# Ali-Xiyao/emr2a-evidence-grounded-multimodal-retrieval

Measured on NVIDIA B200. Metric: queries/sec (cosine Top-K + vote), higher is better.
Workload: dtype bf16+f32

## Files before the change

### emr2a_b200/csrc/api.cu

```cuda
#include "common.cuh"

#include <math.h>
#include <stdlib.h>
#include <string.h>

namespace emr2a {

static thread_local char g_err[512] = "";

int fail(int code, const char* fmt, ...) {
  va_list ap;
  va_start(ap, fmt);
  vsnprintf(g_err, sizeof(g_err), fmt, ap);
  va_end(ap);
  return code;
}
int cuda_fail(cudaError_t e, const char* where) {
  snprintf(g_err, sizeof(g_err), "CUDA error %d (%s) at %s", static_cast<int>(e), cudaGetErrorString(e), where);
  cudaGetLastError();
  return EMR2A_ERR_CUDA;
}
int sm_count() {
  int dev = 0, n = 0;
  if (cudaGetDevice(&dev) != cudaSuccess) return 148;
  if (cudaDeviceGetAttribute(&n, cudaDevAttrMultiProcessorCount, dev) != cudaSuccess || n <= 0) return 148;
  return n;
}

size_t simt_topk_workspace_bytes(int64_t Q, int64_t N, int K);
int simt_topk_search(const float* q, const float* db, int64_t Q, int64_t N, int D, int64_t ldq, int64_t lddb,
                     const uint8_t* q_fold, const uint8_t* db_fold, int64_t idx_base, int K, uint64_t* out_keys,
                     void* workspace, size_t ws_bytes, cudaStream_t st);
size_t tc_topk_workspace_bytes(int64_t Q, int64_t N, int K, int D);
int tc_debug_unit_clocks(unsigned long long* host_out, int64_t cap_units, int64_t* plan_out);
struct TcPartials {
  const uint64_t* parts;
  int splits;
  const uint32_t* tau;
};
int tc_topk_search(const uint16_t* q_hi, const uint16_t* q_lo, const uint16_t* db_hi, const uint16_t* db_lo,
                   int64_t Q, int64_t N, int D, int64_t ldq, int64_t lddb, const uint8_t* q_fold,
                   const uint8_t* db_fold, int64_t idx_base, int K, int passes, uint64_t* out_keys,
                   void* workspace, size_t ws_bytes, float* debug_scores, cudaStream_t st, TcPartials* partials,
                   int fold_sorted, int min_splits);
int tc_planned_splits(int64_t Q, int64_t N, int min_splits);
int tc_timing_enable(int on);
int tc_timing_read(float* ms_out, int cap, int* n_out);
void tc_timing_record(int which, cudaStream_t st);
int tc_range_filter(const uint16_t* q_hi, const uint16_t* db_hi, int64_t Q, int64_t N, int D, int64_t ldq, int64_t lddb,
                    const uint8_t* q_fold, const uint8_t* db_fold, int fold_sorted, int64_t idx_base, float min_score,
                    const float* q_stats, const float* db_stats, uint64_t* cand, int64_t cand_cap,
                    unsigned long long* count, void* workspace, size_t ws_bytes, cudaStream_t st);

size_t rescore_workspace_bytes(int64_t Q, int K);
int rescore_pipeline(const uint64_t* approx, int KP, const uint32_t* tau, const float* q, int64_t ldq, const float* db,
                     int64_t lddb, const emr2a_lazy_rows* db_lazy, const uint16_t* db_hi, int64_t lddb_hi, int64_t Q, int64_t N,
                     int D, int64_t idx_base, int K,
                     const float* q_stats, const float* db_stats, const uint8_t* q_fold, const uint8_t* db_fold,
                     uint64_t* out_keys, int* status, uint8_t* qflags, void* workspace, size_t ws_bytes, cudaStream_t st);

int rescore_kth_scores(const uint64_t* approx, int KP, int K, int64_t Q, float* kth, cudaStream_t st);
int rescore_select_only(const uint64_t* approx, int KP, const uint32_t* tau, const float* kth_floor, const float* q,
                        int64_t ldq, const float* db, int64_t lddb, const emr2a_lazy_rows* db_lazy, int64_t Q, int64_t N, int D,
                        int64_t idx_base, int K, const float* q_stats, const float* db_stats, uint64_t* out_keys,
                        float* bound_out, cudaStream_t st);
int rescore_verify_merged(const uint64_t* keys, int K, int64_t Q, const float* bounds, int parts, int64_t bounds_stride,
                          uint8_t* flags, int* count, cudaStream_t st);
size_t exact_rescan_workspace_bytes(int n_flagged, int K);
int rescore_exact_rescan(const float* q, int64_t ldq, const float* db, int64_t lddb, const emr2a_lazy_rows* db_lazy, int64_t N,
                         int D, int64_t idx_base, int K, const uint8_t* q_fold, const uint8_t* db_fold, const int* flag_list,
                         int n_flagged, uint64_t* out_compact, void* workspace, size_t ws_bytes, const uint16_t* db_hi,
                         int64_t lddb_hi, const float* q_stats, const float* db_stats, const uint64_t* seed_keys,
                         cudaStream_t st);

int range_refine_check(const float* q, int64_t ldq, const float* db, int64_t lddb, const emr2a_lazy_rows* db_lazy, int D);
int range_refine(const uint64_t* cand, int64_t cand_cap, unsigned long long* counts, uint64_t* out, int64_t out_cap,
                 const float* q, int64_t ldq, const float* db, int64_t lddb, const emr2a_lazy_rows* db_lazy, int D,
                 int64_t idx_base, float min_score, cudaStream_t st);

constexpr int RESCORE_KP = 32;
constexpr int RESCORE_KPM = 64;
static inline size_t align256(size_t x) { return (x + 255) & ~static_cast<size_t>(255); }

__global__ void zero_keys_kernel(uint64_t* k, int64_t n) {
  const int64_t i = static_cast<int64_t>(blockIdx.x) * blockDim.x + threadIdx.x;
  if (i < n) k[i] = 0ull;
}

}

using namespace emr2a;

extern "C" int emr2a_abi_version(void) { return EMR2A_ABI_VERSION; }
extern "C" const char* emr2a_last_error(void) { return g_err; }

extern "C" int emr2a_device_check(int* sms, int* cc_major, int* cc_minor) {
  int dev = 0;
  EMR2A_CUDA_TRY(cudaGetDevice(&dev));
  int major = 0, minor = 0, n = 0;
  EMR2A_CUDA_TRY(cudaDeviceGetAttribute(&major, cudaDevAttrComputeCapabilityMajor, dev));
  EMR2A_CUDA_TRY(cudaDeviceGetAttribute(&minor, cudaDevAttrComputeCapabilityMinor, dev));
  EMR2A_CUDA_TRY(cudaDeviceGetAttribute(&n, cudaDevAttrMultiProcessorCount, dev));
  if (sms) *sms = n;
  if (cc_major) *cc_major = major;
  if (cc_minor) *cc_minor = minor;
  if (major != 10) return fail(EMR2A_ERR_UNSUPPORTED, "libemr2a is built for sm_100a only; device is sm_%d%d", major, minor);
  return EMR2A_OK;
}

extern "C" size_t emr2a_topk_search_workspace_bytes(int64_t Q, int64_t N, int D, int K, int precision) {
  if (Q <= 0 || N <= 0 || K <= 0) return 256;
  if (precision == EMR2A_PREC_FP32) return simt_topk_workspace_bytes(Q, N, K) + 256;
  if (precision == EMR2A_PREC_BF16_RESCORE) {
    return align256(sizeof(uint64_t) * static_cast<size_t>(Q) * RESCORE_KPM) +
           align256(tc_topk_workspace_bytes(Q, N, RESCORE_KP, D)) + align256(rescore_workspace_bytes(Q, K));
  }
  return tc_topk_workspace_bytes(Q, N, K, D);
}

static int rescore_filter_stage(const uint16_t* q_hi, int64_t ldq_bf16, const uint16_t* db_hi, int64_t lddb_bf16, int64_t Q,
                                int64_t N, int D, const uint8_t* q_fold, const uint8_t* db_fold, int fold_sorted,
                                int64_t idx_base, int K, uint64_t* approx, void* tc_ws, size_t tc_ws_bytes,
                                float* debug_scores, cudaStream_t st, const uint64_t** cand, int* kpm,
                                const uint32_t** tau) {
  TcPartials parts{};
  const int planned = tc_planned_splits(Q, N, 2);
  int kp = planned > 128 ? 8 : ((planned >= 8 || K <= 5) ? 16 : RESCORE_KP);
  {
    const char* e = getenv("EMR2A_RESCORE_KP");
    const int v = (e && *e) ? atoi(e) : 0;
    if (v == 8 || v == 16 || v == 32) kp = v;
  }
  int rc = tc_topk_search(q_hi, nullptr, db_hi, nullptr, Q, N, D, ldq_bf16, lddb_bf16, q_fold, db_fold, idx_base,
                          kp, 1, nullptr, tc_ws, tc_ws_bytes, debug_scores, st, &parts, fold_sorted, 2);
  if (rc != EMR2A_OK) return rc;
  *kpm = kp;
  *cand = parts.parts;
  *tau = parts.tau;
  if (parts.splits > 1) {
    *kpm = RESCORE_KPM;
    rc = emr2a_topk_merge(parts.parts, parts.splits, Q, kp, Q * kp, kp, RESCORE_KPM, approx, st);
    if (rc != EMR2A_OK) return rc;
    *cand = approx;
  }
  return EMR2A_OK;
}

static int topk_search_impl(const float* q_f32, int64_t ldq_f32, const uint16_t* q_hi, const uint16_t* q_lo,
                            int64_t ldq_bf16, const float* db_f32, int64_t lddb_f32, const uint16_t* db_hi,
                            const uint16_t* db_lo, int64_t lddb_bf16, int64_t Q, int64_t N, int D,
                            const uint8_t* q_fold, const uint8_t* db_fold, int fold_sorted, int64_t idx_base, int K,
                            int precision, const float* q_stats, const float* db_stats, uint64_t* out_keys,
                            int32_t* status, uint8_t* qflags, void* workspace, size_t ws_bytes, float* debug_scores,
                            const emr2a_lazy_rows* db_lazy, void* stream) {
  if (Q < 0 || N < 0 || D <= 0 || K <= 0 || !out_keys) return fail(EMR2A_ERR_INVALID, "topk_search: bad arguments (Q=%lld N=%lld D=%d K=%d)", (long long)Q, (long long)N, D, K);
  if ((q_fold == nullptr) != (db_fold == nullptr)) return fail(EMR2A_ERR_INVALID, "topk_search: q_fold and db_fold must be given together");
  if (idx_base < 0) return fail(EMR2A_ERR_INVALID, "topk_search: negative idx_base");
  cudaStream_t st = static_cast<cudaStream_t>(stream);
  if (Q == 0) return EMR2A_OK;
  if (N == 0) {
    const int64_t n = Q * K;
    zero_keys_kernel<<<static_cast<unsigned>((n + 255) / 256), 256, 0, st>>>(out_keys, n);
    EMR2A_LAUNCH_CHECK("zero_keys_kernel");
    return EMR2A_OK;
  }
  switch (precision) {
    case EMR2A_PREC_FP32:
      if (!q_f32 || !db_f32) return fail(EMR2A_ERR_INVALID, "topk_search(fp32): q_f32/db_f32 required");
      if (ldq_f32 < D || lddb_f32 < D) return fail(EMR2A_ERR_INVALID, "topk_search(fp32): leading dimension smaller than D");
      return simt_topk_search(q_f32, db_f32, Q, N, D, ldq_f32, lddb_f32, q_fold, db_fold, idx_base, K, out_keys, workspace, ws_bytes, st);
    case EMR2A_PREC_BF16X3:
      return tc_topk_search(q_hi, q_lo, db_hi, db_lo, Q, N, D, ldq_bf16, lddb_bf16, q_fold, db_fold, idx_base, K, 3, out_keys, workspace, ws_bytes, debug_scores, st, nullptr, fold_sorted, 1);
    case EMR2A_PREC_BF16X1:
      return tc_topk_search(q_hi, nullptr, db_hi, nullptr, Q, N, D, ldq_bf16, lddb_bf16, q_fold, db_fold, idx_base, K, 1, out_keys, workspace, ws_bytes, debug_scores, st, nullptr, fold_sorted, 1);
    case EMR2A_PREC_BF16_RESCORE: {
      if (K > 10) return fail(EMR2A_ERR_UNSUPPORTED, "topk_search(rescore): K=%d > 10 (use EMR2A_PREC_BF16X3)", K);
      if (!q_f32 || (!db_f32 && !db_lazy)) return fail(EMR2A_ERR_INVALID, "topk_search(rescore): q_f32 and db_f32 (or db_lazy) required");
      if (ldq_f32 < D || (!db_lazy && lddb_f32 < D)) return fail(EMR2A_ERR_INVALID, "topk_search(rescore): leading dimension smaller than D");
      if (!workspace || (reinterpret_cast<uintptr_t>(workspace) & 255)) return fail(EMR2A_ERR_INVALID, "topk_search(rescore): workspace must be 256-byte aligned");
      const size_t a_bytes = align256(sizeof(uint64_t) * static_cast<size_t>(Q) * RESCORE_KPM);
      const size_t t_bytes = align256(tc_topk_workspace_bytes(Q, N, RESCORE_KP, D));
      const size_t r_bytes = align256(rescore_workspace_bytes(Q, K));
      if (ws_bytes < a_bytes + t_bytes + r_bytes) return fail(EMR2A_ERR_WORKSPACE, "topk_search(rescore): workspace %zu < %zu", ws_bytes, a_bytes + t_bytes + r_bytes);
      uint8_t* ws = static_cast<uint8_t*>(workspace);
      const uint64_t* cand = nullptr;
      const uint32_t* tau = nullptr;
      int kpm = 0;
      int rc = rescore_filter_stage(q_hi, ldq_bf16, db_hi, lddb_bf16, Q, N, D, q_fold, db_fold, fold_sorted, idx_base, K,
                                    reinterpret_cast<uint64_t*>(ws), ws + a_bytes, t_bytes, debug_scores, st, &cand, &kpm, &tau);
      if (rc != EMR2A_OK) return rc;
      return rescore_pipeline(cand, kpm, tau, q_f32, ldq_f32, db_f32, lddb_f32, db_lazy, db_hi, lddb_bf16, Q, N, D, idx_base, K, q_stats,
                              db_stats, q_fold, db_fold, out_keys, status, qflags, ws + a_bytes + t_bytes, r_bytes, st);
    }
    default:
      return fail(EMR2A_ERR_INVALID, "topk_search: unknown precision %d", precision);
  }
}

extern "C" int emr2a_topk_search(const float* q_f32, int64_t ldq_f32, const uint16_t* q_hi, const uint16_t* q_lo,
                                 int64_t ldq_bf16, const float* db_f32, int64_t lddb_f32, const uint16_t* db_hi,
                                 const uint16_t* db_lo, int64_t lddb_bf16, int64_t Q, int64_t N, int D,
                                 const uint8_t* q_fold, const uint8_t* db_fold, int fold_sorted, int64_t idx_base,
                                 int K, int precision, const float* q_stats, const float* db_stats,
                                 uint64_t* out_keys, int32_t* status_out, uint8_t* unverified_out, void* workspace,
                                 size_t ws_bytes, const emr2a_lazy_rows* db_lazy, void* stream) {
  if (db_lazy && precision != EMR2A_PREC_BF16_RESCORE) return fail(EMR2A_ERR_INVALID, "topk_search: db_lazy is for EMR2A_PREC_BF16_RESCORE only");
  return topk_search_impl(q_f32, ldq_f32, q_hi, q_lo, ldq_bf16, db_f32, lddb_f32, db_hi, db_lo, lddb_bf16, Q, N, D,
                          q_fold, db_fold, fold_sorted, idx_base, K, precision, q_stats, db_stats, out_keys,
                          status_out, unverified_out, workspace, ws_bytes, nullptr, db_lazy, stream);
}

extern "C" int emr2a_debug_topk_search_dump(const uint16_t* q_hi, const uint16_t* q_lo, const uint16_t* db_hi,
                                            const uint16_t* db_lo, int64_t Q, int64_t N, int D, int64_t ldq,
                                            int64_t lddb, const uint8_t* q_fold, const uint8_t* db_fold,
                                            int64_t idx_base, int K, int precision, uint64_t* out_keys,
                                            void* workspace, size_t ws_bytes, float* debug_scores, void* stream) {
  if (precision != EMR2A_PREC_BF16X3 && precision != EMR2A_PREC_BF16X1)
    return fail(EMR2A_ERR_INVALID, "debug dump is for the tensor-core arms only");
  return topk_search_impl(nullptr, 0, q_hi, q_lo, ldq, nullptr, 0, db_hi, db_lo, lddb, Q, N, D, q_fold, db_fold, 0,
                          idx_base, K, precision, nullptr, nullptr, out_keys, nullptr, nullptr, workspace, ws_bytes,
                          debug_scores, nullptr, stream);
}

extern "C" int emr2a_debug_unit_clocks(uint64_t* host_out, int64_t cap_units, int64_t* plan_out) {
  if (!host_out || !plan_out) return fail(EMR2A_ERR_INVALID, "debug_unit_clocks: null output");
  return tc_debug_unit_clocks(reinterpret_cast<unsigned long long*>(host_out), cap_units, plan_out);
}

extern "C" size_t emr2a_topk_filter_workspace_bytes(int64_t Q, int64_t N, int D, int K) {
  if (Q <= 0 || N <= 0 || K <= 0) return 256;
  return align256(tc_topk_workspace_bytes(Q, N, RESCORE_KP, D));
}

extern "C" int emr2a_topk_filter(const uint16_t* q_hi, int64_t ldq_bf16, const uint16_t* db_hi, int64_t lddb_bf16, int64_t Q,
                                 int64_t N, int D, const uint8_t* q_fold, const uint8_t* db_fold, int fold_sorted,
                                 int64_t idx_base, int K, uint64_t* cand_out, uint32_t* tau_out, float* kth_out,
                                 void* workspace, size_t ws_bytes, void* stream) {
  if (Q < 0 || N < 0 || D <= 0 || K <= 0 || !cand_out || !tau_out) return fail(EMR2A_ERR_INVALID, "topk_filter: bad arguments");
  if (K > 10) return fail(EMR2A_ERR_UNSUPPORTED, "topk_filter: K=%d > 10 (use EMR2A_PREC_BF16X3)", K);
  if ((q_fold == nullptr) != (db_fold == nullptr)) return fail(EMR2A_ERR_INVALID, "topk_filter: q_fold and db_fold must be given together");
  cudaStream_t st = static_cast<cudaStream_t>(stream);
  if (Q == 0) return EMR2A_OK;
  EMR2A_CUDA_TRY(cudaMemsetAsync(tau_out, 0, sizeof(uint32_t) * static_cast<size_t>(Q), st));
  if (N == 0) {
    const int64_t n = Q * RESCORE_KPM;
    zero_keys_kernel<<<static_cast<unsigned>((n + 255) / 256), 256, 0, st>>>(cand_out, n);
    EMR2A_LAUNCH_CHECK("zero_keys_kernel");
  } else {
    if (!workspace || (reinterpret_cast<uintptr_t>(workspace) & 255)) return fail(EMR2A_ERR_INVALID, "topk_filter: workspace must be 256-byte aligned");
    const uint64_t* cand = nullptr;
    const uint32_t* tau = nullptr;
    int kpm = 0;
    int rc = rescore_filter_stage(q_hi, ldq_bf16, db_hi, lddb_bf16, Q, N, D, q_fold, db_fold, fold_sorted, idx_base, K,
                                  cand_out, workspace, ws_bytes, nullptr, st, &cand, &kpm, &tau);
    if (rc != EMR2A_OK) return rc;
    if (cand != cand_out) {
      rc = emr2a_topk_merge(cand, 1, Q, kpm, Q * kpm, kpm, RESCORE_KPM, cand_out, st);
      if (rc != EMR2A_OK) return rc;
    }
    if (tau) EMR2A_CUDA_TRY(cudaMemcpyAsync(tau_out, tau, sizeof(uint32_t) * static_cast<size_t>(Q), cudaMemcpyDeviceToDevice, st));
  }
  if (kth_out) return rescore_kth_scores(cand_out, RESCORE_KPM, K, Q, kth_out, st);
  return EMR2A_OK;
}

extern "C" int emr2a_rescore_candidates(const uint64_t* cand, const uint32_t* tau, const float* kth_floor, const float* q_f32,
                                        int64_t ldq_f32, const float* db_f32, int64_t lddb_f32, int64_t Q, int64_t N, int D,
                                        int64_t idx_base, int K, const float* q_stats, const float* db_stats,
                                        uint64_t* out_keys, float* bound_out, const emr2a_lazy_rows* db_lazy,
                                        void* stream) {
  if (!cand || !tau || !q_f32 || (!db_f32 && !db_lazy) || !q_stats || !db_stats || !out_keys || !bound_out || Q < 0 || N < 0 ||
      D <= 0 || K <= 0 || K > 10 || ldq_f32 < D || (!db_lazy && lddb_f32 < D))
    return fail(EMR2A_ERR_INVALID, "rescore_candidates: bad arguments");
  if (Q == 0) return EMR2A_OK;
  return rescore_select_only(cand, RESCORE_KPM, tau, kth_floor, q_f32, ldq_f32, db_f32, lddb_f32, db_lazy, Q, N, D, idx_base,
                             K, q_stats, db_stats, out_keys, bound_out, static_cast<cudaStream_t>(stream));
}

extern "C" int emr2a_verify_merged(const uint64_t* keys, int K, int64_t Q, const float* bounds, int parts,
                                   int64_t bounds_stride, uint8_t* flags_out, int32_t* status_out, void* stream) {
  if (!keys || !bounds || !flags_out || !status_out || K <= 0 || Q < 0 || parts <= 0 || bounds_stride < Q)
    return fail(EMR2A_ERR_INVALID, "verify_merged: bad arguments");
  if (Q == 0) return EMR2A_OK;
  return rescore_verify_merged(keys, K, Q, bounds, parts, bounds_stride, flags_out, status_out, static_cast<cudaStream_t>(stream));
}

extern "C" size_t emr2a_exact_rescan_workspace_bytes(int n_flagged, int K) { return exact_rescan_workspace_bytes(n_flagged, K) + 256; }

extern "C" int emr2a_exact_rescan(const float* q_f32, int64_t ldq_f32, const float* db_f32, int64_t lddb_f32, int64_t N, int D,
                                  int64_t idx_base, int K, const uint8_t* q_fold, const uint8_t* db_fold,
                                  const int32_t* flag_list, int n_flagged, uint64_t* out_keys, void* workspace,
                                  size_t ws_bytes, const emr2a_lazy_rows* db_lazy, const uint16_t* db_hi,
                                  int64_t lddb_bf16, const float* q_stats, const float* db_stats,
                                  const uint64_t* seed_keys, void* stream) {
  if (!q_f32 || (!db_f32 && !db_lazy && N > 0) || !out_keys || N < 0 || D <= 0 || K <= 0 || n_flagged < 0 || ldq_f32 < D ||
      (!db_lazy && N > 0 && lddb_f32 < D) || (n_flagged > 0 && !flag_list))
    return fail(EMR2A_ERR_INVALID, "exact_rescan: bad arguments");
  if ((q_fold == nullptr) != (db_fold == nullptr)) return fail(EMR2A_ERR_INVALID, "exact_rescan: q_fold and db_fold must be given together");
  if (n_flagged == 0) return EMR2A_OK;
  cudaStream_t st = static_cast<cudaStream_t>(stream);
  if (N == 0) {
    const int64_t n = static_cast<int64_t>(n_flagged) * K;
    zero_keys_kernel<<<static_cast<unsigned>((n + 255) / 256), 256, 0, st>>>(out_keys, n);
    EMR2A_LAUNCH_CHECK("zero_keys_kernel");
    return EMR2A_OK;
  }
  return rescore_exact_rescan(q_f32, ldq_f32, db_f32, lddb_f32, db_lazy, N, D, idx_base, K, q_fold, db_fold, flag_list,
                              n_flagged, out_keys, workspace, ws_bytes, db_hi, lddb_bf16, q_stats, db_stats, seed_keys, st);
}

extern "C" size_t emr2a_range_search_workspace_bytes(int64_t Q, int64_t N, int D) {
  if (Q <= 0 || N <= 0 || D <= 0) return 256;
  return align256(tc_topk_workspace_bytes(Q, N, 1, D));
}

extern "C" int emr2a_range_search(const float* q_f32, int64_t ldq_f32, const uint16_t* q_hi, int64_t ldq_bf16,
                                  const float* db_f32, int64_t lddb_f32, const uint16_t* db_hi, int64_t lddb_bf16,
                                  int64_t Q, int64_t N, int D, const uint8_t* q_fold, const uint8_t* db_fold,
                                  int fold_sorted, int64_t idx_base, float min_score, const float* q_stats,
                                  const float* db_stats, uint64_t* cand, int64_t cand_cap, uint64_t* results,
                                  int64_t result_cap, uint64_t* counts_out, void* workspace, size_t ws_bytes,
                                  const emr2a_lazy_rows* db_lazy, void* stream) {
  if (Q < 0 || N < 0 || D <= 0 || cand_cap < 0 || result_cap < 0 || !counts_out || (cand_cap > 0 && !cand) ||
      (result_cap > 0 && !results))
    return fail(EMR2A_ERR_INVALID, "range_search: bad arguments (Q=%lld N=%lld D=%d)", (long long)Q, (long long)N, D);
  if (!isfinite(min_score)) return fail(EMR2A_ERR_INVALID, "range_search: min_score must be finite");
  if ((q_fold == nullptr) != (db_fold == nullptr)) return fail(EMR2A_ERR_INVALID, "range_search: q_fold and db_fold must be given together");
  if (idx_base < 0) return fail(EMR2A_ERR_INVALID, "range_search: negative idx_base");
  if (!q_f32 || (!db_f32 && !db_lazy) || !q_stats || !db_stats)
    return fail(EMR2A_ERR_INVALID, "range_search: q_f32, db_f32 (or db_lazy), q_stats and db_stats required");
  if (ldq_f32 < D || (!db_lazy && lddb_f32 < D)) return fail(EMR2A_ERR_INVALID, "range_search: leading dimension smaller than D");
  if (Q == 0 || N == 0) return EMR2A_OK;
  if (!workspace || (reinterpret_cast<uintptr_t>(workspace) & 255)) return fail(EMR2A_ERR_INVALID, "range_search: workspace must be 256-byte aligned");
  int rc = range_refine_check(q_f32, ldq_f32, db_f32, lddb_f32, db_lazy, D);
  if (rc != EMR2A_OK) return rc;
  cudaStream_t st = static_cast<cudaStream_t>(stream);
  unsigned long long* counts = reinterpret_cast<unsigned long long*>(counts_out);
  rc = tc_range_filter(q_hi, db_hi, Q, N, D, ldq_bf16, lddb_bf16, q_fold, db_fold, fold_sorted, idx_base, min_score,
                           q_stats, db_stats, cand, cand_cap, counts, workspace, ws_bytes, st);
  if (rc != EMR2A_OK) return rc;
  tc_timing_record(0, st);
  rc = range_refine(cand, cand_cap, counts, results, result_cap, q_f32, ldq_f32, db_f32, lddb_f32, db_lazy, D, idx_base,
                    min_score, st);
  tc_timing_record(1, st);
  return rc;
}

extern "C" int emr2a_debug_tc_timing(int enable) { return tc_timing_enable(enable); }
extern "C" int emr2a_debug_tc_elapsed(float* ms_out_host, int cap, int* n_out_host) {
  if (!ms_out_host || !n_out_host || cap <= 0) return fail(EMR2A_ERR_INVALID, "debug_tc_elapsed: bad arguments");
  return tc_timing_read(ms_out_host, cap, n_out_host);
}
```

### emr2a_b200/csrc/normalize_fuse.cu

```cuda
#include <type_traits>
#include "row_math.cuh"

namespace emr2a {

struct NfParams {
  const void* seg0;
  const void* seg1;
  int64_t n;
  int d0, d1;
  int64_t ld0, ld1;
  float w0, w1;
  int flags;
  float* out_f32;
  int64_t ld_f32;
  uint16_t* out_hi;
  uint16_t* out_lo;
  int64_t ld_bf16;
  float* inv_norm;
  float* stats;
  const float* col_std;
  float* row_div;
};

__device__ __forceinline__ void stats_flush(float* stats, float max_norm2, float max_res2) {
  unsigned int* u = reinterpret_cast<unsigned int*>(stats);
  atomicMax(u, __float_as_uint(__fsqrt_ru(max_norm2)));
  atomicMax(u + 1, __float_as_uint(__fsqrt_ru(max_res2)));
}

template <typename InT, int MAXC>
__device__ __forceinline__ void load_row(const NfParams& p, int64_t row, int lane, int c0, int ctot, float4 (&v)[MAXC]) {
#pragma unroll
  for (int j = 0; j < MAXC; ++j) {
    const int c = lane + 32 * j;
    if (c < c0) v[j] = Loader<InT>::load4(p.seg0, row * p.ld0 + 4 * c);
    else if (c < ctot) v[j] = Loader<InT>::load4(p.seg1, row * p.ld1 + 4 * (c - c0));
    else v[j] = make_float4(0.f, 0.f, 0.f, 0.f);
  }
}

__device__ __forceinline__ float std1(float x, float m, float s, float r) {
  const float t = __fsub_rn(x, m);
  const float q0 = t * r;
  const float rem = fmaf(-q0, s, t);
  return fmaf(rem, r, q0);
}
__device__ __forceinline__ void standardize4(float4& v, const float* __restrict__ col_std, int dtot, int col) {
  const float4 m = __ldg(reinterpret_cast<const float4*>(col_std + col));
  const float4 s = __ldg(reinterpret_cast<const float4*>(col_std + dtot + col));
  const float4 r = __ldg(reinterpret_cast<const float4*>(col_std + 2 * dtot + col));
  v.x = std1(v.x, m.x, s.x, r.x); v.y = std1(v.y, m.y, s.y, r.y);
  v.z = std1(v.z, m.z, s.z, r.z); v.w = std1(v.w, m.w, s.w, r.w);
}

template <typename InT, int MAXC, bool WANT_LO, bool STATS, bool STD = false>
__global__ void __launch_bounds__(256, (MAXC <= 8 ? 2 : 1)) normalize_fuse_vec_kernel(const NfParams p) {
  const int lane = threadIdx.x & 31;
  const int64_t warp0 = (static_cast<int64_t>(blockIdx.x) * blockDim.x + threadIdx.x) >> 5;
  const int64_t nwarps = (static_cast<int64_t>(gridDim.x) * blockDim.x) >> 5;
  const int c0 = p.d0 >> 2;
  const int ctot = (p.d0 + p.d1) >> 2;
  const int cpad = p.out_hi ? static_cast<int>(p.ld_bf16 >> 2) : ctot;
  constexpr bool PREFETCH = MAXC <= 8;
  float max_n2 = 0.f, max_r2 = 0.f;

  float4 nxt[PREFETCH ? MAXC : 1];
  if (PREFETCH && warp0 < p.n) load_row<InT, MAXC>(p, warp0, lane, c0, ctot, reinterpret_cast<float4 (&)[MAXC]>(nxt));

  for (int64_t row = warp0; row < p.n; row += nwarps) {
    float4 v[MAXC];
    if (PREFETCH) {
#pragma unroll
      for (int j = 0; j < MAXC; ++j) v[j] = nxt[PREFETCH ? j : 0];
      if (row + nwarps < p.n) load_row<InT, MAXC>(p, row + nwarps, lane, c0, ctot, reinterpret_cast<float4 (&)[MAXC]>(nxt));
    } else {
      load_row<InT, MAXC>(p, row, lane, c0, ctot, v);
    }
    if (STD) {
#pragma unroll
      for (int j = 0; j < MAXC; ++j) {
        const int c = lane + 32 * j;
        if (c < ctot) standardize4(v[j], p.col_std, p.d0 + p.d1, 4 * c);
      }
    }
    float ss0 = 0.f, ss1 = 0.f;
    float4 divs = make_float4(1.f, 1.f, 1.f, 0.f);
    if (p.flags & EMR2A_NF_SEGNORM) {
#pragma unroll
      for (int j = 0; j < MAXC; ++j) {
        const int c = lane + 32 * j;
        if (c < c0) ss0 += sq4(v[j]); else ss1 += sq4(v[j]);
      }
    }
    if (p.flags & EMR2A_NF_SEGNORM) {
      const RowDiv n0 = row_div(__fsqrt_rn(warp_sum(ss0)) + EMR2A_EPS);
      const RowDiv n1 = row_div(__fsqrt_rn(warp_sum(ss1)) + EMR2A_EPS);
      divs.x = n0.d; divs.y = n1.d;
#pragma unroll
      for (int j = 0; j < MAXC; ++j) {
        const int c = lane + 32 * j;
        if (c < c0) div4(v[j], n0); else if (c < ctot) div4(v[j], n1);
      }
    }
    if (p.w0 != 1.0f || p.w1 != 1.0f) {
#pragma unroll
      for (int j = 0; j < MAXC; ++j) {
        const int c = lane + 32 * j;
        if (c < c0) mul4(v[j], p.w0); else if (c < ctot) mul4(v[j], p.w1);
      }
    }
    float inv = 1.0f;
    if (p.flags & (EMR2A_NF_ROWNORM | EMR2A_NF_ZERO_GUARD)) {
      float ss = 0.f;
#pragma unroll
      for (int j = 0; j < MAXC; ++j) ss += sq4(v[j]);
      float nrm = __fsqrt_rn(warp_sum(ss));
      const bool guard = (p.flags & EMR2A_NF_ZERO_GUARD) != 0;
      if (!guard) nrm += EMR2A_EPS;
      if (!(guard && nrm == 0.f)) {
        const RowDiv dv = row_div(nrm);
#pragma unroll
        for (int j = 0; j < MAXC; ++j) div4(v[j], dv);
        inv = dv.r;
        divs.z = nrm; divs.w = 1.f;
      }
    }
    if (p.inv_norm && lane == 0) p.inv_norm[row] = inv;
    if (p.row_div && lane == 0) reinterpret_cast<float4*>(p.row_div)[row] = divs;
    if (p.out_f32) {
#pragma unroll
      for (int j = 0; j < MAXC; ++j) {
        const int c = lane + 32 * j;
        if (c < ctot) *reinterpret_cast<float4*>(p.out_f32 + row * p.ld_f32 + 4 * c) = v[j];
      }
    }
    if (p.out_hi) {
      float n2 = 0.f, r2 = 0.f;
#pragma unroll
      for (int j = 0; j < MAXC; ++j) {
        const int c = lane + 32 * j;
        if (c < cpad) {
          const __nv_bfloat162 h01 = __floats2bfloat162_rn(v[j].x, v[j].y);
          const __nv_bfloat162 h23 = __floats2bfloat162_rn(v[j].z, v[j].w);
          const uint32_t u01 = *reinterpret_cast<const uint32_t*>(&h01);
          const uint32_t u23 = *reinterpret_cast<const uint32_t*>(&h23);
          *reinterpret_cast<uint2*>(p.out_hi + row * p.ld_bf16 + 4 * c) = make_uint2(u01, u23);
          if (WANT_LO || STATS) {
            const float e0 = v[j].x - __uint_as_float(u01 << 16);
            const float e1 = v[j].y - __uint_as_float(u01 & 0xFFFF0000u);
            const float e2 = v[j].z - __uint_as_float(u23 << 16);
            const float e3 = v[j].w - __uint_as_float(u23 & 0xFFFF0000u);
            if (STATS) {
              n2 += sq4(v[j]);
              r2 += e0 * e0 + e1 * e1 + e2 * e2 + e3 * e3;
            }
            if (WANT_LO) {
              const __nv_bfloat162 l01 = __floats2bfloat162_rn(e0, e1);
              const __nv_bfloat162 l23 = __floats2bfloat162_rn(e2, e3);
              *reinterpret_cast<uint2*>(p.out_lo + row * p.ld_bf16 + 4 * c) =
                  make_uint2(*reinterpret_cast<const uint32_t*>(&l01), *reinterpret_cast<const uint32_t*>(&l23));
            }
          }
        }
      }
      if (STATS) {
        max_n2 = fmaxf(max_n2, warp_sum(n2));
        max_r2 = fmaxf(max_r2, warp_sum(r2));
      }
    }
  }
  if (STATS && lane == 0 && warp0 < p.n) stats_flush(p.stats, max_n2, max_r2);
}

__device__ __forceinline__ float2 block_sum2(float a, float b, float2* red) {
  a = warp_sum(a); b = warp_sum(b);
  if ((threadIdx.x & 31) == 0) red[threadIdx.x >> 5] = make_float2(a, b);
  __syncthreads();
  float2 t = make_float2(0.f, 0.f);
#pragma unroll
  for (int w = 0; w < 8; ++w) { t.x += red[w].x; t.y += red[w].y; }
  __syncthreads();
  return t;
}

template <typename InT, int CPT>
__device__ __forceinline__ void load_row_block(const NfParams& p, int64_t row, int c0, int ctot,
                                               typename Loader<InT>::Raw (&v)[CPT]) {
#pragma unroll
  for (int j = 0; j < CPT; ++j) {
    const int c = threadIdx.x + 256 * j;
    if (c < c0) v[j] = Loader<InT>::load_raw(p.seg0, row * p.ld0 + 4 * c);
    else if (c < ctot) v[j] = Loader<InT>::load_raw(p.seg1, row * p.ld1 + 4 * (c - c0));
  }
}

template <typename InT, int CPT>
__global__ void __launch_bounds__(256, 2) normalize_fuse_block_kernel(const NfParams p) {
  typedef typename Loader<InT>::Raw Raw;
  constexpr int PF = sizeof(Raw) == 16 ? 1 : 2;
  __shared__ float2 red[8];
  const int c0 = p.d0 >> 2;
  const int ctot = (p.d0 + p.d1) >> 2;
  const int cpad = p.out_hi ? static_cast<int>(p.ld_bf16 >> 2) : ctot;
  float max_n2 = 0.f, max_r2 = 0.f;
  Raw ring[PF][CPT];
#pragma unroll
  for (int s = 0; s < PF; ++s) {
    const int64_t r = blockIdx.x + static_cast<int64_t>(s) * gridDim.x;
    if (r < p.n) load_row_block<InT, CPT>(p, r, c0, ctot, ring[s]);
  }
  for (int64_t base = blockIdx.x; base < p.n; base += static_cast<int64_t>(PF) * gridDim.x) {
#pragma unroll
   for (int s = 0; s < PF; ++s) {
    const int64_t row = base + static_cast<int64_t>(s) * gridDim.x;
    if (row >= p.n) break;
    float4 v[CPT];
#pragma unroll
    for (int j = 0; j < CPT; ++j) {
      const int c = threadIdx.x + 256 * j;
      v[j] = c < ctot ? Loader<InT>::widen(ring[s][j]) : make_float4(0.f, 0.f, 0.f, 0.f);
    }
    {
      const int64_t r2 = row + static_cast<int64_t>(PF) * gridDim.x;
      if (r2 < p.n) load_row_block<InT, CPT>(p, r2, c0, ctot, ring[s]);
    }
    float4 divs = make_float4(1.f, 1.f, 1.f, 0.f);
    if (p.flags & EMR2A_NF_SEGNORM) {
      float ss0 = 0.f, ss1 = 0.f;
#pragma unroll
      for (int j = 0; j < CPT; ++j) {
        const int c = threadIdx.x + 256 * j;
        if (c < c0) ss0 += sq4(v[j]); else ss1 += sq4(v[j]);
      }
      const float2 t = block_sum2(ss0, ss1, red);
      const RowDiv n0 = row_div(__fsqrt_rn(t.x) + EMR2A_EPS);
      const RowDiv n1 = row_div(__fsqrt_rn(t.y) + EMR2A_EPS);
      divs.x = n0.d; divs.y = n1.d;
#pragma unroll
      for (int j = 0; j < CPT; ++j) {
        const int c = threadIdx.x + 256 * j;
        if (c < c0) div4(v[j], n0); else if (c < ctot) div4(v[j], n1);
      }
    }
    if (p.w0 != 1.0f || p.w1 != 1.0f) {
#pragma unroll
      for (int j = 0; j < CPT; ++j) {
        const int c = threadIdx.x + 256 * j;
        if (c < c0) mul4(v[j], p.w0); else if (c < ctot) mul4(v[j], p.w1);
      }
    }
    float inv = 1.0f;
    if (p.flags & (EMR2A_NF_ROWNORM | EMR2A_NF_ZERO_GUARD)) {
// ... 215 lines not shown
```

### emr2a_b200/csrc/tc_common.cuh

```cuda
#pragma once
#include <cuda.h>
#include "common.cuh"

namespace emr2a {

constexpr int T_BM = 128;
constexpr int T_BN = 256;
constexpr int T_BK = 64;
constexpr int T_THREADS = 256;
constexpr uint32_t T_A_BYTES = T_BM * T_BK * 2;
constexpr uint32_t T_B_BYTES = T_BN * T_BK * 2;

struct TcParams {
  int64_t Q, N;
  int k_chunks;
  int64_t m_tiles, n_tiles;
  int splits;
  int64_t tiles_per_split;
  const uint8_t* q_fold;
  const uint8_t* db_fold;
  int fold_sorted;
  int64_t idx_base;
  int K;
  uint64_t* keys_out;
  uint32_t* tau;
  float* debug_scores;
  int64_t mg;
  int sync_tiles;
  int sync_points;
  int sync_budget;
  uint32_t* sync_ctr;
  unsigned long long* unit_clock;
  float range_t;
  int D;
  const float* q_stats;
  const float* db_stats;
  ulonglong2* range_out;
  int64_t range_cap;
  unsigned long long* range_count;
};

__device__ __forceinline__ uint32_t smem_u32(const void* p) { return static_cast<uint32_t>(__cvta_generic_to_shared(p)); }

__device__ __forceinline__ void mbar_init(uint32_t bar, uint32_t count) {
  asm volatile("mbarrier.init.shared::cta.b64 [%0], %1;" ::"r"(bar), "r"(count));
}
__device__ __forceinline__ void mbar_arrive_expect_tx(uint32_t bar, uint32_t bytes) {
  asm volatile("mbarrier.arrive.expect_tx.shared::cta.b64 _, [%0], %1;" ::"r"(bar), "r"(bytes) : "memory");
}
__device__ __forceinline__ void mbar_arrive(uint32_t bar) {
  asm volatile("mbarrier.arrive.shared::cta.b64 _, [%0];" ::"r"(bar) : "memory");
}
__device__ __forceinline__ bool mbar_try_wait(uint32_t bar, uint32_t parity) {
  uint32_t ok;
  asm volatile(
      "{\n\t"
      ".reg .pred p;\n\t"
      "mbarrier.try_wait.parity.shared::cta.b64 p, [%1], %2;\n\t"
      "selp.u32 %0, 1, 0, p;\n\t"
      "}\n" : "=r"(ok) : "r"(bar), "r"(parity) : "memory");
  return ok != 0;
}
__device__ __forceinline__ void mbar_wait(uint32_t bar, uint32_t parity) {
  while (!mbar_try_wait(bar, parity)) {}
}
__device__ __forceinline__ void tma_load_2d(uint32_t dst, const CUtensorMap* map, uint32_t bar, int c0, int c1) {
  asm volatile(
      "cp.async.bulk.tensor.2d.shared::cluster.global.mbarrier::complete_tx::bytes [%0], [%1, {%3, %4}], [%2];"
      ::"r"(dst), "l"(reinterpret_cast<uint64_t>(map)), "r"(bar), "r"(c0), "r"(c1) : "memory");
}
__device__ __forceinline__ void tcgen05_fence_before() { asm volatile("tcgen05.fence::before_thread_sync;" ::: "memory"); }
__device__ __forceinline__ void tcgen05_fence_after() { asm volatile("tcgen05.fence::after_thread_sync;" ::: "memory"); }
__device__ __forceinline__ void umma_commit(uint32_t bar) {
  asm volatile("tcgen05.commit.cta_group::1.mbarrier::arrive::one.shared::cluster.b64 [%0];" ::"r"(bar) : "memory");
}
__device__ __forceinline__ void umma_bf16(uint32_t tmem_d, uint64_t desc_a, uint64_t desc_b, uint32_t idesc, uint32_t accumulate) {
  asm volatile(
      "{\n\t"
      ".reg .pred p;\n\t"
      "setp.ne.b32 p, %4, 0;\n\t"
      "tcgen05.mma.cta_group::1.kind::f16 [%0], %1, %2, %3, p;\n\t"
      "}\n" ::"r"(tmem_d), "l"(desc_a), "l"(desc_b), "r"(idesc), "r"(accumulate) : "memory");
}
__device__ __forceinline__ uint64_t make_smem_desc(uint32_t smem_addr) {
  uint64_t d = 0;
  d |= static_cast<uint64_t>((smem_addr & 0x3FFFFu) >> 4);
  d |= static_cast<uint64_t>(0) << 16;
  d |= static_cast<uint64_t>(1024 >> 4) << 32;
  d |= static_cast<uint64_t>(1) << 46;
  d |= static_cast<uint64_t>(2) << 61;
  return d;
}
__device__ __forceinline__ void tmem_ld32(uint32_t taddr, float (&v)[32]) {
  uint32_t r[32];
  asm volatile(
      "tcgen05.ld.sync.aligned.32x32b.x32.b32 "
      "{%0, %1, %2, %3, %4, %5, %6, %7, %8, %9, %10, %11, %12, %13, %14, %15, "
      "%16, %17, %18, %19, %20, %21, %22, %23, %24, %25, %26, %27, %28, %29, %30, %31}, [%32];"
      : "=r"(r[0]), "=r"(r[1]), "=r"(r[2]), "=r"(r[3]), "=r"(r[4]), "=r"(r[5]), "=r"(r[6]), "=r"(r[7]),
        "=r"(r[8]), "=r"(r[9]), "=r"(r[10]), "=r"(r[11]), "=r"(r[12]), "=r"(r[13]), "=r"(r[14]), "=r"(r[15]),
        "=r"(r[16]), "=r"(r[17]), "=r"(r[18]), "=r"(r[19]), "=r"(r[20]), "=r"(r[21]), "=r"(r[22]), "=r"(r[23]),
        "=r"(r[24]), "=r"(r[25]), "=r"(r[26]), "=r"(r[27]), "=r"(r[28]), "=r"(r[29]), "=r"(r[30]), "=r"(r[31])
      : "r"(taddr));
  asm volatile("tcgen05.wait::ld.sync.aligned;" ::: "memory");
#pragma unroll
  for (int i = 0; i < 32; ++i) v[i] = __uint_as_float(r[i]);
}

constexpr uint32_t T_IDESC = (1u << 4) | (1u << 7) | (1u << 10) | ((T_BN >> 3) << 17) | ((T_BM >> 4) << 24);

template <int KCAP>
struct RegTopK {
  float s[KCAP];
  uint32_t i[KCAP];
  __device__ __forceinline__ void reset() {
#pragma unroll
    for (int j = 0; j < KCAP; ++j) { s[j] = -INFINITY; i[j] = 0xFFFFFFFFu; }
  }
  __device__ __forceinline__ float threshold() const { return s[KCAP - 1]; }
  __device__ __forceinline__ void insert(float c, uint32_t ci) {
#pragma unroll
    for (int j = KCAP - 1; j > 0; --j) {
// ... 79 lines not shown
  bool mask_rows = HAS_FOLD, all_masked = false;
  if (HAS_FOLD && p.fold_sorted) {
    const int64_t last = (n0 + T_BN - 1 < p.N) ? n0 + T_BN - 1 : p.N - 1;
    const uint32_t f_lo = __ldg(p.db_fold + n0), f_hi = __ldg(p.db_fold + last);
    if (f_lo == f_hi) { mask_rows = false; all_masked = (f_lo == my_fold); }
  }
#pragma unroll 1
  for (int ch = 0; ch < T_BN / 32; ++ch) {
    float v[32];
    tmem_ld32(taddr + static_cast<uint32_t>(ch * 32), v);
    const int64_t c0 = n0 + ch * 32;
    if (p.debug_scores && q < p.Q) {
#pragma unroll
      for (int c = 0; c < 32; ++c) if (c0 + c < p.N) p.debug_scores[q * p.N + c0 + c] = v[c];
    }
    if (edge) {
#pragma unroll
      for (int c = 0; c < 32; ++c) if (c0 + c >= p.N) v[c] = -INFINITY;
    }
    if (HAS_FOLD && all_masked) {
#pragma unroll
      for (int c = 0; c < 32; ++c) v[c] = -INFINITY;
    }
    if (HAS_FOLD && mask_rows) {
      const uint4* fp = reinterpret_cast<const uint4*>(p.db_fold + c0);
      const uint4 f0 = __ldg(fp), f1 = __ldg(fp + 1);
      const uint32_t w[8] = {f0.x, f0.y, f0.z, f0.w, f1.x, f1.y, f1.z, f1.w};
#pragma unroll
      for (int c = 0; c < 32; ++c) {
        const uint32_t f = (w[c >> 2] >> (8 * (c & 3))) & 0xFFu;
        v[c] = (f == my_fold) ? -INFINITY : v[c];
      }
    }
    if constexpr (RANGE) {
      range_emit(p, v, thr, c0, q);
    } else {
      float mx = v[0];
#pragma unroll
      for (int c = 1; c < 32; ++c) mx = fmaxf(mx, v[c]);
      if (mx > thr) {
        uint32_t mask = 0u;
#pragma unroll
        for (int c = 0; c < 32; ++c) mask |= (v[c] > thr) ? (1u << c) : 0u;
        while (mask) {
          const int c = __ffs(mask) - 1;
          mask &= mask - 1u;
          const float val = select32(v, c);
          if (val > thr) {
            top.insert(val, static_cast<uint32_t>(c0 + c + p.idx_base));
            thr = fmaxf(top.threshold(), thr0);
          }
        }
      }
    }
    __syncwarp();
  }
}

__device__ __forceinline__ void unit_coords(const TcParams& p, int64_t u, int64_t& split, int64_t& mt) {
  const int64_t per_group = p.mg * p.splits;
  const int64_t g = u / per_group;
  const int64_t r = u - g * per_group;
  const int64_t left = p.m_tiles - g * p.mg;
  const int64_t mg_eff = left < p.mg ? left : p.mg;
  split = r / mg_eff;
  mt = g * p.mg + (r - split * mg_eff);
}
__device__ __forceinline__ void unit_cohort(const TcParams& p, int64_t u, int64_t n_workers, int64_t n_units,
                                            int64_t& slot, int& size) {
  const int64_t per_group = p.mg * p.splits;
  const int64_t g = u / per_group;
  const int64_t r = u - g * per_group;
  const int64_t left = p.m_tiles - g * p.mg;
  const int64_t mg_eff = left < p.mg ? left : p.mg;
  const int64_t split = r / mg_eff;
  int64_t c0 = g * per_group + split * mg_eff, c1 = c0 + mg_eff;
  const int64_t step = u / n_workers;
  const int64_t s0 = step * n_workers, s1 = (s0 + n_workers < n_units) ? s0 + n_workers : n_units;
  c0 = c0 > s0 ? c0 : s0;
  c1 = c1 < s1 ? c1 : s1;
  size = static_cast<int>(c1 - c0);
  slot = g * p.splits + split + step;
}
__device__ __forceinline__ void cohort_sync(const TcParams& p, int64_t slot, int point, int size) {
  uint32_t* ctr = p.sync_ctr + slot * p.sync_points + point;
  const uint32_t seen = atomicAdd(ctr, 1u) + 1u;
  if (seen >= static_cast<uint32_t>(size)) return;
  const long long t0 = clock64();
  while (__ldcg(ctr) < static_cast<uint32_t>(size)) {
    if (clock64() - t0 > p.sync_budget) break;
    __nanosleep(40);
  }
}

__device__ __forceinline__ float unit_start_threshold(const TcParams& p, int64_t q) {
  if (p.tau == nullptr || q >= p.Q) return -INFINITY;
  const uint32_t t = __ldcg(p.tau + q);
  if (t == 0u) return -INFINITY;
  const float b = unorder_f32(t);
  const uint32_t bits = __float_as_uint(b);
  if (b > 0.f) return __uint_as_float(bits - 1u);
  if (b < 0.f) return __uint_as_float(bits + 1u);
  return -1e-45f;
}

}
```

### emr2a_b200/csrc/topk_tc.cu

```cuda
#include <stdlib.h>
#include "tc_common.cuh"

namespace emr2a {

template <int PASSES, int KCAP, bool HAS_FOLD, bool RANGE = false>
__global__ void __launch_bounds__(T_THREADS, 1)
tc_topk_kernel(const __grid_constant__ CUtensorMap tm_q_hi, const __grid_constant__ CUtensorMap tm_q_lo,
               const __grid_constant__ CUtensorMap tm_db_hi, const __grid_constant__ CUtensorMap tm_db_lo,
               const TcParams p) {
  constexpr int PLANES = PASSES == 3 ? 2 : 1;
  constexpr uint32_t STAGE_BYTES = PLANES * (T_A_BYTES + T_B_BYTES);
  constexpr int STAGES = PASSES == 3 ? 2 : 4;

  extern __shared__ uint8_t smem_dyn[];
  __shared__ __align__(8) uint64_t bar_full[STAGES];
  __shared__ __align__(8) uint64_t bar_empty[STAGES];
  __shared__ __align__(8) uint64_t bar_tfull[2];
  __shared__ __align__(8) uint64_t bar_tempty[2];
  __shared__ uint32_t tmem_base_smem;

  const int warp = threadIdx.x >> 5;
  const int lane = threadIdx.x & 31;
  const uint32_t tiles_base = (smem_u32(smem_dyn) + 1023u) & ~1023u;

// ... 115 lines not shown
        scan_tile<KCAP, HAS_FOLD, RANGE>(p, top, thr, thr0,
                                         tmem_base + (static_cast<uint32_t>(quarter * 32) << 16) + static_cast<uint32_t>(acc * T_BN),
                                         n0, my_fold, q);
        tcgen05_fence_before();
        __syncwarp();
        if (lane == 0) mbar_arrive(smem_u32(&bar_tempty[acc]));
        if (++acc == 2) { acc = 0; acc_phase ^= 1u; }
      }
      if (!RANGE && q < p.Q) {
        if (p.tau != nullptr && top.i[KCAP - 1] != 0xFFFFFFFFu) atomicMax(p.tau + q, order_f32(top.s[KCAP - 1]));
        uint64_t* dst = p.keys_out + (split * p.Q + q) * p.K;
#pragma unroll
        for (int j = 0; j < KCAP; ++j)
          if (j < p.K) dst[j] = (top.i[j] == 0xFFFFFFFFu) ? 0ull : pack_key(top.s[j], top.i[j]);
      }
    }
  }

  tcgen05_fence_before();
  __syncthreads();
  if (warp == 2) {
    tcgen05_fence_after();
    asm volatile("tcgen05.dealloc.cta_group::1.sync.aligned.b32 %0, %1;" ::"r"(tmem_base), "n"(512));
  }
}

typedef CUresult (*PFN_encodeTiled)(CUtensorMap*, CUtensorMapDataType, cuuint32_t, void*, const cuuint64_t*,
                                    const cuuint64_t*, const cuuint32_t*, const cuuint32_t*, CUtensorMapInterleave,
                                    CUtensorMapSwizzle, CUtensorMapL2promotion, CUtensorMapFloatOOBfill);

static PFN_encodeTiled get_encode() {
  static PFN_encodeTiled fn = nullptr;
  if (!fn) {
    void* sym = nullptr;
    cudaDriverEntryPointQueryResult qres;
    if (cudaGetDriverEntryPoint("cuTensorMapEncodeTiled", &sym, cudaEnableDefault, &qres) == cudaSuccess &&
        qres == cudaDriverEntryPointSuccess)
      fn = reinterpret_cast<PFN_encodeTiled>(sym);
  }
  return fn;
}

static int make_plane_map(CUtensorMap* map, const uint16_t* base, int64_t rows, int64_t cols, int64_t ld, int box_rows) {
  PFN_encodeTiled enc = get_encode();
  if (!enc) return fail(EMR2A_ERR_CUDA, "cuTensorMapEncodeTiled entry point not available");
  cuuint64_t gdim[2] = {static_cast<cuuint64_t>(cols), static_cast<cuuint64_t>(rows)};
  cuuint64_t gstride[1] = {static_cast<cuuint64_t>(ld) * 2};
  cuuint32_t box[2] = {static_cast<cuuint32_t>(T_BK), static_cast<cuuint32_t>(box_rows)};
  cuuint32_t estr[2] = {1, 1};
  CUresult r = enc(map, CU_TENSOR_MAP_DATA_TYPE_BFLOAT16, 2, const_cast<uint16_t*>(base), gdim, gstride, box, estr,
                   CU_TENSOR_MAP_INTERLEAVE_NONE, CU_TENSOR_MAP_SWIZZLE_128B, CU_TENSOR_MAP_L2_PROMOTION_L2_256B,
                   CU_TENSOR_MAP_FLOAT_OOB_FILL_NONE);
  if (r != CUDA_SUCCESS) return fail(EMR2A_ERR_CUDA, "cuTensorMapEncodeTiled failed (CUresult %d): rows=%lld cols=%lld ld=%lld", (int)r, (long long)rows, (long long)cols, (long long)ld);
  return EMR2A_OK;
}

struct TcPartials {
  const uint64_t* parts;
  int splits;
  const uint32_t* tau;
};

struct TcPlan {
  int64_t m_tiles, n_tiles, tiles_per_split;
  int splits;
  int grid;
  size_t keys_bytes, fold_bytes, tau_bytes;
  int64_t mg;
  int sync_tiles, sync_points, sync_budget;
  size_t sync_bytes;
};

static int env_int(const char* name, int dflt) {
  const char* e = getenv(name);
  return (e && *e) ? atoi(e) : dflt;
}

constexpr int64_t UNIT_CLOCK_MAX = 1 << 16;
__device__ unsigned long long g_unit_clock[2 * UNIT_CLOCK_MAX];
static int64_t g_last_plan[8];

int tc2_dispatch(int passes, int kcap, bool has_fold, const CUtensorMap& a, const CUtensorMap& b, const CUtensorMap& c,
                 const CUtensorMap& d, const TcParams& p, int grid, cudaStream_t st);

static bool use_cta_pairs(int64_t Q) {
  static int v = -1;
  if (v < 0) {
    const char* e = getenv("EMR2A_TC2");
    v = !e ? 2 : (e[0] == '0' ? 0 : 1);
  }
  return v == 2 ? Q > T_BM : v == 1;
}

static TcPlan tc_plan(int64_t Q, int64_t N, int K, bool has_fold, bool pairs, int min_splits = 1, int64_t ld = 1024,
                      int planes = 1) {
  TcPlan pl{};
  const int bm = pairs ? 2 * T_BM : T_BM;
  pl.m_tiles = (Q + bm - 1) / bm;
  pl.n_tiles = (N + T_BN - 1) / T_BN;
  const int sms = pairs ? sm_count() / 2 : sm_count();
  int best_s = 1; double best_eff = -1.0;
  int64_t cap = 64;
  if (pl.m_tiles * cap < sms) {
    const int kcap = K <= 8 ? 8 : (K <= 16 ? 16 : 32);
    cap = sms < 2048 / kcap ? sms : 2048 / kcap;
    if (cap < 64) cap = 64;
  }
  const int64_t max_s = pl.n_tiles < cap ? pl.n_tiles : cap;
  int64_t first_s = min_splits < max_s ? min_splits : max_s;
  if (first_s < 1) first_s = 1;
  best_s = static_cast<int>(first_s);
  for (int64_t s = first_s; s <= max_s; ++s) {
    const int64_t tps = (pl.n_tiles + s - 1) / s;
    const int64_t s_eff = (pl.n_tiles + tps - 1) / tps;
    if (s_eff != s) continue;
    const int64_t units = pl.m_tiles * s;
    const int64_t waves = (units + sms - 1) / sms;
    const double cost = static_cast<double>(waves) * (static_cast<double>(tps) + 2.0);
    const double ideal = static_cast<double>(pl.m_tiles) * pl.n_tiles / sms;
    const double eff = ideal / cost;
    if (eff > best_eff + 1e-9) { best_eff = eff; best_s = static_cast<int>(s); }
  }
  pl.splits = best_s;
  pl.tiles_per_split = (pl.n_tiles + pl.splits - 1) / pl.splits;
  const int64_t units = pl.m_tiles * pl.splits;
  pl.grid = static_cast<int>(units < sms ? units : sms) * (pairs ? 2 : 1);
  pl.keys_bytes = sizeof(uint64_t) * static_cast<size_t>(pl.splits) * Q * K;
  pl.fold_bytes = has_fold ? static_cast<size_t>(pl.n_tiles) * T_BN : 0;
  pl.tau_bytes = (sizeof(uint32_t) * static_cast<size_t>(Q) + 255) & ~static_cast<size_t>(255);
  pl.mg = pl.m_tiles;
  if (pairs) {
    const double a_tile = 2.0 * T_BM * static_cast<double>(ld) * 2.0 * planes;
    int64_t mg = static_cast<int64_t>(env_int("EMR2A_TC_A_MB", 40) * 1048576.0 / a_tile);
    if (mg < 1) mg = 1;
    if (mg < pl.m_tiles) {
      const int64_t j = (sms + mg - 1) / mg;
      mg = sms / j;
      if (mg < 1) mg = 1;
      pl.mg = mg;
    }
    const double b_tile = static_cast<double>(T_BN) * static_cast<double>(ld) * 2.0 * planes;
    int st = static_cast<int>(2097152.0 / b_tile + 0.5);
    st = st < 1 ? 1 : (st > 16 ? 16 : st);
    st = env_int("EMR2A_TC_SYNC", st);
    const int64_t cohort_max = pl.mg < pl.m_tiles ? pl.mg : pl.m_tiles;
    if (st > 0 && cohort_max > 1 && units > 1) {
      pl.sync_tiles = st;
      pl.sync_points = static_cast<int>((pl.tiles_per_split + st - 1) / st);
      pl.sync_budget = env_int("EMR2A_TC_SYNC_BUDGET", 12000);
      const int64_t groups = (pl.m_tiles + pl.mg - 1) / pl.mg;
      const int64_t slots = groups * pl.splits + (units + sms - 1) / sms + 2;
      pl.sync_bytes = (sizeof(uint32_t) * static_cast<size_t>(slots) * pl.sync_points + 255) & ~static_cast<size_t>(255);
    }
  }
  return pl;
}

int tc_planned_splits(int64_t Q, int64_t N, int min_splits) {
  return tc_plan(Q, N, 1, false, use_cta_pairs(Q), min_splits).splits;
}

size_t tc_topk_workspace_bytes(int64_t Q, int64_t N, int K, int D) {
  size_t need = 0;
  const int64_t ld = (static_cast<int64_t>(D) + T_BK - 1) / T_BK * T_BK;
  for (int v = 0; v < 8; ++v) {
    TcPlan pl = tc_plan(Q, N, K, true, (v & 1) != 0, (v & 2) ? 2 : 1, ld, (v & 4) ? 2 : 1);
    const size_t b = ((pl.keys_bytes + 255) & ~static_cast<size_t>(255)) + pl.fold_bytes + pl.tau_bytes + pl.sync_bytes + 1024;
    need = b > need ? b : need;
  }
  return need;
}

int tc_debug_unit_clocks(unsigned long long* host_out, int64_t cap_units, int64_t* plan_out) {
  for (int i = 0; i < 8; ++i) plan_out[i] = g_last_plan[i];
  int64_t n = g_last_plan[7];
  if (n > cap_units) n = cap_units;
  if (n > UNIT_CLOCK_MAX) n = UNIT_CLOCK_MAX;
  if (n > 0) EMR2A_CUDA_TRY(cudaMemcpyFromSymbol(host_out, g_unit_clock, sizeof(unsigned long long) * 2 * n));
  return EMR2A_OK;
}

constexpr int TC_EV_RING = 1024;
static cudaEvent_t g_tc_ev[TC_EV_RING][2];
static bool g_tc_ev_made[TC_EV_RING];
static long long g_tc_ev_count = 0;
static int g_tc_ev_on = 0;

static void tc_ev_record(int which, cudaStream_t st) {
  if (!g_tc_ev_on) return;
  const int slot = static_cast<int>(g_tc_ev_count % TC_EV_RING);
  if (!g_tc_ev_made[slot]) {
    if (cudaEventCreate(&g_tc_ev[slot][0]) != cudaSuccess || cudaEventCreate(&g_tc_ev[slot][1]) != cudaSuccess) { g_tc_ev_on = 0; return; }
    g_tc_ev_made[slot] = true;
  }
  cudaEventRecord(g_tc_ev[slot][which], st);
  if (which == 1) ++g_tc_ev_count;
}
int tc_timing_enable(int on) {
  g_tc_ev_on = on ? 1 : 0;
  g_tc_ev_count = 0;
  return EMR2A_OK;
}
int tc_timing_read(float* ms_out, int cap, int* n_out) {
  long long n = g_tc_ev_count < TC_EV_RING ? g_tc_ev_count : TC_EV_RING;
  if (n > cap) n = cap;
  for (long long i = 0; i < n; ++i) {
    const int slot = static_cast<int>((g_tc_ev_count - n + i) % TC_EV_RING);
    EMR2A_CUDA_TRY(cudaEventSynchronize(g_tc_ev[slot][1]));
    EMR2A_CUDA_TRY(cudaEventElapsedTime(ms_out + i, g_tc_ev[slot][0], g_tc_ev[slot][1]));
  }
  *n_out = static_cast<int>(n);
  return EMR2A_OK;
}

template <int PASSES, int KCAP, bool HAS_FOLD, bool RANGE = false>
static int tc_launch(const CUtensorMap& mq_hi, const CUtensorMap& mq_lo, const CUtensorMap& md_hi, const CUtensorMap& md_lo,
                     const TcParams& p, int grid, cudaStream_t st) {
  constexpr int PLANES = PASSES == 3 ? 2 : 1;
  constexpr int STAGES = PASSES == 3 ? 2 : 4;
  const size_t smem = static_cast<size_t>(STAGES) * PLANES * (T_A_BYTES + T_B_BYTES) + 1024;
  auto kern = tc_topk_kernel<PASSES, KCAP, HAS_FOLD, RANGE>;
  EMR2A_CUDA_TRY(cudaFuncSetAttribute(kern, cudaFuncAttributeMaxDynamicSharedMemorySize, static_cast<int>(smem)));
  kern<<<grid, T_THREADS, smem, st>>>(mq_hi, mq_lo, md_hi, md_lo, p);
  EMR2A_LAUNCH_CHECK("tc_topk_kernel");
  return EMR2A_OK;
}

template <int PASSES, int KCAP>
static int tc_launch_fold(bool has_fold, const CUtensorMap& a, const CUtensorMap& b, const CUtensorMap& c, const CUtensorMap& d,
                          const TcParams& p, int grid, cudaStream_t st) {
  return has_fold ? tc_launch<PASSES, KCAP, true>(a, b, c, d, p, grid, st)
                  : tc_launch<PASSES, KCAP, false>(a, b, c, d, p, grid, st);
}

static int check_planes(const char* who, const uint16_t* q_hi, const uint16_t* q_lo, const uint16_t* db_hi,
                        const uint16_t* db_lo, int64_t Q, int64_t N, int D, int64_t ldq, int64_t lddb, int64_t idx_base,
                        int passes) {
  const int64_t Dp = (static_cast<int64_t>(D) + T_BK - 1) / T_BK * T_BK;
  if (ldq < Dp || lddb < Dp || (ldq % 8) || (lddb % 8))
    return fail(EMR2A_ERR_UNSUPPORTED, "%s: planes need ld >= round_up(D,64) and ld %% 8 == 0 (ldq=%lld lddb=%lld D=%d)", who, (long long)ldq, (long long)lddb, D);
  if (!q_hi || !db_hi || (passes == 3 && (!q_lo || !db_lo))) return fail(EMR2A_ERR_INVALID, "%s: missing operand plane", who);
  auto mis = [](const void* ptr) { return (reinterpret_cast<uintptr_t>(ptr) & 15) != 0; };
  if (mis(q_hi) || mis(db_hi) || (passes == 3 && (mis(q_lo) || mis(db_lo))))
    return fail(EMR2A_ERR_UNSUPPORTED, "%s: operand planes must be 16-byte aligned", who);
  if (Q >= (1LL << 31) || N >= (1LL << 31) - T_BN) return fail(EMR2A_ERR_UNSUPPORTED, "%s: Q/N too large for one call", who);
  if (N + idx_base >= 0xFFFFFFFFLL) return fail(EMR2A_ERR_UNSUPPORTED, "%s: global index exceeds 32 bits", who);
  return EMR2A_OK;
}

int tc_topk_search(const uint16_t* q_hi, const uint16_t* q_lo, const uint16_t* db_hi, const uint16_t* db_lo,
                   int64_t Q, int64_t N, int D, int64_t ldq, int64_t lddb,
                   const uint8_t* q_fold, const uint8_t* db_fold, int64_t idx_base, int K, int passes,
                   uint64_t* out_keys, void* workspace, size_t ws_bytes, float* debug_scores, cudaStream_t st,
                   TcPartials* partials, int fold_sorted, int min_splits) {
  if (K > 32) return fail(EMR2A_ERR_UNSUPPORTED, "topk_search(bf16): K=%d > 32 (use EMR2A_PREC_FP32)", K);
  const int64_t Dp = (static_cast<int64_t>(D) + T_BK - 1) / T_BK * T_BK;
  {
    const int rc = check_planes("topk_search(bf16)", q_hi, q_lo, db_hi, db_lo, Q, N, D, ldq, lddb, idx_base, passes);
    if (rc != EMR2A_OK) return rc;
  }
  const bool has_fold = q_fold != nullptr;
  const bool pairs = use_cta_pairs(Q);
  TcPlan pl = tc_plan(Q, N, K, has_fold, pairs, min_splits, lddb > ldq ? lddb : ldq, passes == 3 ? 2 : 1);
  const size_t keys_off = 0;
  const size_t fold_off = (pl.keys_bytes + 255) & ~static_cast<size_t>(255);
  const size_t tau_off = (fold_off + pl.fold_bytes + 255) & ~static_cast<size_t>(255);
  const size_t sync_off = tau_off + pl.tau_bytes;
  const size_t need = sync_off + pl.sync_bytes;
  if (!workspace || ws_bytes < need) return fail(EMR2A_ERR_WORKSPACE, "topk_search(bf16): workspace %zu < %zu", ws_bytes, need);
  uint8_t* ws = static_cast<uint8_t*>(workspace);
  if ((reinterpret_cast<uintptr_t>(ws) & 255) != 0) return fail(EMR2A_ERR_INVALID, "topk_search(bf16): workspace must be 256-byte aligned");

  CUtensorMap mq_hi, mq_lo, md_hi, md_lo;
  int rc;
  if ((rc = make_plane_map(&mq_hi, q_hi, Q, Dp, ldq, T_BM)) != EMR2A_OK) return rc;
  const int db_box = pairs ? T_BN / 2 : T_BN;
  if ((rc = make_plane_map(&md_hi, db_hi, N, Dp, lddb, db_box)) != EMR2A_OK) return rc;
  if (passes == 3) {
    if ((rc = make_plane_map(&mq_lo, q_lo, Q, Dp, ldq, T_BM)) != EMR2A_OK) return rc;
    if ((rc = make_plane_map(&md_lo, db_lo, N, Dp, lddb, db_box)) != EMR2A_OK) return rc;
  } else {
    mq_lo = mq_hi; md_lo = md_hi;
  }
  TcParams p{};
  p.Q = Q; p.N = N; p.k_chunks = static_cast<int>(Dp / T_BK);
  p.m_tiles = pl.m_tiles; p.n_tiles = pl.n_tiles; p.splits = pl.splits; p.tiles_per_split = pl.tiles_per_split;
  p.idx_base = idx_base; p.K = K; p.debug_scores = debug_scores;
  p.keys_out = (pl.splits > 1 || partials) ? reinterpret_cast<uint64_t*>(ws + keys_off) : out_keys;
  if (pl.splits > 1) {
    p.tau = reinterpret_cast<uint32_t*>(ws + tau_off);
    EMR2A_CUDA_TRY(cudaMemsetAsync(p.tau, 0, sizeof(uint32_t) * static_cast<size_t>(Q), st));
  }
  p.mg = pl.mg;
  if (pairs && pl.sync_bytes) {
    p.sync_tiles = pl.sync_tiles; p.sync_points = pl.sync_points; p.sync_budget = pl.sync_budget;
    p.sync_ctr = reinterpret_cast<uint32_t*>(ws + sync_off);
    EMR2A_CUDA_TRY(cudaMemsetAsync(p.sync_ctr, 0, pl.sync_bytes, st));
  }
  if (pairs && env_int("EMR2A_TC_UNIT_CLOCK", 0) && pl.m_tiles * pl.splits <= UNIT_CLOCK_MAX) {
    void* sym = nullptr;
    EMR2A_CUDA_TRY(cudaGetSymbolAddress(&sym, g_unit_clock));
    p.unit_clock = static_cast<unsigned long long*>(sym);
    const int64_t plan[8] = {pl.m_tiles, pl.n_tiles, pl.splits, pl.tiles_per_split, pl.mg, pl.sync_tiles, pl.grid,
                             pl.m_tiles * pl.splits};
    for (int i = 0; i < 8; ++i) g_last_plan[i] = plan[i];
  }
  if (has_fold) {
    uint8_t* fpad = ws + fold_off;
    EMR2A_CUDA_TRY(cudaMemsetAsync(fpad, 0xFF, pl.fold_bytes, st));
    EMR2A_CUDA_TRY(cudaMemcpyAsync(fpad, db_fold, static_cast<size_t>(N), cudaMemcpyDeviceToDevice, st));
    p.q_fold = q_fold; p.db_fold = fpad; p.fold_sorted = fold_sorted;
  }
  const int kcap = K <= 8 ? 8 : (K <= 16 ? 16 : 32);
  tc_ev_record(0, st);
  if (pairs) {
    rc = tc2_dispatch(passes, kcap, has_fold, mq_hi, mq_lo, md_hi, md_lo, p, pl.grid, st);
  } else if (passes == 3) {
    if (kcap == 8) rc = tc_launch_fold<3, 8>(has_fold, mq_hi, mq_lo, md_hi, md_lo, p, pl.grid, st);
    else if (kcap == 16) rc = tc_launch_fold<3, 16>(has_fold, mq_hi, mq_lo, md_hi, md_lo, p, pl.grid, st);
    else rc = tc_launch_fold<3, 32>(has_fold, mq_hi, mq_lo, md_hi, md_lo, p, pl.grid, st);
  } else {
    if (kcap == 8) rc = tc_launch_fold<1, 8>(has_fold, mq_hi, mq_lo, md_hi, md_lo, p, pl.grid, st);
    else if (kcap == 16) rc = tc_launch_fold<1, 16>(has_fold, mq_hi, mq_lo, md_hi, md_lo, p, pl.grid, st);
    else rc = tc_launch_fold<1, 32>(has_fold, mq_hi, mq_lo, md_hi, md_lo, p, pl.grid, st);
  }
  tc_ev_record(1, st);
  if (rc != EMR2A_OK) return rc;
  if (partials) {
    partials->parts = p.keys_out;
    partials->splits = pl.splits;
    partials->tau = p.tau;
    return EMR2A_OK;
  }
  if (pl.splits > 1)
    return emr2a_topk_merge(reinterpret_cast<const uint64_t*>(ws + keys_off), pl.splits, Q, K, Q * K, K, K, out_keys, st);
  return EMR2A_OK;
}

void tc_timing_record(int which, cudaStream_t st) { tc_ev_record(which, st); }

int tc2_range_dispatch(bool has_fold, const CUtensorMap& a, const CUtensorMap& b, const CUtensorMap& c,
                       const CUtensorMap& d, const TcParams& p, int grid, cudaStream_t st);

int tc_range_filter(const uint16_t* q_hi, const uint16_t* db_hi, int64_t Q, int64_t N, int D, int64_t ldq, int64_t lddb,
                    const uint8_t* q_fold, const uint8_t* db_fold, int fold_sorted, int64_t idx_base, float min_score,
                    const float* q_stats, const float* db_stats, uint64_t* cand, int64_t cand_cap,
                    unsigned long long* count, void* workspace, size_t ws_bytes, cudaStream_t st) {
  int rc = check_planes("range_search", q_hi, nullptr, db_hi, nullptr, Q, N, D, ldq, lddb, idx_base, 1);
  if (rc != EMR2A_OK) return rc;
  const int64_t Dp = (static_cast<int64_t>(D) + T_BK - 1) / T_BK * T_BK;
  const bool has_fold = q_fold != nullptr;
  const bool pairs = use_cta_pairs(Q);
  const TcPlan pl = tc_plan(Q, N, 1, has_fold, pairs, 1, lddb > ldq ? lddb : ldq, 1);
  const size_t sync_off = (pl.fold_bytes + 255) & ~static_cast<size_t>(255);
  if (!workspace || ws_bytes < sync_off + pl.sync_bytes)
    return fail(EMR2A_ERR_WORKSPACE, "range_search: workspace %zu < %zu", ws_bytes, sync_off + pl.sync_bytes);
  uint8_t* ws = static_cast<uint8_t*>(workspace);
  CUtensorMap mq, md;
  if ((rc = make_plane_map(&mq, q_hi, Q, Dp, ldq, T_BM)) != EMR2A_OK) return rc;
  if ((rc = make_plane_map(&md, db_hi, N, Dp, lddb, pairs ? T_BN / 2 : T_BN)) != EMR2A_OK) return rc;
  TcParams p{};
  p.Q = Q; p.N = N; p.k_chunks = static_cast<int>(Dp / T_BK);
  p.m_tiles = pl.m_tiles; p.n_tiles = pl.n_tiles; p.splits = pl.splits; p.tiles_per_split = pl.tiles_per_split;
  p.idx_base = idx_base; p.K = 1;
  p.mg = pl.mg;
  if (pairs && pl.sync_bytes) {
    p.sync_tiles = pl.sync_tiles; p.sync_points = pl.sync_points; p.sync_budget = pl.sync_budget;
    p.sync_ctr = reinterpret_cast<uint32_t*>(ws + sync_off);
    EMR2A_CUDA_TRY(cudaMemsetAsync(p.sync_ctr, 0, pl.sync_bytes, st));
  }
  if (has_fold) {
    EMR2A_CUDA_TRY(cudaMemsetAsync(ws, 0xFF, pl.fold_bytes, st));
    EMR2A_CUDA_TRY(cudaMemcpyAsync(ws, db_fold, static_cast<size_t>(N), cudaMemcpyDeviceToDevice, st));
    p.q_fold = q_fold; p.db_fold = ws; p.fold_sorted = fold_sorted;
  }
  p.range_t = min_score; p.D = D; p.q_stats = q_stats; p.db_stats = db_stats;
  p.range_out = reinterpret_cast<ulonglong2*>(cand); p.range_cap = cand_cap; p.range_count = count;
  tc_ev_record(0, st);
  if (pairs) rc = tc2_range_dispatch(has_fold, mq, mq, md, md, p, pl.grid, st);
  else rc = has_fold ? tc_launch<1, 8, true, true>(mq, mq, md, md, p, pl.grid, st)
                     : tc_launch<1, 8, false, true>(mq, mq, md, md, p, pl.grid, st);
  tc_ev_record(1, st);
  return rc;
}

}
```

### emr2a_b200/csrc/topk_tc2.cu

```cuda
#include "tc_common.cuh"

namespace emr2a {

constexpr int T2_BM = 256;
constexpr uint32_t T2_BH_BYTES = 128 * T_BK * 2;
constexpr uint32_t T2_IDESC = (1u << 4) | (1u << 7) | (1u << 10) | ((T_BN >> 3) << 17) | ((T2_BM >> 4) << 24);

__device__ __forceinline__ uint32_t cluster_ctarank() {
  uint32_t r;
  asm volatile("mov.u32 %0, %%cluster_ctarank;" : "=r"(r));
  return r;
}
__device__ __forceinline__ void cluster_sync_all() {
  asm volatile("barrier.cluster.arrive.release.aligned;" ::: "memory");
  asm volatile("barrier.cluster.wait.acquire.aligned;" ::: "memory");
}
__device__ __forceinline__ void mbar_arrive_remote(uint32_t bar, uint32_t cta) {
  asm volatile(
      "{\n\t"
      ".reg .b32 ra;\n\t"
      "mapa.shared::cluster.u32 ra, %0, %1;\n\t"
      "mbarrier.arrive.release.cluster.shared::cluster.b64 _, [ra];\n\t"
      "}\n" ::"r"(bar), "r"(cta) : "memory");
}
__device__ __forceinline__ void tma_load_2d_2sm(uint32_t dst, const CUtensorMap* map, uint32_t bar_leader, int c0, int c1) {
  asm volatile(
      "cp.async.bulk.tensor.2d.cta_group::2.shared::cluster.global.mbarrier::complete_tx::bytes [%0], [%1, {%3, %4}], [%2];"
      ::"r"(dst), "l"(reinterpret_cast<uint64_t>(map)), "r"(bar_leader), "r"(c0), "r"(c1) : "memory");
}
__device__ __forceinline__ void umma_commit_2sm(uint32_t bar) {
  asm volatile("tcgen05.commit.cta_group::2.mbarrier::arrive::one.shared::cluster.multicast::cluster.b64 [%0], %1;"
               ::"r"(bar), "h"(static_cast<uint16_t>(3)) : "memory");
}
__device__ __forceinline__ void umma_bf16_2sm(uint32_t tmem_d, uint64_t desc_a, uint64_t desc_b, uint32_t idesc, uint32_t accumulate) {
  asm volatile(
      "{\n\t"
      ".reg .pred p;\n\t"
      "setp.ne.b32 p, %4, 0;\n\t"
      "tcgen05.mma.cta_group::2.kind::f16 [%0], %1, %2, %3, p;\n\t"
      "}\n" ::"r"(tmem_d), "l"(desc_a), "l"(desc_b), "r"(idesc), "r"(accumulate) : "memory");
}

template <int PASSES, int KCAP, bool HAS_FOLD, bool RANGE = false>
__global__ void __cluster_dims__(2, 1, 1) __launch_bounds__(T_THREADS, 1)
tc2_topk_kernel(const __grid_constant__ CUtensorMap tm_q_hi, const __grid_constant__ CUtensorMap tm_q_lo,
                const __grid_constant__ CUtensorMap tm_db_hi, const __grid_constant__ CUtensorMap tm_db_lo,
                const TcParams p) {
  constexpr int PLANES = PASSES == 3 ? 2 : 1;
  constexpr uint32_t STAGE_BYTES = PLANES * (T_A_BYTES + T2_BH_BYTES);
  constexpr int STAGES = PASSES == 3 ? 3 : 6;

  extern __shared__ uint8_t smem_dyn[];
  __shared__ __align__(8) uint64_t bar_full[STAGES];
  __shared__ __align__(8) uint64_t bar_empty[STAGES];
  __shared__ __align__(8) uint64_t bar_tfull[2];
  __shared__ __align__(8) uint64_t bar_tempty[2];
  __shared__ uint32_t tmem_base_smem;

  const int warp = threadIdx.x >> 5;
  const int lane = threadIdx.x & 31;
  const uint32_t rank = cluster_ctarank();
  const bool leader = rank == 0;
  const uint32_t tiles_base = (smem_u32(smem_dyn) + 1023u) & ~1023u;

  if (warp == 0 && lane == 0) {
    asm volatile("prefetch.tensormap [%0];" ::"l"(reinterpret_cast<uint64_t>(&tm_q_hi)) : "memory");
    asm volatile("prefetch.tensormap [%0];" ::"l"(reinterpret_cast<uint64_t>(&tm_db_hi)) : "memory");
  }
  if (warp == 1 && lane == 0) {
    for (int s = 0; s < STAGES; ++s) { mbar_init(smem_u32(&bar_full[s]), 1); mbar_init(smem_u32(&bar_empty[s]), 1); }
    for (int a = 0; a < 2; ++a) { mbar_init(smem_u32(&bar_tfull[a]), 1); mbar_init(smem_u32(&bar_tempty[a]), 8); }
    asm volatile("fence.mbarrier_init.release.cluster;" ::: "memory");
  }
  if (warp == 2) {
    asm volatile("tcgen05.alloc.cta_group::2.sync.aligned.shared::cta.b32 [%0], %1;" ::"r"(smem_u32(&tmem_base_smem)), "r"(512));
    asm volatile("tcgen05.relinquish_alloc_permit.cta_group::2.sync.aligned;");
  }
  tcgen05_fence_before();
  __syncthreads();
  cluster_sync_all();
  tcgen05_fence_after();
  const uint32_t tmem_base = tmem_base_smem;

  const int64_t n_units = p.m_tiles * p.splits;
  const int64_t pair = blockIdx.x >> 1;
  const int64_t n_pairs = gridDim.x >> 1;

  if (warp == 0) {
    if (lane == 0) {
      int stage = 0; uint32_t phase = 0;
      for (int64_t u = pair; u < n_units; u += n_pairs) {
        int64_t split, mt;
        unit_coords(p, u, split, mt);
        const int m0 = static_cast<int>(mt * T2_BM + rank * T_BM);
        const int64_t t0 = split * p.tiles_per_split;
        const int64_t t1 = (t0 + p.tiles_per_split < p.n_tiles) ? t0 + p.tiles_per_split : p.n_tiles;
        const int ufold = HAS_FOLD ? unit_fold(p, mt, T2_BM) : -1;
        int64_t slot = 0; int cohort = 1;
        if (leader && p.sync_tiles > 0) unit_cohort(p, u, n_pairs, n_units, slot, cohort);
        for (int64_t t = t0; t < t1; ++t) {
          if (leader && cohort > 1 && (t - t0) % p.sync_tiles == 0)
            cohort_sync(p, slot, static_cast<int>((t - t0) / p.sync_tiles), cohort);
          if (leader && p.unit_clock != nullptr && t == t0) {
            unsigned long long now;
            asm volatile("mov.u64 %0, %%globaltimer;" : "=l"(now));
            p.unit_clock[2 * u] = now;
          }
          if (HAS_FOLD && tile_skipped(p, ufold, t)) continue;
          const int n0 = static_cast<int>(t * T_BN + rank * 128);
          for (int kc = 0; kc < p.k_chunks; ++kc) {
            mbar_wait(smem_u32(&bar_empty[stage]), phase ^ 1u);
            const uint32_t full_leader = smem_u32(&bar_full[stage]) & 0xFEFFFFFFu;
            if (leader) mbar_arrive_expect_tx(smem_u32(&bar_full[stage]), 2u * STAGE_BYTES);
            const uint32_t sb = tiles_base + stage * STAGE_BYTES;
            tma_load_2d_2sm(sb, &tm_q_hi, full_leader, kc * T_BK, m0);
            tma_load_2d_2sm(sb + PLANES * T_A_BYTES, &tm_db_hi, full_leader, kc * T_BK, n0);
            if (PASSES == 3) {
              tma_load_2d_2sm(sb + T_A_BYTES, &tm_q_lo, full_leader, kc * T_BK, m0);
              tma_load_2d_2sm(sb + PLANES * T_A_BYTES + T2_BH_BYTES, &tm_db_lo, full_leader, kc * T_BK, n0);
            }
            if (++stage == STAGES) { stage = 0; phase ^= 1u; }
          }
        }
      }
    }
  } else if (warp == 1) {
    if (leader && lane == 0) {
      int stage = 0; uint32_t phase = 0;
      int acc = 0; uint32_t acc_phase = 0;
      for (int64_t u = pair; u < n_units; u += n_pairs) {
        int64_t split, mt;
        unit_coords(p, u, split, mt);
        const int64_t t0 = split * p.tiles_per_split;
        const int64_t t1 = (t0 + p.tiles_per_split < p.n_tiles) ? t0 + p.tiles_per_split : p.n_tiles;
        const int ufold = HAS_FOLD ? unit_fold(p, mt, T2_BM) : -1;
        for (int64_t t = t0; t < t1; ++t) {
          if (HAS_FOLD && tile_skipped(p, ufold, t)) continue;
          mbar_wait(smem_u32(&bar_tempty[acc]), acc_phase ^ 1u);
          tcgen05_fence_after();
          const uint32_t d_tmem = tmem_base + static_cast<uint32_t>(acc * T_BN);
          for (int kc = 0; kc < p.k_chunks; ++kc) {
            mbar_wait(smem_u32(&bar_full[stage]), phase);
            tcgen05_fence_after();
            const uint32_t sb = tiles_base + stage * STAGE_BYTES;
            const uint64_t a_hi = make_smem_desc(sb);
            const uint64_t b_hi = make_smem_desc(sb + PLANES * T_A_BYTES);
            const uint64_t a_lo = make_smem_desc(sb + T_A_BYTES);
            const uint64_t b_lo = make_smem_desc(sb + PLANES * T_A_BYTES + T2_BH_BYTES);
#pragma unroll
            for (int k = 0; k < T_BK / 16; ++k) {
              const uint64_t koff = static_cast<uint64_t>((k * 32) >> 4);
              if (PASSES == 3) {
                umma_bf16_2sm(d_tmem, a_hi + koff, b_lo + koff, T2_IDESC, (kc | k) != 0 ? 1u : 0u);
                umma_bf16_2sm(d_tmem, a_lo + koff, b_hi + koff, T2_IDESC, 1u);
                umma_bf16_2sm(d_tmem, a_hi + koff, b_hi + koff, T2_IDESC, 1u);
              } else {
                umma_bf16_2sm(d_tmem, a_hi + koff, b_hi + koff, T2_IDESC, (kc | k) != 0 ? 1u : 0u);
              }
            }
            umma_commit_2sm(smem_u32(&bar_empty[stage]));
            if (++stage == STAGES) { stage = 0; phase ^= 1u; }
          }
          umma_commit_2sm(smem_u32(&bar_tfull[acc]));
          if (++acc == 2) { acc = 0; acc_phase ^= 1u; }
        }
      }
    }
  } else if (warp >= 4) {
    const int quarter = warp & 3;
    const int row = quarter * 32 + lane;
    int acc = 0; uint32_t acc_phase = 0;
    RegTopK<KCAP> top;
    float cut = 0.f;
    if constexpr (RANGE) cut = range_cut(p);
    for (int64_t u = pair; u < n_units; u += n_pairs) {
      int64_t split, mt;
      unit_coords(p, u, split, mt);
      const int64_t q = mt * T2_BM + rank * T_BM + row;
      const int64_t t0 = split * p.tiles_per_split;
      const int64_t t1 = (t0 + p.tiles_per_split < p.n_tiles) ? t0 + p.tiles_per_split : p.n_tiles;
      const uint32_t my_fold = (HAS_FOLD && q < p.Q) ? p.q_fold[q] : 0xFFFFu;
      if constexpr (!RANGE) top.reset();
      const float thr0 = RANGE ? cut : unit_start_threshold(p, q);
      float thr = thr0;
      const int ufold = HAS_FOLD ? unit_fold(p, mt, T2_BM) : -1;
      for (int64_t t = t0; t < t1; ++t) {
        if (HAS_FOLD && tile_skipped(p, ufold, t)) continue;
        const int64_t n0 = t * T_BN;
        mbar_wait(smem_u32(&bar_tfull[acc]), acc_phase);
        tcgen05_fence_after();
        scan_tile<KCAP, HAS_FOLD, RANGE>(p, top, thr, thr0,
                                         tmem_base + (static_cast<uint32_t>(quarter * 32) << 16) + static_cast<uint32_t>(acc * T_BN),
                                         n0, my_fold, q);
        tcgen05_fence_before();
        __syncwarp();
        if (lane == 0) {
          if (leader) mbar_arrive(smem_u32(&bar_tempty[acc]));
          else mbar_arrive_remote(smem_u32(&bar_tempty[acc]), 0);
        }
        if (++acc == 2) { acc = 0; acc_phase ^= 1u; }
      }
      if (!RANGE && q < p.Q) {
        if (p.tau != nullptr && top.i[KCAP - 1] != 0xFFFFFFFFu) atomicMax(p.tau + q, order_f32(top.s[KCAP - 1]));
        uint64_t* dst = p.keys_out + (split * p.Q + q) * p.K;
#pragma unroll
        for (int j = 0; j < KCAP; ++j)
          if (j < p.K) dst[j] = (top.i[j] == 0xFFFFFFFFu) ? 0ull : pack_key(top.s[j], top.i[j]);
      }
      if (leader && p.unit_clock != nullptr && threadIdx.x == 128) {
        unsigned long long now;
        asm volatile("mov.u64 %0, %%globaltimer;" : "=l"(now));
        p.unit_clock[2 * u + 1] = now;
      }
    }
  }

  tcgen05_fence_before();
  __syncthreads();
  cluster_sync_all();
  if (warp == 2) {
    tcgen05_fence_after();
    asm volatile("tcgen05.dealloc.cta_group::2.sync.aligned.b32 %0, %1;" ::"r"(tmem_base), "r"(512));
  }
}

template <int PASSES, int KCAP, bool HAS_FOLD, bool RANGE = false>
static int tc2_launch(const CUtensorMap& mq_hi, const CUtensorMap& mq_lo, const CUtensorMap& md_hi, const CUtensorMap& md_lo,
                      const TcParams& p, int grid, cudaStream_t st) {
  constexpr int PLANES = PASSES == 3 ? 2 : 1;
  constexpr int STAGES = PASSES == 3 ? 3 : 6;
  const size_t smem = static_cast<size_t>(STAGES) * PLANES * (T_A_BYTES + T2_BH_BYTES) + 1024;
  auto kern = tc2_topk_kernel<PASSES, KCAP, HAS_FOLD, RANGE>;
  EMR2A_CUDA_TRY(cudaFuncSetAttribute(kern, cudaFuncAttributeMaxDynamicSharedMemorySize, static_cast<int>(smem)));
  kern<<<grid, T_THREADS, smem, st>>>(mq_hi, mq_lo, md_hi, md_lo, p);
  EMR2A_LAUNCH_CHECK("tc2_topk_kernel");
  return EMR2A_OK;
}

int tc2_dispatch(int passes, int kcap, bool has_fold, const CUtensorMap& a, const CUtensorMap& b, const CUtensorMap& c,
                 const CUtensorMap& d, const TcParams& p, int grid, cudaStream_t st) {
#define EMR2A_TC2_CASE(P, KC)                                                                  \
  if (passes == P && kcap == KC)                                                              \
    return has_fold ? tc2_launch<P, KC, true>(a, b, c, d, p, grid, st) : tc2_launch<P, KC, false>(a, b, c, d, p, grid, st);
  EMR2A_TC2_CASE(1, 8) EMR2A_TC2_CASE(1, 16) EMR2A_TC2_CASE(1, 32)
  EMR2A_TC2_CASE(3, 8) EMR2A_TC2_CASE(3, 16) EMR2A_TC2_CASE(3, 32)
#undef EMR2A_TC2_CASE
  return fail(EMR2A_ERR_INVALID, "tc2_dispatch: unsupported (passes=%d, kcap=%d)", passes, kcap);
}

int tc2_range_dispatch(bool has_fold, const CUtensorMap& a, const CUtensorMap& b, const CUtensorMap& c,
                       const CUtensorMap& d, const TcParams& p, int grid, cudaStream_t st) {
  return has_fold ? tc2_launch<1, 8, true, true>(a, b, c, d, p, grid, st) : tc2_launch<1, 8, false, true>(a, b, c, d, p, grid, st);
}

}
```

### emr2a_b200/dist.py

```python
from __future__ import annotations

import os
from typing import Dict, List, Optional, Sequence, Tuple

import torch
import torch.distributed as dist

from .engine import Operand


def shard_range(n_rows: int, rank: int, world: int, align: int = 256) -> Tuple[int, int]:
    per = (n_rows + world - 1) // world
    per = (per + align - 1) // align * align
    lo = min(rank * per, n_rows)
    hi = min(lo + per, n_rows)
    return lo, hi


def spread_device(local_rank: int, local_world: int, visible: Optional[int] = None) -> int:
    if visible is None:
        visible = torch.cuda.device_count()
    if os.environ.get("EMR2A_SPREAD_DEVICES", "1") == "0" or local_world <= 0 or visible <= local_world or visible % local_world:
        return local_rank
    return local_rank * (visible // local_world)


_H2D_RATES: Optional[List[float]] = None


def h2d_rates(device, mbytes: int = 256, reps: int = 3) -> List[float]:
    global _H2D_RATES
    if _H2D_RATES is not None:
        return _H2D_RATES
    world = dist.get_world_size() if dist.is_initialized() else 1
    n = (mbytes << 20) // 4
    host = torch.empty(n, dtype=torch.float32).pin_memory()
    buf = torch.empty(n, dtype=torch.float32, device=device)
    buf.copy_(host, non_blocking=True)
    torch.cuda.synchronize(device)
    if world > 1:
        dist.barrier()
    e0, e1 = torch.cuda.Event(enable_timing=True), torch.cuda.Event(enable_timing=True)
    e0.record()
    for _ in range(reps):
        buf.copy_(host, non_blocking=True)
    e1.record()
    torch.cuda.synchronize(device)
    mine = torch.tensor([reps * n * 4 / (e0.elapsed_time(e1) / 1e3) / 1e9], dtype=torch.float64, device=device)
    if world > 1:
        allr = [torch.zeros_like(mine) for _ in range(world)]
        dist.all_gather(allr, mine)
        _H2D_RATES = [float(t) for t in allr]
    else:
        _H2D_RATES = [float(mine)]
    return _H2D_RATES


def weighted_ranges(n_rows: int, weights: Sequence[float], align: int = 256) -> List[Tuple[int, int]]:
    w = [max(float(x), 0.0) for x in weights]
    total = sum(w)
    if total <= 0:
        w, total = [1.0] * len(w), float(len(w))
    out, lo, acc = [], 0, 0.0
    for r, x in enumerate(w):
        acc += x
        hi = n_rows if r == len(w) - 1 else min(n_rows, int(round(n_rows * acc / total / align)) * align)
        hi = max(hi, lo)
        out.append((lo, hi))
        lo = hi
    return out


def gather_host_rows(host_mats: Sequence[torch.Tensor], device) -> Tuple[List[torch.Tensor], int]:
    world = dist.get_world_size() if dist.is_initialized() else 1
    rank = dist.get_rank() if dist.is_initialized() else 0
    out, copied = [], 0
    for m in host_mats:
        n = int(m.shape[0])
        per = (n + world - 1) // world
        lo, hi = min(rank * per, n), min(rank * per + per, n)
        mine = torch.zeros((per,) + tuple(m.shape[1:]), dtype=m.dtype, device=device)
        if hi > lo:
            mine[:hi - lo].copy_(m[lo:hi], non_blocking=True)
            copied += (hi - lo) * int(m[0].numel()) * m.element_size()
        out.append(gather_keys(mine).reshape((world * per,) + tuple(m.shape[1:]))[:n])
    return out, copied


def gather_keys(local_keys: torch.Tensor, group=None) -> torch.Tensor:
    world = dist.get_world_size(group) if dist.is_initialized() else 1
    if world == 1:
        return local_keys.unsqueeze(0)
    local_keys = local_keys.contiguous()
    out = torch.empty((world,) + tuple(local_keys.shape), dtype=local_keys.dtype, device=local_keys.device)
    if local_keys.is_cuda:
        dist.all_gather_into_tensor(out.view(-1), local_keys.view(-1), group=group)
    else:
        parts = [out[r] for r in range(world)]
        dist.all_gather(parts, local_keys, group=group)
    return out


def sharded_search_and_vote(eng, db_segs_local: Sequence, q_segs: Sequence, db_labels_global, q_labels,
                            n_classes: int, k: int, row_offset: int, db_flags: int, q_flags: int,
                            q_weights=(1.0, 1.0), k_list=(1, 3, 5), precision: str = "auto",
                            q_fold=None, db_fold_local=None, q_group=None, n_groups: int = 1,
                            want_lists: bool = True, timers: Optional[dict] = None,
                            defer_status: bool = False, cooperative: bool = True) -> Dict[str, torch.Tensor]:
    n_q = int(q_segs[0].shape[0])
    n_db = int(db_segs_local[0].shape[0])
    dim = sum(int(s.shape[1]) for s in db_segs_local if s is not None)
    world = dist.get_world_size() if dist.is_initialized() else 1
    prec = eng.pick_precision(n_q, max(n_db, 1) * world, dim, k, precision)
    db = eng.prepare(db_segs_local[0], db_segs_local[1] if len(db_segs_local) > 1 else None, 1.0, 1.0, db_flags, prec,
                     defer_f32=eng.defer_default(dim))
    qs = eng.prepare(q_segs[0], q_segs[1] if len(q_segs) > 1 else None, q_weights[0], q_weights[1], q_flags, prec)
    if prec == "rescore" and world > 1 and cooperative and os.environ.get("EMR2A_COOP_SHARDS", "1") != "0":
        return _cooperative_search_and_vote(eng, qs, db, db_labels_global, q_labels, n_classes, k, row_offset, k_list,
                                            q_fold, db_fold_local, q_group, n_groups, want_lists, timers, defer_status)
    if timers is not None:
        timers["k2_start"].record()
    keys = eng.topk_search(qs, db, k, prec, q_fold=q_fold, db_fold=db_fold_local, idx_base=row_offset)
    if timers is not None:
        timers["k2_end"].record()
    status = eng.pop_status_tensor() if prec == "rescore" else None
    if world > 1:
        payload = keys.reshape(-1)
        if status is not None:
            payload = torch.cat([payload, status.to(torch.int64)])
        allp = gather_keys(payload.unsqueeze(0)).squeeze(1)
        allk = allp[:, :keys.numel()].reshape(world, *keys.shape)
        if status is not None:
            status = allp[:, keys.numel():].to(torch.int32).max(dim=0).values
        keys = eng.topk_merge(allk, k)
    res = eng.vote_metrics(keys, db_labels_global, q_labels, n_classes, k_list=k_list, q_group=q_group,
                           n_groups=n_groups, want_lists=want_lists)
    res["keys"] = keys
    res["precision"] = prec
    if status is not None and defer_status:
        res["status"] = status
    elif status is not None:
        st = status.cpu()
        if int(st[1]):
            return sharded_search_and_vote(eng, db_segs_local, q_segs, db_labels_global, q_labels, n_classes, k,
                                           row_offset, db_flags, q_flags, q_weights, k_list, "bf16x3", q_fold,
                                           db_fold_local, q_group, n_groups, want_lists, timers)
        res["unverified"] = int(st[0])
    return res


def _cooperative_search_and_vote(eng, qs, db, db_labels_global, q_labels, n_classes, k, row_offset, k_list, q_fold,
                                 db_fold_local, q_group, n_groups, want_lists, timers, defer_status):
    n_q = qs.n
    if timers is not None:
        timers["k2_start"].record()
    cand, tau, kth = eng.topk_filter(qs, db, k, q_fold=q_fold, db_fold=db_fold_local, idx_base=row_offset)
    if timers is not None:
        timers["k2_end"].record()
    dist.all_reduce(kth, op=dist.ReduceOp.MAX)
    payload = eng.rescore_candidates(cand, tau, kth, qs, db, k, idx_base=row_offset)
    allp = gather_keys(payload.unsqueeze(0)).squeeze(1)
    keys = eng.merge_payload(allp, n_q, k)
    flags, status = eng.verify_merged(keys, allp, k)

    def vote(kk):
        return eng.vote_metrics(kk, db_labels_global, q_labels, n_classes, k_list=k_list, q_group=q_group,
                                n_groups=n_groups, want_lists=want_lists)

    res = vote(keys)
    res["precision"] = "rescore"
    res["keys"] = keys
    if defer_status:
        res["status"] = status
        return res
    n_flagged = int(status.cpu()[0])
    if n_flagged:
        idx = torch.nonzero(flags).squeeze(1).to(torch.int32)
        comp = eng.exact_rescan(qs, db, idx, k, idx_base=row_offset, q_fold=q_fold, db_fold=db_fold_local,
                                seed_keys=keys.index_select(0, idx.long()))
        keys.index_copy_(0, idx.long(), eng.topk_merge(gather_keys(comp), k))
        res = vote(keys)
        res["precision"] = "rescore"
        res["keys"] = keys
    res["unverified"] = n_flagged
    return res


def fold_balanced_ranges(fold_counts: Sequence[int], rank: int, world: int, align: int = 256) -> List[Tuple[int, int]]:
    out, start = [], 0
    for n_f in fold_counts:
        n_f = int(n_f)
        per = (n_f + world - 1) // world
        per = (per + align - 1) // align * align
        lo = min(rank * per, n_f)
        hi = min(lo + per, n_f)
        out.append((start + lo, hi - lo))
        start += n_f
    return out
# ... 132 lines not shown
```

### emr2a_b200/engine.py

```python
from __future__ import annotations

import ctypes as C
import os
from dataclasses import dataclass
from typing import Dict, List, Optional, Sequence, Tuple

import numpy as np
import torch

from . import native

_PREC = {"fp32": native.PREC_FP32, "bf16x3": native.PREC_BF16X3, "bf16x1": native.PREC_BF16X1,
         "rescore": native.PREC_BF16_RESCORE}
_RESCORE_MAX_K = 10
_QPAD_MAX = int(os.environ.get("EMR2A_QPAD_MAX", 256))
_TC_MIN_MACS = float(os.environ.get("EMR2A_TC_MIN_MACS", 2.0e9))


def _round_up(x: int, m: int) -> int:
    return (x + m - 1) // m * m


def _ld(t: torch.Tensor) -> int:
    return int(t.stride(0)) if t.shape[0] > 1 else int(t.shape[1])


@dataclass
class Operand:
    n: int
    dim: int
    f32: Optional[torch.Tensor] = None
    hi: Optional[torch.Tensor] = None
    lo: Optional[torch.Tensor] = None
    inv_norm: Optional[torch.Tensor] = None
    stats: Optional[torch.Tensor] = None
    lazy: Optional["DeferredRows"] = None

    @property
    def ld_planes(self) -> int:
        return 0 if self.hi is None else self.hi.shape[1]


@dataclass
class DeferredRows:
    seg0: torch.Tensor
    seg1: Optional[torch.Tensor]
    code: int
    w0: float
    w1: float
    flags: int
    row_div: torch.Tensor

    def struct(self, lo: int = 0, hi: Optional[int] = None) -> "native.LazyRows":
        a = self.seg0[lo:hi]
        b = self.seg1[lo:hi] if self.seg1 is not None else None
        return native.LazyRows(a.data_ptr(), b.data_ptr() if b is not None else None, int(a.shape[1]),
                               int(b.shape[1]) if b is not None else 0, _ld(a), _ld(b) if b is not None else 0, self.code,
                               float(self.w0), float(self.w1), int(self.flags), self.row_div[lo:hi].data_ptr())

    def slice(self, lo: int, hi: int) -> "DeferredRows":
        return DeferredRows(self.seg0[lo:hi], self.seg1[lo:hi] if self.seg1 is not None else None, self.code, self.w0,
                            self.w1, self.flags, self.row_div[lo:hi])


def _lazy_arg(op: "Operand"):
    if op.lazy is None:
        return None, None
    st = op.lazy.struct()
    return C.byref(st), st


_DEFER_F32 = os.environ.get("EMR2A_DEFER_F32", "1") != "0"
_DEFER_MAX_DIM = int(os.environ.get("EMR2A_DEFER_MAX_DIM", 8192))


class Engine:

    def __init__(self, device: Optional[torch.device] = None):
        if not torch.cuda.is_available():
            raise RuntimeError("emr2a_b200 needs a CUDA device (sm_100a); there is no CPU fallback")
        self.device = torch.device(device) if device is not None else torch.device("cuda", torch.cuda.current_device())
        self.lib = native.load()
        with torch.cuda.device(self.device):
            self.sm_count, self.cc_major, self.cc_minor = native.device_check()
        self.launches = 0
        self._status_log: List[torch.Tensor] = []
        self._dense = set()
        self.last_unverified: Optional[torch.Tensor] = None

    def _stream(self) -> int:
        return torch.cuda.current_stream(self.device).cuda_stream

    def to_device(self, x, dtype=None) -> torch.Tensor:
        if isinstance(x, np.ndarray):
            t = torch.from_numpy(np.ascontiguousarray(x))
        elif isinstance(x, torch.Tensor):
            t = x
        else:
            t = torch.as_tensor(np.asarray(x))
        if dtype is not None and t.dtype != dtype:
            t = t.to(dtype)
        if t.device != self.device:
            t = t.to(self.device, non_blocking=True)
        return t.contiguous()

    def _embedding(self, x) -> Tuple[torch.Tensor, int]:
        if isinstance(x, np.ndarray) and x.dtype not in (np.float32,):
            x = x.astype(np.float32)
        t = self.to_device(x)
        if t.dtype == torch.bfloat16:
            code = native.BF16
        else:
            if t.dtype != torch.float32:
                t = t.float()
            code = native.F32
        if t.dim() == 1:
            t = t.unsqueeze(0)
        return t.contiguous(), code

    def normalize_fuse(self, seg0, seg1=None, w0: float = 1.0, w1: float = 1.0, flags: int = native.NF_ROWNORM,
                       want_f32: bool = True, want_planes: bool = False, want_lo: bool = True,
                       want_inv_norm: bool = False, want_stats: bool = False,
                       col_std: Optional[torch.Tensor] = None, defer_f32: bool = False) -> Operand:
        a, code = self._embedding(seg0)
        n, d0 = a.shape
        b = None
        d1 = 0
        if seg1 is not None:
            b, code_b = self._embedding(seg1)
            if b.shape[0] != n:
                raise ValueError("normalize_fuse: segments have different row counts")
            if code_b != code:
                a, b, code = a.float(), b.float(), native.F32
            d1 = b.shape[1]
        dim = d0 + d1
        out = Operand(n=n, dim=dim)
        row_div = None
        if defer_f32:
            if not self.can_defer(a, b, flags):
                raise ValueError("normalize_fuse(defer_f32): needs segment widths / strides that are multiples of 4 and no fused standardisation")
            want_f32 = False
            row_div = torch.empty((n, 4), dtype=torch.float32, device=self.device)
            out.lazy = DeferredRows(a, b, code, float(w0), float(w1), int(flags), row_div)
        if want_f32:
            out.f32 = torch.empty((n, dim), dtype=torch.float32, device=self.device)
        ld_planes = 0
        if want_planes:
            ld_planes = _round_up(dim, 64)
            out.hi = torch.empty((n, ld_planes), dtype=torch.int16, device=self.device)
            if want_lo:
                out.lo = torch.empty((n, ld_planes), dtype=torch.int16, device=self.device)
        if want_inv_norm:
            out.inv_norm = torch.empty((n,), dtype=torch.float32, device=self.device)
        if want_stats and want_planes:
            out.stats = torch.zeros((2,), dtype=torch.float32, device=self.device)
        if n == 0:
            return out
        with torch.cuda.device(self.device):
            native.check(self.lib.emr2a_normalize_fuse(
                a.data_ptr(), native.ptr(b), n, d0, d1, _ld(a), _ld(b) if b is not None else 0,
                float(w0), float(w1), int(flags), code,
                native.ptr(out.f32), dim, native.ptr(out.hi), native.ptr(out.lo), ld_planes,
                native.ptr(out.inv_norm), native.ptr(out.stats), native.ptr(col_std), native.ptr(row_div), self._stream()))
        self.launches += 1
        return out

    @staticmethod
    def defer_default(dim: int) -> bool:
        return _DEFER_F32 and dim <= _DEFER_MAX_DIM

    @staticmethod
    def can_defer(a: torch.Tensor, b: Optional[torch.Tensor], flags: int) -> bool:
        if flags & native.NF_STANDARDIZE:
            return False
        al = 16 if a.dtype == torch.float32 else 8
        for t in (a, b):
            if t is None:
                continue
            if int(t.shape[1]) % 4 or (int(t.shape[0]) > 1 and int(t.stride(0)) % 4) or t.data_ptr() % al or t.stride(1) != 1:
                return False
        return True

    def scores(self, q: torch.Tensor, db: torch.Tensor) -> torch.Tensor:
        q = self.to_device(q, torch.float32)
        db = self.to_device(db, torch.float32)
        if q.dim() == 1:
            q = q.unsqueeze(0)
        Q, D = q.shape
        N = db.shape[0]
        if db.shape[1] != D:
            raise ValueError(f"scores: query dim {D} != database dim {db.shape[1]}")
        out = torch.empty((Q, N), dtype=torch.float32, device=self.device)
        if Q and N:
            with torch.cuda.device(self.device):
                native.check(self.lib.emr2a_scores(q.data_ptr(), db.data_ptr(), Q, N, D, _ld(q), _ld(db),
                                                   out.data_ptr(), N, self._stream()))
            self.launches += 1
        return out

    def euclid_scores(self, q: torch.Tensor, db: torch.Tensor) -> torch.Tensor:
        q = self.to_device(q, torch.float32).reshape(-1)
        db = self.to_device(db, torch.float32)
        N, D = db.shape
        out = torch.empty((N,), dtype=torch.float32, device=self.device)
        ws = torch.empty((16,), dtype=torch.uint8, device=self.device)
        if N:
            with torch.cuda.device(self.device):
                native.check(self.lib.emr2a_euclid_scores(q.data_ptr(), db.data_ptr(), N, D, _ld(db),
                                                          out.data_ptr(), ws.data_ptr(), 16, self._stream()))
            self.launches += 2
        return out

    def late_fuse_scores(self, text_scores, image_scores, w_text: float, mode: int) -> torch.Tensor:
        ts = self.to_device(text_scores, torch.float32)
        im = self.to_device(image_scores, torch.float32)
        one_d = ts.dim() == 1
        if one_d:
            ts, im = ts.unsqueeze(0), im.unsqueeze(0)
        Q, N = ts.shape
        out = torch.empty((Q, N), dtype=torch.float32, device=self.device)
        if Q and N:
            with torch.cuda.device(self.device):
                native.check(self.lib.emr2a_late_fuse_scores(ts.data_ptr(), im.data_ptr(), Q, N, _ld(ts),
                                                             float(np.float32(w_text)), float(np.float32(1 - w_text)),
                                                             mode, out.data_ptr(), N, self._stream()))
            self.launches += 1
        return out[0] if one_d else out

    def topk_from_scores(self, scores, k: int) -> torch.Tensor:
        s = self.to_device(scores, torch.float32)
        if s.dim() == 1:
            s = s.unsqueeze(0)
        Q, N = s.shape
        keys = torch.zeros((Q, k), dtype=torch.int64, device=self.device)
        if Q and N:
            with torch.cuda.device(self.device):
                native.check(self.lib.emr2a_topk_from_scores(s.data_ptr(), Q, N, _ld(s), k, keys.data_ptr(),
                                                             self._stream()))
            self.launches += 1
        return keys

    def segment_mean(self, x, offsets) -> torch.Tensor:
        x = self.to_device(x, torch.float32)
        off = self.to_device(offsets, torch.int64)
        n_seg = int(off.shape[0]) - 1
        out = torch.empty((max(n_seg, 0), x.shape[1]), dtype=torch.float32, device=self.device)
        if n_seg > 0:
            with torch.cuda.device(self.device):
                native.check(self.lib.emr2a_segment_mean(x.data_ptr(), _ld(x), off.data_ptr(), n_seg, int(x.shape[1]),
                                                         out.data_ptr(), int(x.shape[1]), self._stream()))
            self.launches += 1
        return out

    def pick_precision(self, Q: int, N: int, D: int, K: int, requested: str = "auto") -> str:
        req = os.environ.get("EMR2A_PRECISION", requested) if requested == "auto" else requested
        if req != "auto":
            if req not in _PREC:
                raise ValueError(f"unknown precision {req!r}")
            return req
        if float(Q) * float(N) * float(D) >= _TC_MIN_MACS:
            if K <= _RESCORE_MAX_K and (N, D) not in self._dense:
                return "rescore"
            if K <= 32:
                return "bf16x3"
        return "fp32"

    def prepare(self, seg0, seg1=None, w0=1.0, w1=1.0, flags=native.NF_ROWNORM, precision="fp32",
                defer_f32: bool = False) -> Operand:
        if precision == "fp32":
            return self.normalize_fuse(seg0, seg1, w0, w1, flags, want_f32=True, want_planes=False)
        if precision == "rescore":
            if defer_f32 and _DEFER_F32:
                a = self._embedding(seg0)[0]
                b = self._embedding(seg1)[0] if seg1 is not None else None
                if (b is None or a.dtype == b.dtype) and self.can_defer(a, b, flags):
                    return self.normalize_fuse(a, b, w0, w1, flags, want_planes=True, want_lo=False, want_stats=True,
                                               defer_f32=True)
            return self.normalize_fuse(seg0, seg1, w0, w1, flags, want_f32=True, want_planes=True, want_lo=False,
                                       want_stats=True)
        return self.normalize_fuse(seg0, seg1, w0, w1, flags, want_f32=False, want_planes=True,
                                   want_lo=(precision == "bf16x3"))

    def topk_search(self, q: Operand, db: Operand, k: int, precision: str = "fp32",
                    q_fold: Optional[torch.Tensor] = None, db_fold: Optional[torch.Tensor] = None,
                    fold_sorted: bool = False, idx_base: int = 0, row_ids: Optional[torch.Tensor] = None) -> torch.Tensor:
        if q.dim != db.dim:
            raise ValueError(f"topk_search: query dim {q.dim} != database dim {db.dim}")
        prec = _PREC[precision]
        Q, N, D = q.n, db.n, q.dim
        keys = torch.empty((Q, k), dtype=torch.int64, device=self.device)
        if Q == 0:
            return keys
        ws_bytes = int(self.lib.emr2a_topk_search_workspace_bytes(Q, N, D, k, prec))
        ws = torch.empty((ws_bytes + 256,), dtype=torch.uint8, device=self.device)
        ws_ptr = _round_up(ws.data_ptr(), 256)
        need_f32 = prec in (native.PREC_FP32, native.PREC_BF16_RESCORE)
        need_hi = prec != native.PREC_FP32
        lazy_arg, _lazy_keep = (None, None)
        if prec == native.PREC_BF16_RESCORE and db.f32 is None:
            lazy_arg, _lazy_keep = _lazy_arg(db)
        if need_f32 and (q.f32 is None or (db.f32 is None and lazy_arg is None)):
            raise ValueError(f"topk_search({precision}) needs fp32 operands")
        if need_hi and (q.hi is None or db.hi is None or (prec == native.PREC_BF16X3 and (q.lo is None or db.lo is None))):
            raise ValueError(f"topk_search({precision}) needs bf16 operand planes")
        status = None
        if prec == native.PREC_BF16_RESCORE:
            if q.stats is None or db.stats is None:
                raise ValueError("topk_search(rescore) needs operands prepared with stats")
            if k > _RESCORE_MAX_K:
                raise ValueError(f"topk_search(rescore): K={k} > {_RESCORE_MAX_K}")
            status = torch.zeros((4,), dtype=torch.int32, device=self.device)
            self.last_unverified = torch.empty((Q,), dtype=torch.uint8, device=self.device)
        if q_fold is not None:
            q_fold = self.to_device(q_fold, torch.uint8)
            db_fold = self.to_device(db_fold, torch.uint8)
        with torch.cuda.device(self.device):
            native.check(self.lib.emr2a_topk_search(
                native.ptr(q.f32), _ld(q.f32) if q.f32 is not None else 0,
                native.ptr(q.hi), native.ptr(q.lo), _ld(q.hi) if q.hi is not None else 0,
                native.ptr(db.f32), _ld(db.f32) if db.f32 is not None else 0,
                native.ptr(db.hi), native.ptr(db.lo), _ld(db.hi) if db.hi is not None else 0,
                Q, N, D, native.ptr(q_fold), native.ptr(db_fold), int(fold_sorted),
                int(idx_base), int(k), prec, native.ptr(q.stats), native.ptr(db.stats),
                keys.data_ptr(), native.ptr(status), native.ptr(self.last_unverified if status is not None else None),
                ws_ptr, ws_bytes, lazy_arg, self._stream()))
        self.launches += 2 if status is None else 6
        if status is not None:
            self._status_log.append(status)
        if row_ids is not None:
            row_ids = self.to_device(row_ids, torch.int32)
            if int(row_ids.shape[0]) != N:
                raise ValueError(f"topk_search: row_ids has {int(row_ids.shape[0])} entries for {N} database rows")
            with torch.cuda.device(self.device):
                native.check(self.lib.emr2a_keys_map_rows(keys.data_ptr(), Q * k, row_ids.data_ptr(), N, int(idx_base),
                                                          self._stream()))
            self.launches += 1
        return keys

    CAND_WIDTH = 64

    def topk_filter(self, q: Operand, db: Operand, k: int, q_fold=None, db_fold=None, fold_sorted: bool = False,
                    idx_base: int = 0) -> Tuple[torch.Tensor, torch.Tensor, torch.Tensor]:
        if q.hi is None or db.hi is None:
            raise ValueError("topk_filter needs bf16 operand planes")
        if k > _RESCORE_MAX_K:
            raise ValueError(f"topk_filter: K={k} > {_RESCORE_MAX_K}")
        Q, N, D = q.n, db.n, q.dim
        cand = torch.empty((Q, self.CAND_WIDTH), dtype=torch.int64, device=self.device)
        tau = torch.empty((Q,), dtype=torch.int32, device=self.device)
        kth = torch.empty((Q,), dtype=torch.float32, device=self.device)
        if Q == 0:
            return cand, tau, kth
        ws_bytes = int(self.lib.emr2a_topk_filter_workspace_bytes(Q, N, D, k))
        ws = torch.empty((ws_bytes + 256,), dtype=torch.uint8, device=self.device)
        if q_fold is not None:
            q_fold = self.to_device(q_fold, torch.uint8)
            db_fold = self.to_device(db_fold, torch.uint8)
        with torch.cuda.device(self.device):
            native.check(self.lib.emr2a_topk_filter(
                q.hi.data_ptr(), _ld(q.hi), db.hi.data_ptr() if N else None, _ld(db.hi) if N else 0, Q, N, D,
                native.ptr(q_fold), native.ptr(db_fold), int(fold_sorted), int(idx_base), int(k),
                cand.data_ptr(), tau.data_ptr(), kth.data_ptr(), _round_up(ws.data_ptr(), 256), ws_bytes, self._stream()))
        self.launches += 3
        return cand, tau, kth

    def rescore_candidates(self, cand: torch.Tensor, tau: torch.Tensor, kth_floor: Optional[torch.Tensor], q: Operand,
                           db: Operand, k: int, idx_base: int = 0) -> torch.Tensor:
        lazy_arg, _lazy_keep = _lazy_arg(db) if db.f32 is None else (None, None)
        if q.f32 is None or (db.f32 is None and lazy_arg is None and db.n) or q.stats is None or db.stats is None:
            raise ValueError("rescore_candidates needs fp32 operands prepared with stats")
        Q, N, D = q.n, db.n, q.dim
        payload = torch.zeros((Q * k + (Q + 1) // 2,), dtype=torch.int64, device=self.device)
        if Q == 0:
            return payload
        keys, bounds = self.split_payload(payload, Q, k)
        if N == 0:
            bounds.fill_(float("-inf"))
            return payload
        with torch.cuda.device(self.device):
            native.check(self.lib.emr2a_rescore_candidates(
                cand.data_ptr(), tau.data_ptr(), native.ptr(kth_floor), q.f32.data_ptr(), _ld(q.f32), native.ptr(db.f32),
                _ld(db.f32) if db.f32 is not None else 0, Q, N, D, int(idx_base), int(k), q.stats.data_ptr(),
                db.stats.data_ptr(), keys.data_ptr(), bounds.data_ptr(), lazy_arg, self._stream()))
        self.launches += 1
        return payload

    @staticmethod
    def split_payload(payload: torch.Tensor, Q: int, k: int) -> Tuple[torch.Tensor, torch.Tensor]:
        lead = payload.shape[:-1]
        keys = payload[..., :Q * k].unflatten(-1, (Q, k)) if lead else payload[:Q * k].view(Q, k)
        bounds = payload[..., Q * k:].view(torch.float32)[..., :Q]
        return keys, bounds

    def verify_merged(self, keys: torch.Tensor, all_payload: torch.Tensor, k: int) -> Tuple[torch.Tensor, torch.Tensor]:
        Q = int(keys.shape[0])
        P, width = all_payload.shape
        flags = torch.zeros((Q,), dtype=torch.uint8, device=self.device)
        status = torch.zeros((4,), dtype=torch.int32, device=self.device)
        if Q:
            bounds_ptr = all_payload.data_ptr() + 8 * Q * k
            with torch.cuda.device(self.device):
                native.check(self.lib.emr2a_verify_merged(keys.data_ptr(), int(k), Q, bounds_ptr, int(P),
                                                          int(all_payload.stride(0)) * 2, flags.data_ptr(),
                                                          status.data_ptr(), self._stream()))
            self.launches += 1
        return flags, status

    def merge_payload(self, all_payload: torch.Tensor, Q: int, k: int) -> torch.Tensor:
        P = int(all_payload.shape[0])
        out = torch.empty((Q, k), dtype=torch.int64, device=self.device)
        if Q:
            with torch.cuda.device(self.device):
                native.check(self.lib.emr2a_topk_merge(all_payload.data_ptr(), P, Q, k, int(all_payload.stride(0)), k, k,
                                                       out.data_ptr(), self._stream()))
            self.launches += 1
        return out

    def exact_rescan(self, q: Operand, db: Operand, flag_list: torch.Tensor, k: int, idx_base: int = 0, q_fold=None,
                     db_fold=None, seed_keys: Optional[torch.Tensor] = None) -> torch.Tensor:
        flag_list = self.to_device(flag_list, torch.int32)
        n = int(flag_list.shape[0])
        out = torch.zeros((n, k), dtype=torch.int64, device=self.device)
        if n == 0:
            return out
        lazy_arg, _lazy_keep = _lazy_arg(db) if (db.f32 is None and db.n) else (None, None)
        if q.f32 is None or (db.n and db.f32 is None and lazy_arg is None):
            raise ValueError("exact_rescan needs fp32 operands")
        ws_bytes = int(self.lib.emr2a_exact_rescan_workspace_bytes(n, k))
        ws = torch.empty((ws_bytes + 256,), dtype=torch.uint8, device=self.device)
        if q_fold is not None:
            q_fold = self.to_device(q_fold, torch.uint8)
            db_fold = self.to_device(db_fold, torch.uint8)
        filtered = seed_keys is not None and db.hi is not None and q.stats is not None and db.stats is not None
        if seed_keys is not None:
            seed_keys = seed_keys.contiguous()
            if tuple(seed_keys.shape) != (n, k):
                raise ValueError(f"exact_rescan: seed_keys must be [{n}, {k}]")
        with torch.cuda.device(self.device):
            native.check(self.lib.emr2a_exact_rescan(
                q.f32.data_ptr(), _ld(q.f32), native.ptr(db.f32) if db.n else q.f32.data_ptr(),
                (_ld(db.f32) if db.f32 is not None else 0) if db.n else q.dim,
                db.n, q.dim, int(idx_base), int(k), native.ptr(q_fold), native.ptr(db_fold), flag_list.data_ptr(), n,
                out.data_ptr(), _round_up(ws.data_ptr(), 256), ws_bytes, lazy_arg,
                native.ptr(db.hi) if (filtered and db.n) else None, _ld(db.hi) if (filtered and db.n) else 0,
                native.ptr(q.stats) if filtered else None, native.ptr(db.stats) if filtered else None,
# ... 5 lines not shown
        if not self._status_log:
            return None
        st = torch.stack(self._status_log)
        self._status_log = []
        return torch.stack([st[:, 0].sum(), st[:, 1].max(), st[:, 2].max(), st[:, 3].max()]).to(torch.int32)

    @staticmethod
    def check_deferred(statuses: Sequence[torch.Tensor]) -> Tuple[int, bool]:
        if not statuses:
            return 0, False
        st = torch.stack(list(statuses)).cpu().numpy()
        return int(st[:, 0].sum()), bool(st[:, 1].any())

    def consume_status(self) -> Tuple[int, bool]:
        if not self._status_log:
            return 0, False
        st = torch.stack(self._status_log).cpu().numpy()
        self._status_log = []
        return int(st[:, 0].sum()), bool(st[:, 1].any())

    def topk_merge(self, parts: torch.Tensor, k_out: int) -> torch.Tensor:
        P, Q, K_in = parts.shape
        parts = parts.contiguous()
        out = torch.empty((Q, k_out), dtype=torch.int64, device=self.device)
        if Q:
            with torch.cuda.device(self.device):
                native.check(self.lib.emr2a_topk_merge(parts.data_ptr(), P, Q, K_in, Q * K_in, K_in, k_out,
                                                       out.data_ptr(), self._stream()))
            self.launches += 1
        return out

    def vote_metrics(self, keys: torch.Tensor, db_labels, q_labels, n_classes: int,
                     k_list: Sequence[int] = (1, 3, 5), wacc_f32: bool = False,
                     q_group: Optional[torch.Tensor] = None, n_groups: int = 1, label_base: int = 0,
                     per_query: bool = True, want_lists: bool = True) -> Dict[str, torch.Tensor]:
        Q, K = keys.shape
        db_labels = self.to_device(db_labels, torch.int32)
        q_labels = self.to_device(q_labels, torch.int32)
        if q_group is not None:
            q_group = self.to_device(q_group, torch.uint8)
        nk = len(k_list)
        dev = self.device
        nk_alloc = max(nk, 1)
        counters = torch.zeros((n_groups * (nk_alloc + 3 + 1 + 2 * n_classes * n_classes),), dtype=torch.int64, device=dev)
        o = 0
        hit = counters[o:o + n_groups * nk_alloc]; o += n_groups * nk_alloc
        votes = counters[o:o + n_groups * 3]; o += n_groups * 3
        sizes = counters[o:o + n_groups]; o += n_groups
        conf = counters[o:]
        res: Dict[str, torch.Tensor] = {}
        if want_lists:
            res["top_idx"] = torch.empty((Q, K), dtype=torch.int64, device=dev)
            res["top_scores"] = torch.empty((Q, K), dtype=torch.float32, device=dev)
            res["top_labels"] = torch.empty((Q, K), dtype=torch.int32, device=dev)
        if per_query:
            for name in ("pred_top1", "pred_vote", "pred_weighted"):
                res[name] = torch.empty((Q,), dtype=torch.int32, device=dev)
        kl = (C.c_int32 * max(nk, 1))(*[int(k) for k in k_list])
        if Q:
            with torch.cuda.device(dev):
                native.check(self.lib.emr2a_vote_metrics(
                    keys.data_ptr(), Q, K, db_labels.data_ptr(), int(label_base), q_labels.data_ptr(),
                    native.ptr(q_group), n_groups, n_classes, kl, nk, int(wacc_f32),
                    native.ptr(res.get("top_idx")), native.ptr(res.get("top_scores")), native.ptr(res.get("top_labels")),
                    native.ptr(res.get("pred_top1")), native.ptr(res.get("pred_vote")), native.ptr(res.get("pred_weighted")),
                    hit.data_ptr(), votes.data_ptr(), conf.data_ptr(), sizes.data_ptr(), self._stream()))
            self.launches += 1
        res["hit_counts"] = hit.view(n_groups, nk_alloc)[:, :nk]
        res["vote_counts"] = votes.view(n_groups, 3)
        res["group_sizes"] = sizes
        res["confusion"] = conf.view(n_groups, 2, n_classes, n_classes)
        return res

    def search_and_vote(self, db_segs: Sequence, q_segs: Sequence, db_labels, q_labels, n_classes: int, k: int,
                        db_weights=(1.0, 1.0), q_weights=(1.0, 1.0), db_flags: int = native.NF_ROWNORM,
                        q_flags: int = native.NF_ROWNORM, k_list: Sequence[int] = (1, 3, 5),
                        precision: str = "auto", wacc_f32: bool = False, q_fold=None, db_fold=None,
                        q_group=None, n_groups: int = 1, want_lists: bool = True) -> Dict[str, torch.Tensor]:
        n_db = int(db_segs[0].shape[0])
        n_q = int(q_segs[0].shape[0])
        dim = sum(int(s.shape[1]) for s in db_segs if s is not None)
        prec = self.pick_precision(n_q, n_db, dim, k, precision)
        db = self.prepare(db_segs[0], db_segs[1] if len(db_segs) > 1 else None, db_weights[0], db_weights[1], db_flags, prec,
                          defer_f32=self.defer_default(dim))
        qs = self.prepare(q_segs[0], q_segs[1] if len(q_segs) > 1 else None, q_weights[0], q_weights[1], q_flags, prec)
        keys = self.topk_search(qs, db, k, prec, q_fold=q_fold, db_fold=db_fold)
        res = self.vote_metrics(keys, db_labels, q_labels, n_classes, k_list=k_list, wacc_f32=wacc_f32,
                                q_group=q_group, n_groups=n_groups, want_lists=want_lists)
        if prec == "rescore":
            unverified, overflow = self.consume_status()
            if overflow:
                flagged = torch.nonzero(self.last_unverified).squeeze(1)
                if int(flagged.numel()) * 2 > n_q:
                    self._dense.add((n_db, dim))
                q_dev = [self._embedding(s)[0].index_select(0, flagged) for s in q_segs if s is not None]
                db3 = self.prepare(db_segs[0], db_segs[1] if len(db_segs) > 1 else None, db_weights[0], db_weights[1],
                                   db_flags, "bf16x3")
                qs3 = self.prepare(q_dev[0], q_dev[1] if len(q_dev) > 1 else None, q_weights[0], q_weights[1], q_flags,
                                   "bf16x3")
                qf = self.to_device(q_fold, torch.uint8).index_select(0, flagged) if q_fold is not None else None
                keys3 = self.topk_search(qs3, db3, k, "bf16x3", q_fold=qf, db_fold=db_fold)
                keys.index_copy_(0, flagged, keys3)
                res = self.vote_metrics(keys, db_labels, q_labels, n_classes, k_list=k_list, wacc_f32=wacc_f32,
                                        q_group=q_group, n_groups=n_groups, want_lists=want_lists)
                res["precision"] = "rescore+bf16x3"
                res["unverified"] = int(flagged.numel())
                res["keys"] = keys
                return res
            res["unverified"] = unverified
        res["keys"] = keys
        res["precision"] = prec
        return res


    def build_index(self, db_segs: Sequence, db_labels, n_classes: int, flags: int = native.NF_ROWNORM,
                    weights=(1.0, 1.0), precision: str = "auto", expected_queries: int = 4096, k: int = 10) -> "DatabaseIndex":
        n_db = int(db_segs[0].shape[0])
        dim = sum(int(s.shape[1]) for s in db_segs if s is not None)
        prec = self.pick_precision(expected_queries, n_db, dim, k, precision)
        op = self.prepare(db_segs[0], db_segs[1] if len(db_segs) > 1 else None, weights[0], weights[1], flags, prec)
        return DatabaseIndex(self, op, self.to_device(db_labels, torch.int32), n_classes, flags, prec)

    @staticmethod
    def _rows(op: "Operand", lo: int, hi: int) -> "Operand":
        cut = lambda t: None if t is None else t[lo:hi]
        return Operand(n=hi - lo, dim=op.dim, f32=cut(op.f32), hi=cut(op.hi), lo=cut(op.lo),
                       inv_norm=cut(op.inv_norm), stats=op.stats)

    def cv_search_and_vote(self, segs: Sequence, labels, folds, n_classes: int, k: int,
                           flags: int = native.NF_ROWNORM, q_weights=(1.0, 1.0),
                           k_list: Sequence[int] = (1, 3, 5), precision: str = "auto",
                           n_folds: Optional[int] = None, q_block: int = 1 << 20,
                           want_lists: bool = True, distributed: Optional[bool] = None) -> Dict[str, torch.Tensor]:
        folds_t = self.to_device(folds, torch.uint8)
        n = int(folds_t.shape[0])
        if n_folds is None:
            n_folds = int(folds_t.max().item()) + 1 if n else 1
        labels_t = self.to_device(labels, torch.int32)
        mats = [self._embedding(x)[0] for x in segs if x is not None]
        perm = _fold_order(folds_t)
        if perm is not None:
            mats = [m.index_select(0, perm) for m in mats]
            labels_t = labels_t.index_select(0, perm)
            folds_t = folds_t.index_select(0, perm)
        dim = sum(int(m.shape[1]) for m in mats)
        prec = self.pick_precision(n, n, dim, k, precision)
        import torch.distributed as tdist
        if distributed is None:
            distributed = (os.environ.get("EMR2A_CV_DISTRIBUTED") == "1" and tdist.is_available() and tdist.is_initialized()
                           and tdist.get_world_size() > 1 and tdist.get_backend() == "nccl")
        if distributed:
            from .dist import fold_balanced_ranges, ranges_to_rows, sharded_cv_search_and_vote
            world, rank = tdist.get_world_size(), tdist.get_rank()
            sig = torch.stack([torch.tensor(float(n), device=self.device, dtype=torch.float64),
                               folds_t.double().sum(), (labels_t.double() * (torch.arange(n, device=self.device) % 8191 + 1)).sum()])
            lo_sig, hi_sig = sig.clone(), sig.clone()
            tdist.all_reduce(lo_sig, op=tdist.ReduceOp.MIN)
            tdist.all_reduce(hi_sig, op=tdist.ReduceOp.MAX)
            if not torch.equal(lo_sig, hi_sig):
                raise ValueError("cv_search_and_vote(distributed=True): the ranks were called with different cohorts "
                                 "(row count / fold / label checksums differ); every rank must pass the same arrays")
            counts = torch.bincount(folds_t.long(), minlength=n_folds).cpu().tolist()
            rows = ranges_to_rows(fold_balanced_ranges(counts, rank, world), self.device)
            res = sharded_cv_search_and_vote(self, [m.index_select(0, rows.long()) for m in mats], labels_t, folds_t,
                                             n_classes, k, 0, flags, q_weights, k_list, prec, n_folds,
                                             min(q_block, 1 << 18), True, want_lists, None, rows)
            return self._cv_unpermute(res, perm, want_lists)
# ... 418 lines not shown
```

### emr2a_b200/native.py

```python
from __future__ import annotations

import ctypes as C
import os
from typing import Optional

PKG = os.path.dirname(os.path.abspath(__file__))
LIB_PATH = os.path.join(PKG, "libemr2a.so")

OK, ERR_INVALID, ERR_CUDA, ERR_UNSUPPORTED, ERR_WORKSPACE = 0, 1, 2, 3, 4
F32, BF16 = 0, 1
NF_SEGNORM, NF_ROWNORM, NF_ZERO_GUARD, NF_STANDARDIZE = 1, 2, 4, 8
PREC_FP32, PREC_BF16X3, PREC_BF16X1, PREC_BF16_RESCORE = 0, 1, 2, 3
SCORE_NONE, SCORE_ZSCORE, SCORE_MINMAX = 0, 1, 2
ABI_VERSION = 12

_p = C.c_void_p
_i64 = C.c_int64
_int = C.c_int
_f = C.c_float
_sz = C.c_size_t

_SIGNATURES = {
    "emr2a_abi_version": (_int, []),
    "emr2a_last_error": (C.c_char_p, []),
    "emr2a_device_check": (_int, [C.POINTER(_int), C.POINTER(_int), C.POINTER(_int)]),
    "emr2a_normalize_fuse": (_int, [_p, _p, _i64, _int, _int, _i64, _i64, _f, _f, _int, _int,
                                    _p, _i64, _p, _p, _i64, _p, _p, _p, _p, _p]),
    "emr2a_scores": (_int, [_p, _p, _i64, _i64, _int, _i64, _i64, _p, _i64, _p]),
    "emr2a_euclid_workspace_bytes": (_sz, [_i64]),
    "emr2a_euclid_scores": (_int, [_p, _p, _i64, _int, _i64, _p, _p, _sz, _p]),
    "emr2a_late_fuse_scores": (_int, [_p, _p, _i64, _i64, _i64, _f, _f, _int, _p, _i64, _p]),
    "emr2a_topk_search_workspace_bytes": (_sz, [_i64, _i64, _int, _int, _int]),
    "emr2a_topk_search": (_int, [_p, _i64, _p, _p, _i64, _p, _i64, _p, _p, _i64, _i64, _i64, _int, _p, _p, _int,
                                 _i64, _int, _int, _p, _p, _p, _p, _p, _p, _sz, _p, _p]),
    "emr2a_topk_filter_workspace_bytes": (_sz, [_i64, _i64, _int, _int]),
    "emr2a_topk_filter": (_int, [_p, _i64, _p, _i64, _i64, _i64, _int, _p, _p, _int, _i64, _int, _p, _p, _p, _p, _sz, _p]),
    "emr2a_rescore_candidates": (_int, [_p, _p, _p, _p, _i64, _p, _i64, _i64, _i64, _int, _i64, _int, _p, _p, _p, _p, _p, _p]),
    "emr2a_verify_merged": (_int, [_p, _int, _i64, _p, _int, _i64, _p, _p, _p]),
    "emr2a_exact_rescan_workspace_bytes": (_sz, [_int, _int]),
    "emr2a_exact_rescan": (_int, [_p, _i64, _p, _i64, _i64, _int, _i64, _int, _p, _p, _p, _int, _p, _p, _sz, _p,
                                  _p, _i64, _p, _p, _p, _p]),
    "emr2a_range_search_workspace_bytes": (_sz, [_i64, _i64, _int]),
    "emr2a_range_search": (_int, [_p, _i64, _p, _i64, _p, _i64, _p, _i64, _i64, _i64, _int, _p, _p, _int, _i64, _f, _p, _p,
                                  _p, _i64, _p, _i64, _p, _p, _sz, _p, _p]),
    "emr2a_topk_merge": (_int, [_p, _int, _i64, _int, _i64, _i64, _int, _p, _p]),
    "emr2a_keys_map_rows": (_int, [_p, _i64, _p, _i64, _i64, _p]),
    "emr2a_vote_metrics": (_int, [_p, _i64, _int, _p, _i64, _p, _p, _int, _int, C.POINTER(C.c_int32), _int, _int,
                                  _p, _p, _p, _p, _p, _p, _p, _p, _p, _p, _p]),
    "emr2a_topk_from_scores": (_int, [_p, _i64, _i64, _i64, _int, _p, _p]),
    "emr2a_column_moments_workspace_bytes": (_sz, [_i64, _int]),
    "emr2a_column_moments": (_int, [_p, _i64, _i64, _int, _p, _p, _p, _p, _sz, _p]),
    "emr2a_standardize": (_int, [_p, _i64, _i64, _int, _p, _p, _p, _i64, _p]),
    "emr2a_gram_f64_workspace_bytes": (_sz, [_i64, _int]),
    "emr2a_gram_f64": (_int, [_p, _i64, _i64, _int, _p, _p, _p, _p, _p, _sz, _p]),
    "emr2a_project": (_int, [_p, _i64, _i64, _int, _p, _p, _p, _i64, _int, _p, _p, _i64, _p]),
    "emr2a_scale_segments": (_int, [_p, _i64, _int, _int, _i64, _p, _p, _p]),
    "emr2a_keys_add_offset": (_int, [_p, _i64, _int, _p, _p]),
    "emr2a_segment_mean": (_int, [_p, _i64, _p, _i64, _int, _p, _i64, _p]),
    "emr2a_debug_topk_search_dump": (_int, [_p, _p, _p, _p, _i64, _i64, _int, _i64, _i64, _p, _p, _i64, _int, _int,
                                            _p, _p, _sz, _p, _p]),
    "emr2a_debug_unit_clocks": (_int, [_p, _i64, _p]),
    "emr2a_debug_tc_timing": (_int, [_int]),
    "emr2a_debug_tc_elapsed": (_int, [_p, _int, _p]),
}


class LazyRows(C.Structure):
    _fields_ = [("seg0", C.c_void_p), ("seg1", C.c_void_p), ("d0", C.c_int32), ("d1", C.c_int32),
                ("ld0", C.c_int64), ("ld1", C.c_int64), ("dtype", C.c_int32), ("w0", C.c_float), ("w1", C.c_float),
                ("flags", C.c_int32), ("row_div", C.c_void_p)]


def symbols():
    return sorted(_SIGNATURES)


class Emr2aError(RuntimeError):
    def __init__(self, code: int, text: str):
        super().__init__(f"libemr2a error {code}: {text}")
        self.code = code


_lib: Optional[C.CDLL] = None


def load(check_device: bool = False) -> C.CDLL:
    global _lib
    if _lib is None:
        if os.environ.get("EMR2A_NO_AUTOBUILD") != "1":
            try:
                from . import build as _build
                _build.build()
            except Exception as exc:
                if not os.path.exists(LIB_PATH):
                    raise ImportError(f"libemr2a.so is missing and could not be built: {exc}") from exc
        if not os.path.exists(LIB_PATH):
            raise ImportError(
                f"{LIB_PATH} not found: build it with `python -m emr2a_b200.build` "
                "(the EMR2A B200 path has no CPU fallback)")
        lib = C.CDLL(LIB_PATH)
        for name, (res, args) in _SIGNATURES.items():
            fn = getattr(lib, name)
            fn.restype = res
            fn.argtypes = args
        if lib.emr2a_abi_version() != ABI_VERSION:
            raise ImportError(f"libemr2a ABI {lib.emr2a_abi_version()} != binding {ABI_VERSION}; rebuild")
        _lib = lib
    if check_device:
        device_check()
    return _lib


def last_error() -> str:
    return load().emr2a_last_error().decode("utf-8", "replace")


def check(rc: int) -> None:
    if rc == OK:
        return
# ... 17 lines not shown
```

### include/emr2a.h

```cpp
#ifndef EMR2A_H
#define EMR2A_H

#include <stddef.h>
#include <stdint.h>

#ifdef __cplusplus
extern "C" {
#endif

#define EMR2A_ABI_VERSION 12

enum emr2a_status {
  EMR2A_OK = 0,
  EMR2A_ERR_INVALID = 1,
  EMR2A_ERR_CUDA = 2,
  EMR2A_ERR_UNSUPPORTED = 3,
  EMR2A_ERR_WORKSPACE = 4
};

enum emr2a_dtype { EMR2A_F32 = 0, EMR2A_BF16 = 1 };

enum emr2a_nf_flags {
  EMR2A_NF_SEGNORM = 1,
  EMR2A_NF_ROWNORM = 2,
  EMR2A_NF_ZERO_GUARD = 4,
  EMR2A_NF_STANDARDIZE = 8
};

enum emr2a_precision {
  EMR2A_PREC_FP32 = 0,
  EMR2A_PREC_BF16X3 = 1,
  EMR2A_PREC_BF16X1 = 2,
  EMR2A_PREC_BF16_RESCORE = 3
};

enum emr2a_score_mode { EMR2A_SCORE_NONE = 0, EMR2A_SCORE_ZSCORE = 1, EMR2A_SCORE_MINMAX = 2 };

int emr2a_abi_version(void);
const char* emr2a_last_error(void);

int emr2a_device_check(int* sm_count, int* cc_major, int* cc_minor);

int emr2a_normalize_fuse(const void* seg0, const void* seg1, int64_t n, int d0, int d1,
                         int64_t ld0, int64_t ld1, float w0, float w1, int flags, int in_dtype,
                         float* out_f32, int64_t ld_f32,
                         uint16_t* out_hi, uint16_t* out_lo, int64_t ld_bf16,
                         float* inv_norm_out, float* stats_out, const float* col_std,
                         float* row_div_out, void* stream);

typedef struct emr2a_lazy_rows {
  const void* seg0;
  const void* seg1;
  int32_t d0, d1;
  int64_t ld0, ld1;
  int32_t dtype;
  float w0, w1;
  int32_t flags;
  const float* row_div;
} emr2a_lazy_rows;

int emr2a_scores(const float* q, const float* db, int64_t Q, int64_t N, int D,
                 int64_t ldq, int64_t lddb, float* out, int64_t ld_out, void* stream);

size_t emr2a_euclid_workspace_bytes(int64_t N);
int emr2a_euclid_scores(const float* q, const float* db, int64_t N, int D, int64_t lddb,
                        float* out, void* workspace, size_t ws_bytes, void* stream);

int emr2a_late_fuse_scores(const float* text_scores, const float* image_scores, int64_t Q, int64_t N,
                           int64_t ld, float w_text, float one_minus_w, int mode,
                           float* out, int64_t ld_out, void* stream);

size_t emr2a_topk_search_workspace_bytes(int64_t Q, int64_t N, int D, int K, int precision);
int emr2a_topk_search(const float* q_f32, int64_t ldq_f32,
                      const uint16_t* q_hi, const uint16_t* q_lo, int64_t ldq_bf16,
                      const float* db_f32, int64_t lddb_f32,
                      const uint16_t* db_hi, const uint16_t* db_lo, int64_t lddb_bf16,
                      int64_t Q, int64_t N, int D,
                      const uint8_t* q_fold, const uint8_t* db_fold, int fold_sorted,
                      int64_t idx_base, int K, int precision,
                      const float* q_stats, const float* db_stats,
                      uint64_t* out_keys, int32_t* status_out, uint8_t* unverified_out,
                      void* workspace, size_t ws_bytes, const emr2a_lazy_rows* db_lazy, void* stream);

size_t emr2a_topk_filter_workspace_bytes(int64_t Q, int64_t N, int D, int K);
int emr2a_topk_filter(const uint16_t* q_hi, int64_t ldq_bf16, const uint16_t* db_hi, int64_t lddb_bf16,
                      int64_t Q, int64_t N, int D,
                      const uint8_t* q_fold, const uint8_t* db_fold, int fold_sorted,
                      int64_t idx_base, int K,
                      uint64_t* cand_out, uint32_t* tau_out, float* kth_out,
                      void* workspace, size_t ws_bytes, void* stream);
int emr2a_rescore_candidates(const uint64_t* cand, const uint32_t* tau, const float* kth_floor,
                             const float* q_f32, int64_t ldq_f32, const float* db_f32, int64_t lddb_f32,
                             int64_t Q, int64_t N, int D, int64_t idx_base, int K,
                             const float* q_stats, const float* db_stats,
                             uint64_t* out_keys, float* bound_out, const emr2a_lazy_rows* db_lazy, void* stream);
int emr2a_verify_merged(const uint64_t* keys, int K, int64_t Q, const float* bounds, int parts,
                        int64_t bounds_stride, uint8_t* flags_out, int32_t* status_out, void* stream);
size_t emr2a_exact_rescan_workspace_bytes(int n_flagged, int K);
int emr2a_exact_rescan(const float* q_f32, int64_t ldq_f32, const float* db_f32, int64_t lddb_f32,
                       int64_t N, int D, int64_t idx_base, int K,
                       const uint8_t* q_fold, const uint8_t* db_fold,
                       const int32_t* flag_list, int n_flagged,
                       uint64_t* out_keys, void* workspace, size_t ws_bytes,
                       const emr2a_lazy_rows* db_lazy,
                       const uint16_t* db_hi, int64_t lddb_bf16, const float* q_stats, const float* db_stats,
                       const uint64_t* seed_keys, void* stream);

size_t emr2a_range_search_workspace_bytes(int64_t Q, int64_t N, int D);
int emr2a_range_search(const float* q_f32, int64_t ldq_f32, const uint16_t* q_hi, int64_t ldq_bf16,
                       const float* db_f32, int64_t lddb_f32, const uint16_t* db_hi, int64_t lddb_bf16,
                       int64_t Q, int64_t N, int D,
                       const uint8_t* q_fold, const uint8_t* db_fold, int fold_sorted, int64_t idx_base,
                       float min_score, const float* q_stats, const float* db_stats,
                       uint64_t* cand, int64_t cand_cap, uint64_t* results, int64_t result_cap,
                       uint64_t* counts_out, void* workspace, size_t ws_bytes,
                       const emr2a_lazy_rows* db_lazy, void* stream);

int emr2a_topk_merge(const uint64_t* keys_in, int parts, int64_t Q, int K_in,
                     int64_t part_stride, int64_t q_stride, int K_out,
                     uint64_t* keys_out, void* stream);

int emr2a_keys_map_rows(uint64_t* keys, int64_t n_keys, const uint32_t* row_ids, int64_t n_rows,
                        int64_t idx_base, void* stream);

int emr2a_vote_metrics(const uint64_t* keys, int64_t Q, int K,
                       const int32_t* db_labels, int64_t label_base,
                       const int32_t* q_labels, const uint8_t* q_group, int n_groups, int C,
                       const int32_t* k_list_host, int nk, int wacc_f32,
                       int64_t* top_idx, float* top_scores, int32_t* top_labels,
                       int32_t* pred_top1, int32_t* pred_vote, int32_t* pred_weighted,
                       unsigned long long* hit_counts, unsigned long long* vote_counts,
                       unsigned long long* confusion, unsigned long long* group_sizes,
                       void* stream);

int emr2a_segment_mean(const float* x, int64_t ld, const int64_t* offsets, int64_t n_segments, int D,
                       float* out, int64_t ld_out, void* stream);

size_t emr2a_gram_f64_workspace_bytes(int64_t n, int D);
int emr2a_gram_f64(const float* x, int64_t ld, int64_t n, int D, const float* mean, const float* scale,
                   double* gram, double* zsum, void* workspace, size_t ws_bytes, void* stream);
int emr2a_project(const float* x, int64_t ld, int64_t n, int D, const float* mean, const float* scale,
                  const float* w, int64_t ldw, int P, const float* bias, float* out, int64_t ld_out, void* stream);
size_t emr2a_column_moments_workspace_bytes(int64_t n, int D);
int emr2a_column_moments(const float* x, int64_t ld, int64_t n, int D, const float* shift,
                         double* sum, double* sumsq, void* workspace, size_t ws_bytes, void* stream);
int emr2a_standardize(const float* x, int64_t ld, int64_t n, int D, const float* mean, const float* scale,
                      float* out, int64_t ld_out, void* stream);

int emr2a_scale_segments(float* x, int64_t n, int d0, int d1, int64_t ld, const float* g0, const float* g1,
                         void* stream);
int emr2a_keys_add_offset(uint64_t* keys, int64_t Q, int K, const float* offset, void* stream);

int emr2a_topk_from_scores(const float* scores, int64_t Q, int64_t N, int64_t ld, int K,
                           uint64_t* out_keys, void* stream);

#ifdef __cplusplus
}
#endif
#endif
```

Before: 623,700.

## Fuse database normalization and bf16 conversion into the CTA-pair filter kernel

Adds prepare_topk_search/filter entry points that pass raw database rows into the tensor-core filter. CTAs claim row blocks through workspace counters, normalize them and write the bf16 plane and stats on the fly, so no separate preparation pass runs before the search. This is meant to remove one kernel launch and one full read/write pass over the database. In exchange it adds cross-CTA claim/ready synchronization and only works for aligned layouts and Q > 128.

```diff
diff --git a/emr2a_b200/csrc/api.cu b/emr2a_b200/csrc/api.cu
--- a/emr2a_b200/csrc/api.cu
+++ b/emr2a_b200/csrc/api.cu
@@ -1,4 +1,4 @@
-#include "common.cuh"
+#include "nf_row.cuh"
 
 #include <math.h>
 #include <stdlib.h>
@@ -42,8 +42,9 @@
                    int64_t Q, int64_t N, int D, int64_t ldq, int64_t lddb, const uint8_t* q_fold,
                    const uint8_t* db_fold, int64_t idx_base, int K, int passes, uint64_t* out_keys,
                    void* workspace, size_t ws_bytes, float* debug_scores, cudaStream_t st, TcPartials* partials,
-                   int fold_sorted, int min_splits);
+                   int fold_sorted, int min_splits, const DbPrep* prep = nullptr);
 int tc_planned_splits(int64_t Q, int64_t N, int min_splits);
+bool tc_uses_cta_pairs(int64_t Q);
 int tc_timing_enable(int on);
 int tc_timing_read(float* ms_out, int cap, int* n_out);
 void tc_timing_record(int which, cudaStream_t st);
@@ -122,7 +123,7 @@
                                 int64_t N, int D, const uint8_t* q_fold, const uint8_t* db_fold, int fold_sorted,
                                 int64_t idx_base, int K, uint64_t* approx, void* tc_ws, size_t tc_ws_bytes,
                                 float* debug_scores, cudaStream_t st, const uint64_t** cand, int* kpm,
-                                const uint32_t** tau) {
+                                const uint32_t** tau, const DbPrep* prep = nullptr) {
   TcPartials parts{};
   const int planned = tc_planned_splits(Q, N, 2);
   int kp = planned > 128 ? 8 : ((planned >= 8 || K <= 5) ? 16 : RESCORE_KP);
@@ -132,7 +133,7 @@
     if (v == 8 || v == 16 || v == 32) kp = v;
   }
   int rc = tc_topk_search(q_hi, nullptr, db_hi, nullptr, Q, N, D, ldq_bf16, lddb_bf16, q_fold, db_fold, idx_base,
-                          kp, 1, nullptr, tc_ws, tc_ws_bytes, debug_scores, st, &parts, fold_sorted, 2);
+                          kp, 1, nullptr, tc_ws, tc_ws_bytes, debug_scores, st, &parts, fold_sorted, 2, prep);
   if (rc != EMR2A_OK) return rc;
   *kpm = kp;
   *cand = parts.parts;
@@ -152,7 +153,7 @@
                             const uint8_t* q_fold, const uint8_t* db_fold, int fold_sorted, int64_t idx_base, int K,
                             int precision, const float* q_stats, const float* db_stats, uint64_t* out_keys,
                             int32_t* status, uint8_t* qflags, void* workspace, size_t ws_bytes, float* debug_scores,
-                            const emr2a_lazy_rows* db_lazy, void* stream) {
+                            const emr2a_lazy_rows* db_lazy, void* stream, const DbPrep* prep = nullptr) {
   if (Q < 0 || N < 0 || D <= 0 || K <= 0 || !out_keys) return fail(EMR2A_ERR_INVALID, "topk_search: bad arguments (Q=%lld N=%lld D=%d K=%d)", (long long)Q, (long long)N, D, K);
   if ((q_fold == nullptr) != (db_fold == nullptr)) return fail(EMR2A_ERR_INVALID, "topk_search: q_fold and db_fold must be given together");
   if (idx_base < 0) return fail(EMR2A_ERR_INVALID, "topk_search: negative idx_base");
@@ -187,7 +188,8 @@
       const uint32_t* tau = nullptr;
       int kpm = 0;
       int rc = rescore_filter_stage(q_hi, ldq_bf16, db_hi, lddb_bf16, Q, N, D, q_fold, db_fold, fold_sorted, idx_base, K,
-                                    reinterpret_cast<uint64_t*>(ws), ws + a_bytes, t_bytes, debug_scores, st, &cand, &kpm, &tau);
+                                    reinterpret_cast<uint64_t*>(ws), ws + a_bytes, t_bytes, debug_scores, st, &cand, &kpm, &tau,
+                                    prep);
       if (rc != EMR2A_OK) return rc;
       return rescore_pipeline(cand, kpm, tau, q_f32, ldq_f32, db_f32, lddb_f32, db_lazy, db_hi, lddb_bf16, Q, N, D, idx_base, K, q_stats,
                               db_stats, q_fold, db_fold, out_keys, status, qflags, ws + a_bytes + t_bytes, r_bytes, st);
@@ -232,10 +234,10 @@
   return align256(tc_topk_workspace_bytes(Q, N, RESCORE_KP, D));
 }
 
-extern "C" int emr2a_topk_filter(const uint16_t* q_hi, int64_t ldq_bf16, const uint16_t* db_hi, int64_t lddb_bf16, int64_t Q,
-                                 int64_t N, int D, const uint8_t* q_fold, const uint8_t* db_fold, int fold_sorted,
-                                 int64_t idx_base, int K, uint64_t* cand_out, uint32_t* tau_out, float* kth_out,
-                                 void* workspace, size_t ws_bytes, void* stream) {
+static int topk_filter_impl(const uint16_t* q_hi, int64_t ldq_bf16, const uint16_t* db_hi, int64_t lddb_bf16, int64_t Q,
+                            int64_t N, int D, const uint8_t* q_fold, const uint8_t* db_fold, int fold_sorted,
+                            int64_t idx_base, int K, uint64_t* cand_out, uint32_t* tau_out, float* kth_out,
+                            void* workspace, size_t ws_bytes, void* stream, const DbPrep* prep) {
   if (Q < 0 || N < 0 || D <= 0 || K <= 0 || !cand_out || !tau_out) return fail(EMR2A_ERR_INVALID, "topk_filter: bad arguments");
   if (K > 10) return fail(EMR2A_ERR_UNSUPPORTED, "topk_filter: K=%d > 10 (use EMR2A_PREC_BF16X3)", K);
   if ((q_fold == nullptr) != (db_fold == nullptr)) return fail(EMR2A_ERR_INVALID, "topk_filter: q_fold and db_fold must be given together");
@@ -252,7 +254,7 @@
     const uint32_t* tau = nullptr;
     int kpm = 0;
     int rc = rescore_filter_stage(q_hi, ldq_bf16, db_hi, lddb_bf16, Q, N, D, q_fold, db_fold, fold_sorted, idx_base, K,
-                                  cand_out, workspace, ws_bytes, nullptr, st, &cand, &kpm, &tau);
+                                  cand_out, workspace, ws_bytes, nullptr, st, &cand, &kpm, &tau, prep);
     if (rc != EMR2A_OK) return rc;
     if (cand != cand_out) {
       rc = emr2a_topk_merge(cand, 1, Q, kpm, Q * kpm, kpm, RESCORE_KPM, cand_out, st);
@@ -262,6 +264,14 @@
   }
   if (kth_out) return rescore_kth_scores(cand_out, RESCORE_KPM, K, Q, kth_out, st);
   return EMR2A_OK;
+}
+
+extern "C" int emr2a_topk_filter(const uint16_t* q_hi, int64_t ldq_bf16, const uint16_t* db_hi, int64_t lddb_bf16, int64_t Q,
+                                 int64_t N, int D, const uint8_t* q_fold, const uint8_t* db_fold, int fold_sorted,
+                                 int64_t idx_base, int K, uint64_t* cand_out, uint32_t* tau_out, float* kth_out,
+                                 void* workspace, size_t ws_bytes, void* stream) {
+  return topk_filter_impl(q_hi, ldq_bf16, db_hi, lddb_bf16, Q, N, D, q_fold, db_fold, fold_sorted, idx_base, K, cand_out,
+                          tau_out, kth_out, workspace, ws_bytes, stream, nullptr);
 }
 
 extern "C" int emr2a_rescore_candidates(const uint64_t* cand, const uint32_t* tau, const float* kth_floor, const float* q_f32,
@@ -307,6 +317,89 @@
   }
   return rescore_exact_rescan(q_f32, ldq_f32, db_f32, lddb_f32, db_lazy, N, D, idx_base, K, q_fold, db_fold, flag_list,
                               n_flagged, out_keys, workspace, ws_bytes, db_hi, lddb_bf16, q_stats, db_stats, seed_keys, st);
+}
+
+static size_t prep_counter_bytes(int64_t N) { return align256(sizeof(uint32_t) * static_cast<size_t>((N + 255) / 256 + 2)); }
+
+static int prep_setup(const char* who, const emr2a_lazy_rows* db, uint16_t* db_hi, int64_t lddb_bf16, float* db_stats,
+                      int64_t Q, int64_t N, int D, void* workspace, cudaStream_t st, DbPrep* out) {
+  if (!db || !db_hi || !db_stats || !db->seg0 || !db->row_div || (db->d1 > 0 && !db->seg1))
+    return fail(EMR2A_ERR_INVALID, "%s: db_raw (with seg0 and row_div), db_hi and db_stats are required", who);
+  if (db->d0 <= 0 || db->d1 < 0 || db->d0 + db->d1 != D)
+    return fail(EMR2A_ERR_INVALID, "%s: raw segment widths %d + %d != D = %d", who, db->d0, db->d1, D);
+  if (db->dtype != EMR2A_F32 && db->dtype != EMR2A_BF16) return fail(EMR2A_ERR_INVALID, "%s: unknown dtype %d", who, db->dtype);
+  if (db->flags & EMR2A_NF_STANDARDIZE) return fail(EMR2A_ERR_UNSUPPORTED, "%s: no fused standardisation", who);
+  if (db->ld0 < db->d0 || (db->d1 > 0 && db->ld1 < db->d1))
+    return fail(EMR2A_ERR_INVALID, "%s: leading dimension smaller than row", who);
+  const size_t in_align = db->dtype == EMR2A_F32 ? 16 : 8;
+  auto aligned = [](const void* q, size_t a) { return (reinterpret_cast<uintptr_t>(q) % a) == 0; };
+  const int64_t Dp = (static_cast<int64_t>(D) + 63) / 64 * 64;
+  if ((db->d0 % 4) || (db->d1 % 4) || (db->ld0 % 4) || (db->d1 > 0 && db->ld1 % 4) || !aligned(db->seg0, in_align) ||
+      (db->d1 > 0 && !aligned(db->seg1, in_align)) || !aligned(db->row_div, 16) || !aligned(db_hi, 16) ||
+      lddb_bf16 < Dp || (lddb_bf16 % 8) || lddb_bf16 > 2048)
+    return fail(EMR2A_ERR_UNSUPPORTED, "%s: the filter prepares aligned rows of up to 2048 plane columns (segment widths "
+                                       "and leading dimensions multiples of 4, lddb_bf16 >= round_up(D, 64), %% 8)", who);
+  if (!tc_uses_cta_pairs(Q))
+    return fail(EMR2A_ERR_UNSUPPORTED, "%s: the database is prepared inside the CTA-pair filter, which runs for Q > 128", who);
+  if (!workspace || (reinterpret_cast<uintptr_t>(workspace) & 255)) return fail(EMR2A_ERR_INVALID, "%s: workspace must be 256-byte aligned", who);
+  NfParams& nf = out->nf;
+  nf = NfParams{db->seg0, db->seg1, N, db->d0, db->d1, db->ld0, db->d1 > 0 ? db->ld1 : 0, db->w0, db->w1, db->flags,
+                nullptr, 0, db_hi, nullptr, lddb_bf16, nullptr, db_stats, nullptr, const_cast<float*>(db->row_div)};
+  out->in_bf16 = db->dtype == EMR2A_BF16;
+  out->wide = lddb_bf16 > 1024;
+  out->claim = static_cast<uint32_t*>(workspace);
+  out->done = out->claim + 1;
+  out->ready = out->claim + 2;
+  EMR2A_CUDA_TRY(cudaMemsetAsync(workspace, 0, prep_counter_bytes(N), st));
+  EMR2A_CUDA_TRY(cudaMemsetAsync(db_stats, 0, 2 * sizeof(float), st));
+  return EMR2A_OK;
+}
+
+extern "C" size_t emr2a_prepare_topk_search_workspace_bytes(int64_t Q, int64_t N, int D, int K) {
+  return prep_counter_bytes(N > 0 ? N : 0) + emr2a_topk_search_workspace_bytes(Q, N, D, K, EMR2A_PREC_BF16_RESCORE);
+}
+
+extern "C" int emr2a_prepare_topk_search(const emr2a_lazy_rows* db_raw, uint16_t* db_hi, int64_t lddb_bf16, float* db_stats,
+                                         const float* q_f32, int64_t ldq_f32, const uint16_t* q_hi, int64_t ldq_bf16,
+                                         const float* q_stats, int64_t Q, int64_t N, int D, const uint8_t* q_fold,
+                                         const uint8_t* db_fold, int fold_sorted, int64_t idx_base, int K,
+                                         uint64_t* out_keys, int32_t* status_out, uint8_t* unverified_out,
+                                         void* workspace, size_t ws_bytes, void* stream) {
+  if (Q <= 0 || N <= 0 || D <= 0 || K <= 0 || !out_keys)
+    return fail(EMR2A_ERR_INVALID, "prepare_topk_search: bad arguments (Q=%lld N=%lld D=%d K=%d)", (long long)Q, (long long)N, D, K);
+  if (K > 10) return fail(EMR2A_ERR_UNSUPPORTED, "prepare_topk_search: K=%d > 10", K);
+  cudaStream_t st = static_cast<cudaStream_t>(stream);
+  const size_t pb = prep_counter_bytes(N);
+  if (ws_bytes < pb) return fail(EMR2A_ERR_WORKSPACE, "prepare_topk_search: workspace %zu < %zu", ws_bytes, pb);
+  DbPrep prep{};
+  int rc = prep_setup("prepare_topk_search", db_raw, db_hi, lddb_bf16, db_stats, Q, N, D, workspace, st, &prep);
+  if (rc != EMR2A_OK) return rc;
+
+  return topk_search_impl(q_f32, ldq_f32, q_hi, nullptr, ldq_bf16, nullptr, 0, db_hi, nullptr, lddb_bf16, Q, N, D, q_fold,
+                          db_fold, fold_sorted, idx_base, K, EMR2A_PREC_BF16_RESCORE, q_stats, db_stats, out_keys,
+                          status_out, unverified_out, static_cast<uint8_t*>(workspace) + pb, ws_bytes - pb, nullptr, db_raw,
+                          stream, &prep);
+}
+
+extern "C" size_t emr2a_prepare_topk_filter_workspace_bytes(int64_t Q, int64_t N, int D, int K) {
+  return prep_counter_bytes(N > 0 ? N : 0) + emr2a_topk_filter_workspace_bytes(Q, N, D, K);
+}
+
+extern "C" int emr2a_prepare_topk_filter(const emr2a_lazy_rows* db_raw, uint16_t* db_hi, int64_t lddb_bf16, float* db_stats,
+                                         const uint16_t* q_hi, int64_t ldq_bf16, int64_t Q, int64_t N, int D,
+                                         const uint8_t* q_fold, const uint8_t* db_fold, int fold_sorted, int64_t idx_base,
+                                         int K, uint64_t* cand_out, uint32_t* tau_out, float* kth_out, void* workspace,
+                                         size_t ws_bytes, void* stream) {
+  if (Q <= 0 || N <= 0 || D <= 0 || K <= 0)
+    return fail(EMR2A_ERR_INVALID, "prepare_topk_filter: bad arguments (Q=%lld N=%lld D=%d K=%d)", (long long)Q, (long long)N, D, K);
+  cudaStream_t st = static_cast<cudaStream_t>(stream);
+  const size_t pb = prep_counter_bytes(N);
+  if (ws_bytes < pb) return fail(EMR2A_ERR_WORKSPACE, "prepare_topk_filter: workspace %zu < %zu", ws_bytes, pb);
+  DbPrep prep{};
+  int rc = prep_setup("prepare_topk_filter", db_raw, db_hi, lddb_bf16, db_stats, Q, N, D, workspace, st, &prep);
+  if (rc != EMR2A_OK) return rc;
+  return topk_filter_impl(q_hi, ldq_bf16, db_hi, lddb_bf16, Q, N, D, q_fold, db_fold, fold_sorted, idx_base, K, cand_out,
+                          tau_out, kth_out, static_cast<uint8_t*>(workspace) + pb, ws_bytes - pb, stream, &prep);
 }
 
 extern "C" size_t emr2a_range_search_workspace_bytes(int64_t Q, int64_t N, int D) {
diff --git a/emr2a_b200/csrc/nf_row.cuh b/emr2a_b200/csrc/nf_row.cuh
--- /dev/null
+++ b/emr2a_b200/csrc/nf_row.cuh
@@ -0,0 +1,197 @@
+#pragma once
+#include "row_math.cuh"
+
+namespace emr2a {
+
+struct NfParams {
+  const void* seg0;
+  const void* seg1;
+  int64_t n;
+  int d0, d1;
+  int64_t ld0, ld1;
+  float w0, w1;
+  int flags;
+  float* out_f32;
+  int64_t ld_f32;
+  uint16_t* out_hi;
+  uint16_t* out_lo;
+  int64_t ld_bf16;
+  float* inv_norm;
+  float* stats;
+  const float* col_std;
+  float* row_div;
+};
+
+__device__ __forceinline__ void stats_flush(float* stats, float max_norm2, float max_res2) {
+  unsigned int* u = reinterpret_cast<unsigned int*>(stats);
+  atomicMax(u, __float_as_uint(__fsqrt_ru(max_norm2)));
+  atomicMax(u + 1, __float_as_uint(__fsqrt_ru(max_res2)));
+}
+
+__device__ __forceinline__ uint64_t l2_evict_first_policy() {
+  uint64_t pol;
+  asm volatile("createpolicy.fractional.L2::evict_first.b64 %0, 1.0;" : "=l"(pol));
+  return pol;
+}
+template <typename InT> struct LoaderEF;
+template <> struct LoaderEF<float> {
+  static __device__ __forceinline__ float4 load4(const void* base, int64_t elem, uint64_t pol) {
+    float4 r;
+    asm volatile("ld.global.nc.L1::no_allocate.L2::cache_hint.v4.f32 {%0,%1,%2,%3}, [%4], %5;"
+                 : "=f"(r.x), "=f"(r.y), "=f"(r.z), "=f"(r.w)
+                 : "l"(static_cast<const float*>(base) + elem), "l"(pol));
+    return r;
+  }
+};
+template <> struct LoaderEF<__nv_bfloat16> {
+  static __device__ __forceinline__ float4 load4(const void* base, int64_t elem, uint64_t pol) {
+    uint2 r;
+    asm volatile("ld.global.nc.L1::no_allocate.L2::cache_hint.v2.u32 {%0,%1}, [%2], %3;"
+                 : "=r"(r.x), "=r"(r.y) : "l"(static_cast<const uint16_t*>(base) + elem), "l"(pol));
+    return Loader<__nv_bfloat16>::widen(r);
+  }
+};
+
+template <typename InT, int MAXC, bool EVICT_FIRST = false>
+__device__ __forceinline__ void load_row(const NfParams& p, int64_t row, int lane, int c0, int ctot, float4 (&v)[MAXC],
+                                         uint64_t pol = 0) {
+#pragma unroll
+  for (int j = 0; j < MAXC; ++j) {
+    const int c = lane + 32 * j;
+    if (EVICT_FIRST) {
+      if (c < c0) v[j] = LoaderEF<InT>::load4(p.seg0, row * p.ld0 + 4 * c, pol);
+      else if (c < ctot) v[j] = LoaderEF<InT>::load4(p.seg1, row * p.ld1 + 4 * (c - c0), pol);
+      else v[j] = make_float4(0.f, 0.f, 0.f, 0.f);
+    } else {
+      if (c < c0) v[j] = Loader<InT>::load4(p.seg0, row * p.ld0 + 4 * c);
+      else if (c < ctot) v[j] = Loader<InT>::load4(p.seg1, row * p.ld1 + 4 * (c - c0));
+      else v[j] = make_float4(0.f, 0.f, 0.f, 0.f);
+    }
+  }
+}
+
+__device__ __forceinline__ float std1(float x, float m, float s, float r) {
+  const float t = __fsub_rn(x, m);
+  const float q0 = t * r;
+  const float rem = fmaf(-q0, s, t);
+  return fmaf(rem, r, q0);
+}
+__device__ __forceinline__ void standardize4(float4& v, const float* __restrict__ col_std, int dtot, int col) {
+  const float4 m = __ldg(reinterpret_cast<const float4*>(col_std + col));
+  const float4 s = __ldg(reinterpret_cast<const float4*>(col_std + dtot + col));
+  const float4 r = __ldg(reinterpret_cast<const float4*>(col_std + 2 * dtot + col));
+  v.x = std1(v.x, m.x, s.x, r.x); v.y = std1(v.y, m.y, s.y, r.y);
+  v.z = std1(v.z, m.z, s.z, r.z); v.w = std1(v.w, m.w, s.w, r.w);
+}
+
+template <int MAXC, bool WANT_LO, bool STATS, bool STD, bool ST_POLICY = false>
+__device__ __forceinline__ void nf_row(const NfParams& p, int64_t row, int lane, int c0, int ctot, int cpad,
+                                       float4 (&v)[MAXC], float& max_n2, float& max_r2, uint64_t st_pol = 0) {
+  if (STD) {
+#pragma unroll
+    for (int j = 0; j < MAXC; ++j) {
+      const int c = lane + 32 * j;
+      if (c < ctot) standardize4(v[j], p.col_std, p.d0 + p.d1, 4 * c);
+    }
+  }
+  float ss0 = 0.f, ss1 = 0.f;
+  float4 divs = make_float4(1.f, 1.f, 1.f, 0.f);
+  if (p.flags & EMR2A_NF_SEGNORM) {
+#pragma unroll
+    for (int j = 0; j < MAXC; ++j) {
+      const int c = lane + 32 * j;
+      if (c < c0) ss0 += sq4(v[j]); else ss1 += sq4(v[j]);
+    }
+  }
+  if (p.flags & EMR2A_NF_SEGNORM) {
+    const RowDiv n0 = row_div(__fsqrt_rn(warp_sum(ss0)) + EMR2A_EPS);
+    const RowDiv n1 = row_div(__fsqrt_rn(warp_sum(ss1)) + EMR2A_EPS);
+    divs.x = n0.d; divs.y = n1.d;
+#pragma unroll
+    for (int j = 0; j < MAXC; ++j) {
+      const int c = lane + 32 * j;
+      if (c < c0) div4(v[j], n0); else if (c < ctot) div4(v[j], n1);
+    }
+  }
+  if (p.w0 != 1.0f || p.w1 != 1.0f) {
+#pragma unroll
+    for (int j = 0; j < MAXC; ++j) {
+      const int c = lane + 32 * j;
+      if (c < c0) mul4(v[j], p.w0); else if (c < ctot) mul4(v[j], p.w1);
+    }
+  }
+  float inv = 1.0f;
+  if (p.flags & (EMR2A_NF_ROWNORM | EMR2A_NF_ZERO_GUARD)) {
+    float ss = 0.f;
+#pragma unroll
+    for (int j = 0; j < MAXC; ++j) ss += sq4(v[j]);
+    float nrm = __fsqrt_rn(warp_sum(ss));
+    const bool guard = (p.flags & EMR2A_NF_ZERO_GUARD) != 0;
+    if (!guard) nrm += EMR2A_EPS;
+    if (!(guard && nrm == 0.f)) {
+      const RowDiv dv = row_div(nrm);
+#pragma unroll
+      for (int j = 0; j < MAXC; ++j) div4(v[j], dv);
+      inv = dv.r;
+      divs.z = nrm; divs.w = 1.f;
+    }
+  }
+  if (p.inv_norm && lane == 0) p.inv_norm[row] = inv;
+  if (p.row_div && lane == 0) reinterpret_cast<float4*>(p.row_div)[row] = divs;
+  if (p.out_f32) {
+#pragma unroll
+    for (int j = 0; j < MAXC; ++j) {
+      const int c = lane + 32 * j;
+      if (c < ctot) *reinterpret_cast<float4*>(p.out_f32 + row * p.ld_f32 + 4 * c) = v[j];
+    }
+  }
+  if (p.out_hi) {
+    float n2 = 0.f, r2 = 0.f;
+#pragma unroll
+    for (int j = 0; j < MAXC; ++j) {
+      const int c = lane + 32 * j;
+      if (c < cpad) {
+        const __nv_bfloat162 h01 = __floats2bfloat162_rn(v[j].x, v[j].y);
+        const __nv_bfloat162 h23 = __floats2bfloat162_rn(v[j].z, v[j].w);
+        const uint32_t u01 = *reinterpret_cast<const uint32_t*>(&h01);
+        const uint32_t u23 = *reinterpret_cast<const uint32_t*>(&h23);
+        if (ST_POLICY)
+          asm volatile("st.global.L2::cache_hint.v2.u32 [%0], {%1,%2}, %3;"
+                       ::"l"(p.out_hi + row * p.ld_bf16 + 4 * c), "r"(u01), "r"(u23), "l"(st_pol) : "memory");
+        else
+          *reinterpret_cast<uint2*>(p.out_hi + row * p.ld_bf16 + 4 * c) = make_uint2(u01, u23);
+        if (WANT_LO || STATS) {
+          const float e0 = v[j].x - __uint_as_float(u01 << 16);
+          const float e1 = v[j].y - __uint_as_float(u01 & 0xFFFF0000u);
+          const float e2 = v[j].z - __uint_as_float(u23 << 16);
+          const float e3 = v[j].w - __uint_as_float(u23 & 0xFFFF0000u);
+          if (STATS) {
+            n2 += sq4(v[j]);
+            r2 += e0 * e0 + e1 * e1 + e2 * e2 + e3 * e3;
+          }
+          if (WANT_LO) {
+            const __nv_bfloat162 l01 = __floats2bfloat162_rn(e0, e1);
+            const __nv_bfloat162 l23 = __floats2bfloat162_rn(e2, e3);
+            *reinterpret_cast<uint2*>(p.out_lo + row * p.ld_bf16 + 4 * c) =
+                make_uint2(*reinterpret_cast<const uint32_t*>(&l01), *reinterpret_cast<const uint32_t*>(&l23));
+          }
+        }
+      }
+    }
+    if (STATS) {
+      max_n2 = fmaxf(max_n2, warp_sum(n2));
+      max_r2 = fmaxf(max_r2, warp_sum(r2));
+    }
+  }
+}
+
+struct DbPrep {
+  NfParams nf;
+  bool in_bf16;
+  uint32_t* claim;
+  uint32_t* ready;
+  uint32_t* done;
+  bool wide;
+};
+
+}
diff --git a/emr2a_b200/csrc/normalize_fuse.cu b/emr2a_b200/csrc/normalize_fuse.cu
--- a/emr2a_b200/csrc/normalize_fuse.cu
+++ b/emr2a_b200/csrc/normalize_fuse.cu
@@ -1,57 +1,7 @@
 #include <type_traits>
-#include "row_math.cuh"
+#include "nf_row.cuh"
 
 namespace emr2a {
-
-struct NfParams {
-  const void* seg0;
-  const void* seg1;
-  int64_t n;
-  int d0, d1;
-  int64_t ld0, ld1;
-  float w0, w1;
-  int flags;
-  float* out_f32;
-  int64_t ld_f32;
-  uint16_t* out_hi;
-  uint16_t* out_lo;
-  int64_t ld_bf16;
-  float* inv_norm;
-  float* stats;
-  const float* col_std;
-  float* row_div;
-};
-
-__device__ __forceinline__ void stats_flush(float* stats, float max_norm2, float max_res2) {
-  unsigned int* u = reinterpret_cast<unsigned int*>(stats);
-  atomicMax(u, __float_as_uint(__fsqrt_ru(max_norm2)));
-  atomicMax(u + 1, __float_as_uint(__fsqrt_ru(max_res2)));
-}
-
-template <typename InT, int MAXC>
-__device__ __forceinline__ void load_row(const NfParams& p, int64_t row, int lane, int c0, int ctot, float4 (&v)[MAXC]) {
-#pragma unroll
-  for (int j = 0; j < MAXC; ++j) {
-    const int c = lane + 32 * j;
-    if (c < c0) v[j] = Loader<InT>::load4(p.seg0, row * p.ld0 + 4 * c);
-    else if (c < ctot) v[j] = Loader<InT>::load4(p.seg1, row * p.ld1 + 4 * (c - c0));
-    else v[j] = make_float4(0.f, 0.f, 0.f, 0.f);
-  }
-}
-
-__device__ __forceinline__ float std1(float x, float m, float s, float r) {
-  const float t = __fsub_rn(x, m);
-  const float q0 = t * r;
-  const float rem = fmaf(-q0, s, t);
-  return fmaf(rem, r, q0);
-}
-__device__ __forceinline__ void standardize4(float4& v, const float* __restrict__ col_std, int dtot, int col) {
-  const float4 m = __ldg(reinterpret_cast<const float4*>(col_std + col));
-  const float4 s = __ldg(reinterpret_cast<const float4*>(col_std + dtot + col));
-  const float4 r = __ldg(reinterpret_cast<const float4*>(col_std + 2 * dtot + col));
-  v.x = std1(v.x, m.x, s.x, r.x); v.y = std1(v.y, m.y, s.y, r.y);
-  v.z = std1(v.z, m.z, s.z, r.z); v.w = std1(v.w, m.w, s.w, r.w);
-}
 
 template <typename InT, int MAXC, bool WANT_LO, bool STATS, bool STD = false>
 __global__ void __launch_bounds__(256, (MAXC <= 8 ? 2 : 1)) normalize_fuse_vec_kernel(const NfParams p) {
@@ -76,98 +26,7 @@
     } else {
       load_row<InT, MAXC>(p, row, lane, c0, ctot, v);
     }
-    if (STD) {
-#pragma unroll
-      for (int j = 0; j < MAXC; ++j) {
-        const int c = lane + 32 * j;
-        if (c < ctot) standardize4(v[j], p.col_std, p.d0 + p.d1, 4 * c);
-      }
-    }
-    float ss0 = 0.f, ss1 = 0.f;
-    float4 divs = make_float4(1.f, 1.f, 1.f, 0.f);
-    if (p.flags & EMR2A_NF_SEGNORM) {
-#pragma unroll
-      for (int j = 0; j < MAXC; ++j) {
-        const int c = lane + 32 * j;
-        if (c < c0) ss0 += sq4(v[j]); else ss1 += sq4(v[j]);
-      }
-    }
-    if (p.flags & EMR2A_NF_SEGNORM) {
-      const RowDiv n0 = row_div(__fsqrt_rn(warp_sum(ss0)) + EMR2A_EPS);
-      const RowDiv n1 = row_div(__fsqrt_rn(warp_sum(ss1)) + EMR2A_EPS);
-      divs.x = n0.d; divs.y = n1.d;
-#pragma unroll
-      for (int j = 0; j < MAXC; ++j) {
-        const int c = lane + 32 * j;
-        if (c < c0) div4(v[j], n0); else if (c < ctot) div4(v[j], n1);
-      }
-    }
-    if (p.w0 != 1.0f || p.w1 != 1.0f) {
-#pragma unroll
-      for (int j = 0; j < MAXC; ++j) {
-        const int c = lane + 32 * j;
-        if (c < c0) mul4(v[j], p.w0); else if (c < ctot) mul4(v[j], p.w1);
-      }
-    }
-    float inv = 1.0f;
-    if (p.flags & (EMR2A_NF_ROWNORM | EMR2A_NF_ZERO_GUARD)) {
-      float ss = 0.f;
-#pragma unroll
-      for (int j = 0; j < MAXC; ++j) ss += sq4(v[j]);
-      float nrm = __fsqrt_rn(warp_sum(ss));
-      const bool guard = (p.flags & EMR2A_NF_ZERO_GUARD) != 0;
-      if (!guard) nrm += EMR2A_EPS;
-      if (!(guard && nrm == 0.f)) {
-        const RowDiv dv = row_div(nrm);
-#pragma unroll
-        for (int j = 0; j < MAXC; ++j) div4(v[j], dv);
-        inv = dv.r;
-        divs.z = nrm; divs.w = 1.f;
-      }
-    }
-    if (p.inv_norm && lane == 0) p.inv_norm[row] = inv;
-    if (p.row_div && lane == 0) reinterpret_cast<float4*>(p.row_div)[row] = divs;
-    if (p.out_f32) {
-#pragma unroll
-      for (int j = 0; j < MAXC; ++j) {
-        const int c = lane + 32 * j;
-        if (c < ctot) *reinterpret_cast<float4*>(p.out_f32 + row * p.ld_f32 + 4 * c) = v[j];
-      }
-    }
-    if (p.out_hi) {
-      float n2 = 0.f, r2 = 0.f;
-#pragma unroll
-      for (int j = 0; j < MAXC; ++j) {
-        const int c = lane + 32 * j;
-        if (c < cpad) {
-          const __nv_bfloat162 h01 = __floats2bfloat162_rn(v[j].x, v[j].y);
-          const __nv_bfloat162 h23 = __floats2bfloat162_rn(v[j].z, v[j].w);
-          const uint32_t u01 = *reinterpret_cast<const uint32_t*>(&h01);
-          const uint32_t u23 = *reinterpret_cast<const uint32_t*>(&h23);
-          *reinterpret_cast<uint2*>(p.out_hi + row * p.ld_bf16 + 4 * c) = make_uint2(u01, u23);
-          if (WANT_LO || STATS) {
-            const float e0 = v[j].x - __uint_as_float(u01 << 16);
-            const float e1 = v[j].y - __uint_as_float(u01 & 0xFFFF0000u);
-            const float e2 = v[j].z - __uint_as_float(u23 << 16);
-            const float e3 = v[j].w - __uint_as_float(u23 & 0xFFFF0000u);
-            if (STATS) {
-              n2 += sq4(v[j]);
-              r2 += e0 * e0 + e1 * e1 + e2 * e2 + e3 * e3;
-            }
-            if (WANT_LO) {
-              const __nv_bfloat162 l01 = __floats2bfloat162_rn(e0, e1);
-              const __nv_bfloat162 l23 = __floats2bfloat162_rn(e2, e3);
-              *reinterpret_cast<uint2*>(p.out_lo + row * p.ld_bf16 + 4 * c) =
-                  make_uint2(*reinterpret_cast<const uint32_t*>(&l01), *reinterpret_cast<const uint32_t*>(&l23));
-            }
-          }
-        }
-      }
-      if (STATS) {
-        max_n2 = fmaxf(max_n2, warp_sum(n2));
-        max_r2 = fmaxf(max_r2, warp_sum(r2));
-      }
-    }
+    nf_row<MAXC, WANT_LO, STATS, STD>(p, row, lane, c0, ctot, cpad, v, max_n2, max_r2);
   }
   if (STATS && lane == 0 && warp0 < p.n) stats_flush(p.stats, max_n2, max_r2);
 }
diff --git a/emr2a_b200/csrc/tc_common.cuh b/emr2a_b200/csrc/tc_common.cuh
--- a/emr2a_b200/csrc/tc_common.cuh
+++ b/emr2a_b200/csrc/tc_common.cuh
@@ -1,6 +1,6 @@
 #pragma once
 #include <cuda.h>
-#include "common.cuh"
+#include "nf_row.cuh"
 
 namespace emr2a {
 
@@ -38,6 +38,11 @@
   ulonglong2* range_out;
   int64_t range_cap;
   unsigned long long* range_count;
+  NfParams nf;
+  uint32_t* prep_claim;
+  uint32_t* prep_ready;
+  uint32_t* prep_done;
+  int xmask, xst;
 };
 
 __device__ __forceinline__ uint32_t smem_u32(const void* p) { return static_cast<uint32_t>(__cvta_generic_to_shared(p)); }
@@ -283,6 +288,31 @@
   size = static_cast<int>(c1 - c0);
   slot = g * p.splits + split + step;
 }
+constexpr int PREP_PIECE_ROWS = 16;
+constexpr int PREP_PIECES = T_BN / PREP_PIECE_ROWS;
+
+__host__ __device__ __forceinline__ int64_t prep_claim_tile(int64_t pos, int64_t splits, int64_t tps, int64_t n_tiles,
+                                                            int64_t mg_eff, int64_t n_pairs) {
+  const int64_t s0 = pos / tps;
+  const int64_t v = s0 * mg_eff / n_pairs;
+  const int64_t s_lo = (v * n_pairs + mg_eff - 1) / mg_eff;
+  int64_t s_hi = ((v + 1) * n_pairs + mg_eff - 1) / mg_eff;
+  if (s_hi > splits) s_hi = splits;
+  const int64_t k = s_hi - s_lo;
+  int64_t r = pos - s_lo * tps;
+  const int64_t last = n_tiles - (splits - 1) * tps;
+  int64_t o, s;
+  if (s_hi == splits && last < tps && r >= k * last) {
+    r -= k * last;
+    o = last + r / (k - 1);
+    s = s_lo + r % (k - 1);
+  } else {
+    o = r / k;
+    s = s_lo + r % k;
+  }
+  return s * tps + o;
+}
+
 __device__ __forceinline__ void cohort_sync(const TcParams& p, int64_t slot, int point, int size) {
   uint32_t* ctr = p.sync_ctr + slot * p.sync_points + point;
   const uint32_t seen = atomicAdd(ctr, 1u) + 1u;
diff --git a/emr2a_b200/csrc/topk_tc.cu b/emr2a_b200/csrc/topk_tc.cu
--- a/emr2a_b200/csrc/topk_tc.cu
+++ b/emr2a_b200/csrc/topk_tc.cu
@@ -221,6 +221,8 @@
 
 int tc2_dispatch(int passes, int kcap, bool has_fold, const CUtensorMap& a, const CUtensorMap& b, const CUtensorMap& c,
                  const CUtensorMap& d, const TcParams& p, int grid, cudaStream_t st);
+int tc2_prep_dispatch(int kcap, bool has_fold, bool in_bf16, bool wide, const CUtensorMap& a, const CUtensorMap& c,
+                      const TcParams& p, int grid, cudaStream_t st);
 
 static bool use_cta_pairs(int64_t Q) {
   static int v = -1;
@@ -295,6 +297,8 @@
   return pl;
 }
 
+bool tc_uses_cta_pairs(int64_t Q) { return use_cta_pairs(Q); }
+
 int tc_planned_splits(int64_t Q, int64_t N, int min_splits) {
   return tc_plan(Q, N, 1, false, use_cta_pairs(Q), min_splits).splits;
 }
@@ -391,7 +395,7 @@
                    int64_t Q, int64_t N, int D, int64_t ldq, int64_t lddb,
                    const uint8_t* q_fold, const uint8_t* db_fold, int64_t idx_base, int K, int passes,
                    uint64_t* out_keys, void* workspace, size_t ws_bytes, float* debug_scores, cudaStream_t st,
-                   TcPartials* partials, int fold_sorted, int min_splits) {
+                   TcPartials* partials, int fold_sorted, int min_splits, const DbPrep* prep) {
   if (K > 32) return fail(EMR2A_ERR_UNSUPPORTED, "topk_search(bf16): K=%d > 32 (use EMR2A_PREC_FP32)", K);
   const int64_t Dp = (static_cast<int64_t>(D) + T_BK - 1) / T_BK * T_BK;
   {
@@ -400,6 +404,9 @@
   }
   const bool has_fold = q_fold != nullptr;
   const bool pairs = use_cta_pairs(Q);
+  if (prep && (!pairs || passes != 1))
+    return fail(EMR2A_ERR_UNSUPPORTED, "topk_search(bf16): the database is prepared inside the CTA-pair 1-pass filter only "
+                                       "(Q=%lld > 128 queries)", (long long)Q);
   TcPlan pl = tc_plan(Q, N, K, has_fold, pairs, min_splits, lddb > ldq ? lddb : ldq, passes == 3 ? 2 : 1);
   const size_t keys_off = 0;
   const size_t fold_off = (pl.keys_bytes + 255) & ~static_cast<size_t>(255);
@@ -451,8 +458,14 @@
     p.q_fold = q_fold; p.db_fold = fpad; p.fold_sorted = fold_sorted;
   }
   const int kcap = K <= 8 ? 8 : (K <= 16 ? 16 : 32);
+  if (prep) {
+    p.nf = prep->nf; p.prep_claim = prep->claim; p.prep_ready = prep->ready; p.prep_done = prep->done;
+    p.xmask = env_int("EMR2A_PREP_XMASK", 0xF0C); p.xst = env_int("EMR2A_PREP_XST", 0);
+  }
   tc_ev_record(0, st);
-  if (pairs) {
+  if (prep) {
+    rc = tc2_prep_dispatch(kcap, has_fold, prep->in_bf16, prep->wide, mq_hi, md_hi, p, pl.grid, st);
+  } else if (pairs) {
     rc = tc2_dispatch(passes, kcap, has_fold, mq_hi, mq_lo, md_hi, md_lo, p, pl.grid, st);
   } else if (passes == 3) {
     if (kcap == 8) rc = tc_launch_fold<3, 8>(has_fold, mq_hi, mq_lo, md_hi, md_lo, p, pl.grid, st);
diff --git a/emr2a_b200/csrc/topk_tc2.cu b/emr2a_b200/csrc/topk_tc2.cu
--- a/emr2a_b200/csrc/topk_tc2.cu
+++ b/emr2a_b200/csrc/topk_tc2.cu
@@ -41,8 +41,70 @@
       "}\n" ::"r"(tmem_d), "l"(desc_a), "l"(desc_b), "r"(idesc), "r"(accumulate) : "memory");
 }
 
-template <int PASSES, int KCAP, bool HAS_FOLD, bool RANGE = false>
-__global__ void __cluster_dims__(2, 1, 1) __launch_bounds__(T_THREADS, 1)
+constexpr int T2_PREP_THREADS = 384;
+
+template <typename InT, int MAXC>
+__device__ __forceinline__ void prep_worker(const TcParams& p, int lane, int64_t n_pairs) {
+  const NfParams& nf = p.nf;
+  const int c0 = nf.d0 >> 2;
+  const int ctot = (nf.d0 + nf.d1) >> 2;
+  const int cpad = static_cast<int>(nf.ld_bf16 >> 2);
+  const int64_t mg_eff = p.mg < p.m_tiles ? p.mg : p.m_tiles;
+  const uint32_t n_claims = static_cast<uint32_t>(p.n_tiles) * PREP_PIECES;
+  const uint64_t pol = l2_evict_first_policy();
+  float max_n2 = 0.f, max_r2 = 0.f;
+  for (;;) {
+    uint32_t c = 0;
+    if (lane == 0) c = atomicAdd(p.prep_claim, 1u);
+    c = __shfl_sync(0xffffffffu, c, 0);
+    if (c >= n_claims) break;
+    const int64_t t = prep_claim_tile(c / PREP_PIECES, p.splits, p.tiles_per_split, p.n_tiles, mg_eff, n_pairs);
+    const int64_t r0 = t * T_BN + static_cast<int64_t>(c % PREP_PIECES) * PREP_PIECE_ROWS;
+    const int64_t r1 = (r0 + PREP_PIECE_ROWS < nf.n) ? r0 + PREP_PIECE_ROWS : nf.n;
+    constexpr bool PREFETCH = MAXC <= 8;
+    float4 nxt[PREFETCH ? MAXC : 1];
+    if (PREFETCH && r0 < r1) load_row<InT, MAXC, true>(nf, r0, lane, c0, ctot, reinterpret_cast<float4 (&)[MAXC]>(nxt), pol);
+    for (int64_t row = r0; row < r1; ++row) {
+      float4 v[MAXC];
+      if (PREFETCH) {
+#pragma unroll
+        for (int j = 0; j < MAXC; ++j) v[j] = nxt[PREFETCH ? j : 0];
+        if (row + 1 < r1) load_row<InT, MAXC, true>(nf, row + 1, lane, c0, ctot, reinterpret_cast<float4 (&)[MAXC]>(nxt), pol);
+      } else {
+        load_row<InT, MAXC, true>(nf, row, lane, c0, ctot, v, pol);
+      }
+      if (p.xst) nf_row<MAXC, false, true, false, true>(nf, row, lane, c0, ctot, cpad, v, max_n2, max_r2, pol);
+      else nf_row<MAXC, false, true, false>(nf, row, lane, c0, ctot, cpad, v, max_n2, max_r2);
+    }
+    asm volatile("fence.proxy.async.global;" ::: "memory");
+    __syncwarp();
+    if (lane == 0) {
+      asm volatile("red.release.gpu.global.add.u32 [%0], 1;" ::"l"(p.prep_ready + t) : "memory");
+      asm volatile("red.release.gpu.global.add.u32 [%0], 1;" ::"l"(p.prep_done) : "memory");
+    }
+  }
+  if (lane == 0) stats_flush(nf.stats, max_n2, max_r2);
+}
+
+__device__ __forceinline__ void prep_acquire_tile(const TcParams& p, int64_t t, bool& all_ready) {
+  if (all_ready) return;
+  uint32_t v;
+  asm volatile("ld.acquire.gpu.global.u32 %0, [%1];" : "=r"(v) : "l"(p.prep_done) : "memory");
+  if (v >= static_cast<uint32_t>(p.n_tiles) * PREP_PIECES) {
+    all_ready = true;
+  } else {
+    const uint32_t* flag = p.prep_ready + t;
+    for (;;) {
+      asm volatile("ld.acquire.gpu.global.u32 %0, [%1];" : "=r"(v) : "l"(flag) : "memory");
+      if (v >= static_cast<uint32_t>(PREP_PIECES)) break;
+      __nanosleep(64);
+    }
+  }
+  asm volatile("fence.proxy.async.global;" ::: "memory");
+}
+
+template <int PASSES, int KCAP, bool HAS_FOLD, bool RANGE = false, int PREP = 0>
+__global__ void __cluster_dims__(2, 1, 1) __launch_bounds__(PREP != 0 ? T2_PREP_THREADS : T_THREADS, 1)
 tc2_topk_kernel(const __grid_constant__ CUtensorMap tm_q_hi, const __grid_constant__ CUtensorMap tm_q_lo,
                 const __grid_constant__ CUtensorMap tm_db_hi, const __grid_constant__ CUtensorMap tm_db_lo,
                 const TcParams p) {
@@ -89,6 +151,7 @@
   if (warp == 0) {
     if (lane == 0) {
       int stage = 0; uint32_t phase = 0;
+      bool prep_all_ready = false;
       for (int64_t u = pair; u < n_units; u += n_pairs) {
         int64_t split, mt;
         unit_coords(p, u, split, mt);
@@ -107,6 +170,7 @@
             p.unit_clock[2 * u] = now;
           }
           if (HAS_FOLD && tile_skipped(p, ufold, t)) continue;
+          if constexpr (PREP != 0) prep_acquire_tile(p, t, prep_all_ready);
           const int n0 = static_cast<int>(t * T_BN + rank * 128);
           for (int kc = 0; kc < p.k_chunks; ++kc) {
             mbar_wait(smem_u32(&bar_empty[stage]), phase ^ 1u);
@@ -166,7 +230,13 @@
         }
       }
     }
-  } else if (warp >= 4) {
+  } else if (warp < 4 || warp >= 8) {
+    if (!((p.xmask >> warp) & 1)) {} else
+    if constexpr (PREP == 1) prep_worker<float, 8>(p, lane, n_pairs);
+    if constexpr (PREP == 2) prep_worker<__nv_bfloat16, 8>(p, lane, n_pairs);
+    if constexpr (PREP == 3) prep_worker<float, 16>(p, lane, n_pairs);
+    if constexpr (PREP == 4) prep_worker<__nv_bfloat16, 16>(p, lane, n_pairs);
+  } else {
     const int quarter = warp & 3;
     const int row = quarter * 32 + lane;
     int acc = 0; uint32_t acc_phase = 0;
@@ -224,15 +294,15 @@
   }
 }
 
-template <int PASSES, int KCAP, bool HAS_FOLD, bool RANGE = false>
+template <int PASSES, int KCAP, bool HAS_FOLD, bool RANGE = false, int PREP = 0>
 static int tc2_launch(const CUtensorMap& mq_hi, const CUtensorMap& mq_lo, const CUtensorMap& md_hi, const CUtensorMap& md_lo,
                       const TcParams& p, int grid, cudaStream_t st) {
   constexpr int PLANES = PASSES == 3 ? 2 : 1;
   constexpr int STAGES = PASSES == 3 ? 3 : 6;
   const size_t smem = static_cast<size_t>(STAGES) * PLANES * (T_A_BYTES + T2_BH_BYTES) + 1024;
-  auto kern = tc2_topk_kernel<PASSES, KCAP, HAS_FOLD, RANGE>;
+  auto kern = tc2_topk_kernel<PASSES, KCAP, HAS_FOLD, RANGE, PREP>;
   EMR2A_CUDA_TRY(cudaFuncSetAttribute(kern, cudaFuncAttributeMaxDynamicSharedMemorySize, static_cast<int>(smem)));
-  kern<<<grid, T_THREADS, smem, st>>>(mq_hi, mq_lo, md_hi, md_lo, p);
+  kern<<<grid, PREP != 0 ? T2_PREP_THREADS : T_THREADS, smem, st>>>(mq_hi, mq_lo, md_hi, md_lo, p);
   EMR2A_LAUNCH_CHECK("tc2_topk_kernel");
   return EMR2A_OK;
 }
@@ -253,4 +323,19 @@
   return has_fold ? tc2_launch<1, 8, true, true>(a, b, c, d, p, grid, st) : tc2_launch<1, 8, false, true>(a, b, c, d, p, grid, st);
 }
 
-}
+int tc2_prep_dispatch(int kcap, bool has_fold, bool in_bf16, bool wide, const CUtensorMap& a, const CUtensorMap& c,
+                      const TcParams& p, int grid, cudaStream_t st) {
+#define EMR2A_TC2_PREP_CASE(KC, PR)                                                                                  \
+  if (kcap == KC && prep == PR)                                                                                     \
+    return has_fold ? tc2_launch<1, KC, true, false, PR>(a, a, c, c, p, grid, st)                                  \
+                    : tc2_launch<1, KC, false, false, PR>(a, a, c, c, p, grid, st);
+  const int prep = 1 + (in_bf16 ? 1 : 0) + (wide ? 2 : 0);
+  EMR2A_TC2_PREP_CASE(8, 1) EMR2A_TC2_PREP_CASE(16, 1) EMR2A_TC2_PREP_CASE(32, 1)
+  EMR2A_TC2_PREP_CASE(8, 2) EMR2A_TC2_PREP_CASE(16, 2) EMR2A_TC2_PREP_CASE(32, 2)
+  EMR2A_TC2_PREP_CASE(8, 3) EMR2A_TC2_PREP_CASE(16, 3) EMR2A_TC2_PREP_CASE(32, 3)
+  EMR2A_TC2_PREP_CASE(8, 4) EMR2A_TC2_PREP_CASE(16, 4) EMR2A_TC2_PREP_CASE(32, 4)
+#undef EMR2A_TC2_PREP_CASE
+  return fail(EMR2A_ERR_INVALID, "tc2_prep_dispatch: unsupported kcap=%d", kcap);
+}
+
+}
diff --git a/emr2a_b200/dist.py b/emr2a_b200/dist.py
--- a/emr2a_b200/dist.py
+++ b/emr2a_b200/dist.py
@@ -6,7 +6,7 @@
 import torch
 import torch.distributed as dist
 
-from .engine import Operand
+from .engine import Operand, k1_in_filter
 
 
 def shard_range(n_rows: int, rank: int, world: int, align: int = 256) -> Tuple[int, int]:
@@ -112,8 +112,11 @@
     dim = sum(int(s.shape[1]) for s in db_segs_local if s is not None)
     world = dist.get_world_size() if dist.is_initialized() else 1
     prec = eng.pick_precision(n_q, max(n_db, 1) * world, dim, k, precision)
-    db = eng.prepare(db_segs_local[0], db_segs_local[1] if len(db_segs_local) > 1 else None, 1.0, 1.0, db_flags, prec,
-                     defer_f32=eng.defer_default(dim))
+    db_seg1 = db_segs_local[1] if len(db_segs_local) > 1 else None
+    if k1_in_filter(n_q, n_db, dim, prec):
+        db = eng.prepare(db_segs_local[0], db_seg1, 1.0, 1.0, db_flags, prec, defer_f32=True, in_filter=True)
+    else:
+        db = eng.prepare(db_segs_local[0], db_seg1, 1.0, 1.0, db_flags, prec, defer_f32=eng.defer_default(dim))
     qs = eng.prepare(q_segs[0], q_segs[1] if len(q_segs) > 1 else None, q_weights[0], q_weights[1], q_flags, prec)
     if prec == "rescore" and world > 1 and cooperative and os.environ.get("EMR2A_COOP_SHARDS", "1") != "0":
         return _cooperative_search_and_vote(eng, qs, db, db_labels_global, q_labels, n_classes, k, row_offset, k_list,
diff --git a/emr2a_b200/engine.py b/emr2a_b200/engine.py
--- a/emr2a_b200/engine.py
+++ b/emr2a_b200/engine.py
@@ -35,6 +35,7 @@
     inv_norm: Optional[torch.Tensor] = None
     stats: Optional[torch.Tensor] = None
     lazy: Optional["DeferredRows"] = None
+    pending: bool = False
 
     @property
     def ld_planes(self) -> int:
@@ -63,7 +64,9 @@
                             self.w1, self.flags, self.row_div[lo:hi])
 
 
-def _lazy_arg(op: "Operand"):
+def _lazy_arg(op: "Operand", pending_ok: bool = False):
+    if op.pending and not pending_ok:
+        raise ValueError("database operand not prepared yet: its K1 runs inside the next topk_search / topk_filter")
     if op.lazy is None:
         return None, None
     st = op.lazy.struct()
@@ -72,6 +75,20 @@
 
 _DEFER_F32 = os.environ.get("EMR2A_DEFER_F32", "1") != "0"
 _DEFER_MAX_DIM = int(os.environ.get("EMR2A_DEFER_MAX_DIM", 8192))
+_FUSED_K1 = os.environ.get("EMR2A_FUSED_K1", "1") != "0"
+_FUSED_K1_MAX_LD = 2048
+
+
+def _cta_pairs(n_q: int) -> bool:
+    e = os.environ.get("EMR2A_TC2")
+    if e is None:
+        return n_q > 128
+    return not e.startswith("0")
+
+
+def k1_in_filter(n_q: int, n_db: int, dim: int, precision: str) -> bool:
+    return (_FUSED_K1 and precision == "rescore" and _DEFER_F32 and dim <= _DEFER_MAX_DIM and n_db > 0
+            and _round_up(dim, 64) <= _FUSED_K1_MAX_LD and _cta_pairs(n_q))
 
 
 class Engine:
@@ -121,7 +138,8 @@
     def normalize_fuse(self, seg0, seg1=None, w0: float = 1.0, w1: float = 1.0, flags: int = native.NF_ROWNORM,
                        want_f32: bool = True, want_planes: bool = False, want_lo: bool = True,
                        want_inv_norm: bool = False, want_stats: bool = False,
-                       col_std: Optional[torch.Tensor] = None, defer_f32: bool = False) -> Operand:
+                       col_std: Optional[torch.Tensor] = None, defer_f32: bool = False,
+                       in_filter: bool = False) -> Operand:
         a, code = self._embedding(seg0)
         n, d0 = a.shape
         b = None
@@ -156,6 +174,13 @@
             out.stats = torch.zeros((2,), dtype=torch.float32, device=self.device)
         if n == 0:
             return out
+        if in_filter:
+            if out.lazy is None or out.hi is None or out.lo is not None or out.stats is None or want_inv_norm \
+                    or col_std is not None or ld_planes > _FUSED_K1_MAX_LD:
+                raise ValueError("normalize_fuse(in_filter): needs deferred fp32 rows, the hi plane and stats only, "
+                                 f"and at most {_FUSED_K1_MAX_LD} plane columns")
+            out.pending = True
+            return out
         with torch.cuda.device(self.device):
             native.check(self.lib.emr2a_normalize_fuse(
                 a.data_ptr(), native.ptr(b), n, d0, d1, _ld(a), _ld(b) if b is not None else 0,
@@ -266,7 +291,7 @@
         return "fp32"
 
     def prepare(self, seg0, seg1=None, w0=1.0, w1=1.0, flags=native.NF_ROWNORM, precision="fp32",
-                defer_f32: bool = False) -> Operand:
+                defer_f32: bool = False, in_filter: bool = False) -> Operand:
         if precision == "fp32":
             return self.normalize_fuse(seg0, seg1, w0, w1, flags, want_f32=True, want_planes=False)
         if precision == "rescore":
@@ -275,7 +300,7 @@
                 b = self._embedding(seg1)[0] if seg1 is not None else None
                 if (b is None or a.dtype == b.dtype) and self.can_defer(a, b, flags):
                     return self.normalize_fuse(a, b, w0, w1, flags, want_planes=True, want_lo=False, want_stats=True,
-                                               defer_f32=True)
+                                               defer_f32=True, in_filter=in_filter)
             return self.normalize_fuse(seg0, seg1, w0, w1, flags, want_f32=True, want_planes=True, want_lo=False,
                                        want_stats=True)
         return self.normalize_fuse(seg0, seg1, w0, w1, flags, want_f32=False, want_planes=True,
@@ -291,14 +316,18 @@
         keys = torch.empty((Q, k), dtype=torch.int64, device=self.device)
         if Q == 0:
             return keys
-        ws_bytes = int(self.lib.emr2a_topk_search_workspace_bytes(Q, N, D, k, prec))
+        if db.pending and prec != native.PREC_BF16_RESCORE:
+            raise ValueError("topk_search: a database prepared inside the filter needs precision='rescore'")
+        ws_query = self.lib.emr2a_prepare_topk_search_workspace_bytes if db.pending else \
+            (lambda *a: self.lib.emr2a_topk_search_workspace_bytes(*a, prec))
+        ws_bytes = int(ws_query(Q, N, D, k))
         ws = torch.empty((ws_bytes + 256,), dtype=torch.uint8, device=self.device)
         ws_ptr = _round_up(ws.data_ptr(), 256)
         need_f32 = prec in (native.PREC_FP32, native.PREC_BF16_RESCORE)
         need_hi = prec != native.PREC_FP32
         lazy_arg, _lazy_keep = (None, None)
         if prec == native.PREC_BF16_RESCORE and db.f32 is None:
-            lazy_arg, _lazy_keep = _lazy_arg(db)
+            lazy_arg, _lazy_keep = _lazy_arg(db, pending_ok=True)
         if need_f32 and (q.f32 is None or (db.f32 is None and lazy_arg is None)):
             raise ValueError(f"topk_search({precision}) needs fp32 operands")
         if need_hi and (q.hi is None or db.hi is None or (prec == native.PREC_BF16X3 and (q.lo is None or db.lo is None))):
@@ -315,15 +344,23 @@
             q_fold = self.to_device(q_fold, torch.uint8)
             db_fold = self.to_device(db_fold, torch.uint8)
         with torch.cuda.device(self.device):
-            native.check(self.lib.emr2a_topk_search(
-                native.ptr(q.f32), _ld(q.f32) if q.f32 is not None else 0,
-                native.ptr(q.hi), native.ptr(q.lo), _ld(q.hi) if q.hi is not None else 0,
-                native.ptr(db.f32), _ld(db.f32) if db.f32 is not None else 0,
-                native.ptr(db.hi), native.ptr(db.lo), _ld(db.hi) if db.hi is not None else 0,
-                Q, N, D, native.ptr(q_fold), native.ptr(db_fold), int(fold_sorted),
-                int(idx_base), int(k), prec, native.ptr(q.stats), native.ptr(db.stats),
-                keys.data_ptr(), native.ptr(status), native.ptr(self.last_unverified if status is not None else None),
-                ws_ptr, ws_bytes, lazy_arg, self._stream()))
+            if db.pending:
+                native.check(self.lib.emr2a_prepare_topk_search(
+                    lazy_arg, db.hi.data_ptr(), _ld(db.hi), db.stats.data_ptr(),
+                    q.f32.data_ptr(), _ld(q.f32), q.hi.data_ptr(), _ld(q.hi), q.stats.data_ptr(),
+                    Q, N, D, native.ptr(q_fold), native.ptr(db_fold), int(fold_sorted), int(idx_base), int(k),
+                    keys.data_ptr(), status.data_ptr(), self.last_unverified.data_ptr(), ws_ptr, ws_bytes, self._stream()))
+                db.pending = False
+            else:
+                native.check(self.lib.emr2a_topk_search(
+                    native.ptr(q.f32), _ld(q.f32) if q.f32 is not None else 0,
+                    native.ptr(q.hi), native.ptr(q.lo), _ld(q.hi) if q.hi is not None else 0,
+                    native.ptr(db.f32), _ld(db.f32) if db.f32 is not None else 0,
+                    native.ptr(db.hi), native.ptr(db.lo), _ld(db.hi) if db.hi is not None else 0,
+                    Q, N, D, native.ptr(q_fold), native.ptr(db_fold), int(fold_sorted),
+                    int(idx_base), int(k), prec, native.ptr(q.stats), native.ptr(db.stats),
+                    keys.data_ptr(), native.ptr(status), native.ptr(self.last_unverified if status is not None else None),
+                    ws_ptr, ws_bytes, lazy_arg, self._stream()))
         self.launches += 2 if status is None else 6
         if status is not None:
             self._status_log.append(status)
@@ -351,16 +388,28 @@
         kth = torch.empty((Q,), dtype=torch.float32, device=self.device)
         if Q == 0:
             return cand, tau, kth
-        ws_bytes = int(self.lib.emr2a_topk_filter_workspace_bytes(Q, N, D, k))
+        ws_query = self.lib.emr2a_prepare_topk_filter_workspace_bytes if db.pending else \
+            self.lib.emr2a_topk_filter_workspace_bytes
+        ws_bytes = int(ws_query(Q, N, D, k))
         ws = torch.empty((ws_bytes + 256,), dtype=torch.uint8, device=self.device)
         if q_fold is not None:
             q_fold = self.to_device(q_fold, torch.uint8)
             db_fold = self.to_device(db_fold, torch.uint8)
         with torch.cuda.device(self.device):
-            native.check(self.lib.emr2a_topk_filter(
-                q.hi.data_ptr(), _ld(q.hi), db.hi.data_ptr() if N else None, _ld(db.hi) if N else 0, Q, N, D,
-                native.ptr(q_fold), native.ptr(db_fold), int(fold_sorted), int(idx_base), int(k),
-                cand.data_ptr(), tau.data_ptr(), kth.data_ptr(), _round_up(ws.data_ptr(), 256), ws_bytes, self._stream()))
+            if db.pending:
+                lazy_arg, _lazy_keep = _lazy_arg(db, pending_ok=True)
+                native.check(self.lib.emr2a_prepare_topk_filter(
+                    lazy_arg, db.hi.data_ptr(), _ld(db.hi), db.stats.data_ptr(), q.hi.data_ptr(), _ld(q.hi), Q, N, D,
+                    native.ptr(q_fold), native.ptr(db_fold), int(fold_sorted), int(idx_base), int(k),
+                    cand.data_ptr(), tau.data_ptr(), kth.data_ptr(), _round_up(ws.data_ptr(), 256), ws_bytes,
+                    self._stream()))
+                db.pending = False
+            else:
+                native.check(self.lib.emr2a_topk_filter(
+                    q.hi.data_ptr(), _ld(q.hi), db.hi.data_ptr() if N else None, _ld(db.hi) if N else 0, Q, N, D,
+                    native.ptr(q_fold), native.ptr(db_fold), int(fold_sorted), int(idx_base), int(k),
+                    cand.data_ptr(), tau.data_ptr(), kth.data_ptr(), _round_up(ws.data_ptr(), 256), ws_bytes,
+                    self._stream()))
         self.launches += 3
         return cand, tau, kth
 
@@ -532,7 +581,8 @@
         dim = sum(int(s.shape[1]) for s in db_segs if s is not None)
         prec = self.pick_precision(n_q, n_db, dim, k, precision)
         db = self.prepare(db_segs[0], db_segs[1] if len(db_segs) > 1 else None, db_weights[0], db_weights[1], db_flags, prec,
-                          defer_f32=self.defer_default(dim))
+                          defer_f32=self.defer_default(dim),
+                          in_filter=k1_in_filter(n_q, n_db, dim, prec))
         qs = self.prepare(q_segs[0], q_segs[1] if len(q_segs) > 1 else None, q_weights[0], q_weights[1], q_flags, prec)
         keys = self.topk_search(qs, db, k, prec, q_fold=q_fold, db_fold=db_fold)
         res = self.vote_metrics(keys, db_labels, q_labels, n_classes, k_list=k_list, wacc_f32=wacc_f32,
diff --git a/emr2a_b200/native.py b/emr2a_b200/native.py
--- a/emr2a_b200/native.py
+++ b/emr2a_b200/native.py
@@ -12,7 +12,7 @@
 NF_SEGNORM, NF_ROWNORM, NF_ZERO_GUARD, NF_STANDARDIZE = 1, 2, 4, 8
 PREC_FP32, PREC_BF16X3, PREC_BF16X1, PREC_BF16_RESCORE = 0, 1, 2, 3
 SCORE_NONE, SCORE_ZSCORE, SCORE_MINMAX = 0, 1, 2
-ABI_VERSION = 12
+ABI_VERSION = 13
 
 _p = C.c_void_p
 _i64 = C.c_int64
@@ -35,6 +35,12 @@
                                  _i64, _int, _int, _p, _p, _p, _p, _p, _p, _sz, _p, _p]),
     "emr2a_topk_filter_workspace_bytes": (_sz, [_i64, _i64, _int, _int]),
     "emr2a_topk_filter": (_int, [_p, _i64, _p, _i64, _i64, _i64, _int, _p, _p, _int, _i64, _int, _p, _p, _p, _p, _sz, _p]),
+    "emr2a_prepare_topk_search_workspace_bytes": (_sz, [_i64, _i64, _int, _int]),
+    "emr2a_prepare_topk_search": (_int, [_p, _p, _i64, _p, _p, _i64, _p, _i64, _p, _i64, _i64, _int, _p, _p, _int, _i64,
+                                         _int, _p, _p, _p, _p, _sz, _p]),
+    "emr2a_prepare_topk_filter_workspace_bytes": (_sz, [_i64, _i64, _int, _int]),
+    "emr2a_prepare_topk_filter": (_int, [_p, _p, _i64, _p, _p, _i64, _i64, _i64, _int, _p, _p, _int, _i64, _int, _p, _p, _p,
+                                         _p, _sz, _p]),
     "emr2a_rescore_candidates": (_int, [_p, _p, _p, _p, _i64, _p, _i64, _i64, _i64, _int, _i64, _int, _p, _p, _p, _p, _p, _p]),
     "emr2a_verify_merged": (_int, [_p, _int, _i64, _p, _int, _i64, _p, _p, _p]),
     "emr2a_exact_rescan_workspace_bytes": (_sz, [_int, _int]),
diff --git a/include/emr2a.h b/include/emr2a.h
--- a/include/emr2a.h
+++ b/include/emr2a.h
@@ -8,7 +8,7 @@
 extern "C" {
 #endif
 
-#define EMR2A_ABI_VERSION 12
+#define EMR2A_ABI_VERSION 13
 
 enum emr2a_status {
   EMR2A_OK = 0,
@@ -106,6 +106,20 @@
                        const uint16_t* db_hi, int64_t lddb_bf16, const float* q_stats, const float* db_stats,
                        const uint64_t* seed_keys, void* stream);
 
+size_t emr2a_prepare_topk_search_workspace_bytes(int64_t Q, int64_t N, int D, int K);
+int emr2a_prepare_topk_search(const emr2a_lazy_rows* db_raw, uint16_t* db_hi, int64_t lddb_bf16, float* db_stats,
+                              const float* q_f32, int64_t ldq_f32, const uint16_t* q_hi, int64_t ldq_bf16,
+                              const float* q_stats, int64_t Q, int64_t N, int D,
+                              const uint8_t* q_fold, const uint8_t* db_fold, int fold_sorted,
+                              int64_t idx_base, int K, uint64_t* out_keys, int32_t* status_out, uint8_t* unverified_out,
+                              void* workspace, size_t ws_bytes, void* stream);
+size_t emr2a_prepare_topk_filter_workspace_bytes(int64_t Q, int64_t N, int D, int K);
+int emr2a_prepare_topk_filter(const emr2a_lazy_rows* db_raw, uint16_t* db_hi, int64_t lddb_bf16, float* db_stats,
+                              const uint16_t* q_hi, int64_t ldq_bf16, int64_t Q, int64_t N, int D,
+                              const uint8_t* q_fold, const uint8_t* db_fold, int fold_sorted,
+                              int64_t idx_base, int K, uint64_t* cand_out, uint32_t* tau_out, float* kth_out,
+                              void* workspace, size_t ws_bytes, void* stream);
+
 size_t emr2a_range_search_workspace_bytes(int64_t Q, int64_t N, int D);
 int emr2a_range_search(const float* q_f32, int64_t ldq_f32, const uint16_t* q_hi, int64_t ldq_bf16,
                        const float* db_f32, int64_t lddb_f32, const uint16_t* db_hi, int64_t lddb_bf16,
```

After: 634,600, median of 6. +1.7%, better.
